# 82magnolia/piccolo

Measured on AMD Instinct MI355X. Metric: candidate-poses/s, higher is better.
Workload: dtype f32

## Files before the change

### include/piccolo_hip.h

```cpp
#ifndef PICCOLO_HIP_H
#define PICCOLO_HIP_H

#include <stddef.h>
#include <stdint.h>

#ifdef __cplusplus
extern "C" {
#endif

#define PCL_ABI_VERSION 11

#define PCL_EINVAL (-1)
#define PCL_EWORKSPACE (-2)

#define PCL_MAX_POINTS ((int64_t)1 << 27)

#define PCL_RESULT_STRIDE 8

int pcl_abi_version(void);
const char *pcl_error_string(int code);
const char *pcl_source_hash(void);
const char *pcl_library_hash(void);

#define PCL_PANO_F32 0
#define PCL_PANO_U8 1
#define PCL_PANO_F16 2
#define PCL_PANO_U8P 3
#define PCL_PANO_U8V 4
int64_t pcl_cloud_stride(int64_t n);
size_t pcl_cloud_bytes(int64_t n);
int pcl_cloud_pack(const float *xyz, const float *rgb, const int64_t *order, int64_t n, float *cloud, void *stream);
size_t pcl_cloud_sets_bytes(int64_t n, int nsets);
int pcl_cloud_pack_sets(const float *xyz, const float *const *rgb_host, int nsets, const int64_t *order, int64_t n, float *cloud, void *stream);
size_t pcl_cloud_order_workspace_bytes(int64_t n);
int pcl_cloud_order(const float *xyz, int64_t n, int64_t *order, void *workspace, size_t workspace_bytes, void *stream);
int pcl_morton_keys(const float *xyz, int64_t n, const float *lo_host, const float *hi_host, int64_t *keys, void *stream);

size_t pcl_pano_bytes(int H, int W, int pano_format);
int pcl_pano_pack(const float *img_hwc, int H, int W, float *pano, void *stream);
int pcl_pano_pack_u8(const float *img_hwc, int H, int W, uint32_t *pano, int *not_exact, void *stream);
int pcl_pano_pack_u8p(const float *img_hwc, int H, int W, uint32_t *pano, int *not_exact, void *stream);
int pcl_pano_pack_u8v(const float *img_hwc, int H, int W, uint32_t *pano, int *not_exact, void *stream);
int pcl_pano_pack_f16(const float *img_hwc, int H, int W, void *pano, int *not_exact, void *stream);

size_t pcl_loss_workspace_bytes(int64_t n, int B);
size_t pcl_loss_depth_workspace_bytes(int64_t n, int B, int H, int W, int depth_h, int depth_w, int depth_stride);
int pcl_sampling_loss_depth(const float *cloud, int64_t n, const void *pano, int pano_format, int H, int W, const float *trans,
                            const float *rot, int B, int with_grad, int depth_h, int depth_w, float tau, int depth_stride, float *result,
                            void *workspace, size_t workspace_bytes, void *stream);
int pcl_sampling_loss(const float *cloud, int64_t n, const void *pano, int pano_format, int H, int W, const float *trans,
                      const float *rot, int B, int with_grad, const uint8_t *visible, float *result, void *workspace,
                      size_t workspace_bytes, void *stream);

#define PCL_GD_SEQUENTIAL 0
#define PCL_GD_BATCH 1
#define PCL_GD_RESULT_STRIDE 16

typedef struct pcl_gd_hyper {
    double lr;
    double factor;
    int32_t patience;
    int32_t mode;
    int32_t depth_mask;
    float depth_tau;
    int32_t depth_h;
    int32_t depth_w;
    int32_t depth_stride;
    int32_t fuse;
    int32_t images;
    int32_t color_sets;
} pcl_gd_hyper;

size_t pcl_gd_state_bytes(int B);
size_t pcl_gd_workspace_bytes(int64_t n, int B, int H, int W, const pcl_gd_hyper *hyper_host);
int pcl_gd_init(void *state, const float *trans, const float *rot, int B, const pcl_gd_hyper *hyper_host, void *stream);
int pcl_gd_run(const float *cloud, int64_t n, const void *pano, int pano_format, int H, int W, void *state, int B, const float *box,
               const pcl_gd_hyper *hyper_host, int num_iter, float *loss_history, void *workspace,
               size_t workspace_bytes, void *timer, void *stream);
int pcl_gd_result(const void *state, int B, float *result, void *stream);
int pcl_gd_step_from_grads(void *state, int B, const float *loss, const float *grad, const float *box, const pcl_gd_hyper *hyper_host,
                           float *scratch, void *stream);
int pcl_gd_plan(int64_t n, int B, int *nchunks_host, int *poses_per_block_host, int *fused_host);
int pcl_gd_plan_hyper(int64_t n, int B, const pcl_gd_hyper *hyper_host, int *nchunks_host, int *poses_per_block_host, int *fused_host);
int pcl_gd_set_panos(void *state, const uint64_t *panos, int B, void *stream);
int pcl_gd_set_pano_groups(void *state, const uint64_t *panos_host, int nimages, int per_image, void *stream);
int pcl_gd_winner(const void *state, int nimages, int per_image, float *winners, float *leaf_trans, float *leaf_rot, void *stream);

#define PCL_GD_MAX_ROOMS 32
typedef struct pcl_gd_room {
    const float *cloud;
    int64_t n;
    const float *box;
} pcl_gd_room;
size_t pcl_gd_rooms_workspace_bytes(const pcl_gd_room *rooms_host, int nrooms, int per_room, const pcl_gd_hyper *hyper_host);
int pcl_gd_plan_rooms(const pcl_gd_room *rooms_host, int nrooms, int per_room, const pcl_gd_hyper *hyper_host, int *nchunks_host,
                      int *poses_per_block_host, int *fused_host);
int pcl_gd_run_rooms(const pcl_gd_room *rooms_host, int nrooms, const void *pano, int pano_format, int H, int W, void *state, int per_room,
                     const pcl_gd_hyper *hyper_host, int num_iter, float *loss_history, void *workspace, size_t workspace_bytes, void *timer,
                     void *stream);

void *pcl_timer_create(int capacity);
void pcl_timer_destroy(void *timer);
void pcl_timer_reset(void *timer);
void pcl_timer_set_stride(void *timer, int stride);
int pcl_timer_read(void *timer, double *total_ms_host, int *launches_host);
int pcl_timer_calibrate(void *timer, int reps, double *pair_ms_host, void *stream);

int pcl_cloud2idx(const float *xyz, int64_t n, float *coord, void *stream);
int pcl_sample_from_img(const void *pano, int pano_format, int H, int W, const float *coord, int64_t n, float *rgb_out,
                        void *stream);
int pcl_cloud2idx_backward(const float *xyz, const float *grad_coord, int64_t n, float *grad_xyz, void *stream);
int pcl_sample_from_img_backward(const void *pano, int pano_format, int H, int W, const float *coord, const float *grad_rgb,
                                 int64_t n, float *grad_coord, float *grad_img, void *stream);
int pcl_rot_from_ypr(const float *rot, int B, float *R, void *stream);
size_t pcl_quantile_workspace_bytes(void);
int pcl_quantile_box(const float *xyz, int64_t n, double q, float *box, void *workspace, void *stream);

int pcl_scatter_min_depth(const float *xyz_cam, int64_t n, int H, int W, uint64_t *zbuf, void *stream);
int pcl_scatter_min_unpack(const uint64_t *zbuf, int64_t n, int H, int W, float *zmin, int64_t *argmin, void *stream);
int pcl_make_pano(const float *xyz_cam, const float *rgb, int64_t n, int H, int W, float *image, uint64_t *workspace,
                  void *stream);
size_t pcl_hist_trim_workspace_bytes(int ncand, int H, int W, int nsh, int nsw);
size_t pcl_hist_trim_workspace_bytes_n(int64_t n, int ncand, int H, int W, int nsh, int nsw);
int pcl_hist_trim_scores(const float *cloud, int64_t n, const float *img_hwc, int H, int W, const float *trans,
                         const float *rot, int ncand, int nsh, int nsw, float *inter, int32_t *nproj, int32_t *nimg,
                         void *workspace, size_t workspace_bytes, void *stream);
int pcl_hist_trim_reduce(const float *inter, const int32_t *nproj, const int32_t *nimg, int ncand, int nsh, int nsw, float *score,
                         void *stream);
size_t pcl_hist_trim_images_workspace_bytes(int64_t n, int nimages, int cand_per_image, int H, int W, int nsh, int nsw);
int pcl_hist_trim_scores_images(const float *cloud, int64_t n, const float *const *imgs_host, int nimages, int cand_per_image, int H, int W,
                                const float *trans, const float *rot, int nsh, int nsw, float *inter, int32_t *nproj, int32_t *nimg,
                                void *workspace, size_t workspace_bytes, void *stream);
size_t pcl_hist_trim_images_sets_workspace_bytes(int64_t n, int color_sets, int nimages, int cand_per_image, int H, int W, int nsh, int nsw);
int pcl_hist_trim_scores_images_sets(const float *cloud, int64_t n, int color_sets, const float *const *imgs_host, int nimages, int cand_per_image,
                                     int H, int W, const float *trans, const float *rot, int nsh, int nsw, float *inter, int32_t *nproj,
                                     int32_t *nimg, void *workspace, size_t workspace_bytes, void *stream);
int pcl_hist_trim_reduce_images(const float *inter, const int32_t *nproj, const int32_t *nimg, int nimages, int cand_per_image, int nsh,
                                int nsw, float *score, void *stream);
size_t pcl_trim_groups_bytes(int R);
int pcl_select_poses(const float *values, int nprob, int M, int n_keep, int largest, const float *trans, const float *rot,
                     int rot_per_trans, int64_t pose_stride, float *out_trans, float *out_rot, int *out_idx, void *stream);
int pcl_trim_groups(const float *rot, int R, void *groups, void *stream);
size_t pcl_trim_loss_workspace_bytes(int64_t n, int K, int ngroups);
int pcl_trim_loss(const float *cloud, int64_t n, const void *pano, int pano_format, int H, int W, const float *trans, int K,
                  const float *rot, int R, const void *groups, int ngroups, const void *order, float *loss_table, float *count_table,
                  void *workspace, size_t workspace_bytes, void *stream);
size_t pcl_trim_order_bytes(int64_t n, int K, int ngroups);
size_t pcl_trim_order_workspace_bytes(int64_t n, int K, int ngroups);
int pcl_trim_order(const float *cloud, int64_t n, int pano_format, int H, int W, const float *trans, int K, const float *rot, int R,
                   const void *groups, int ngroups, void *order, void *workspace, size_t workspace_bytes, void *stream);
size_t pcl_trim_loss_images_workspace_bytes(int64_t n, int K, int ngroups, int nimages);
int pcl_trim_loss_images(const float *cloud, int64_t n, const void *const *panos_host, int nimages, int pano_format, int H, int W,
                         const float *trans, int K, const float *rot, int R, const void *groups, int ngroups, const void *order,
                         float *loss_tables, float *count_tables, void *workspace, size_t workspace_bytes, void *stream);
int pcl_trim_loss_images_sets(const float *cloud, int64_t n, int color_sets, const void *const *panos_host, int nimages, int pano_format, int H,
                              int W, const float *trans, int K, const float *rot, int R, const void *groups, int ngroups, const void *order,
                              float *loss_tables, float *count_tables, void *workspace, size_t workspace_bytes, void *stream);
int pcl_depth_default(int64_t n, int H, int W, int stride_in, int *depth_h_host, int *depth_w_host, float *tau_host, int *stride_host);
size_t pcl_depth_workspace_bytes(int B, int H, int W);
int pcl_depth_mask(const float *cloud, int64_t n, const float *trans, const float *rot, int B, int H, int W, float tau, int stride,
                   uint8_t *visible, void *workspace, size_t workspace_bytes, void *stream);
size_t pcl_color_template_bytes(int64_t n);
size_t pcl_color_template_workspace_bytes(int64_t n);
int pcl_color_template_build(const float *rgb, int64_t n, float *tmpl, void *workspace, size_t workspace_bytes, void *stream);
size_t pcl_color_workspace_bytes(void);
int pcl_color_match(const float *img_hwc, int H, int W, const float *tmpl, int64_t n, float *out, int32_t *not_exact,
                    void *workspace, size_t workspace_bytes, void *stream);
int pcl_color_mod(const float *img_hwc, int H, int W, const float *rgb, int64_t n, int num_bins, float *out_img,
                  float *out_rgb, void *workspace, size_t workspace_bytes, void *stream);
size_t pcl_histogram_workspace_bytes(int c0, int c1, int c2);
int pcl_histogram(const float *img, const uint8_t *mask, int64_t npix, int c0, int c1, int c2, int normalize, float eps,
                  float *hist, void *workspace, size_t workspace_bytes, void *stream);
int pcl_histogram_intersection(const float *a, const float *b, int batch, int nbins, float *out, void *stream);
int pcl_transform_cloud(const float *xyz, int64_t n, const float *trans, const float *rot, float *out, void *stream);

int64_t pcl_cloud_txt_rows(const char *path);
int64_t pcl_cloud_txt_read(const char *path, int64_t rows, int cols, double *out, int nthreads);

#ifdef __cplusplus
}
#endif
#endif
```

### piccolo_amd/_lib.py

```python
import ctypes
import os

from . import build as _build

_c = ctypes
_vp, _i64, _int, _sz, _dbl = _c.c_void_p, _c.c_int64, _c.c_int, _c.c_size_t, _c.c_double

ABI_VERSION = 11
RESULT_STRIDE = 8
GD_RESULT_STRIDE = 16
GD_SEQUENTIAL, GD_BATCH = 0, 1
PANO_F32, PANO_U8, PANO_F16, PANO_U8P, PANO_U8V = 0, 1, 2, 3, 4


class GdHyper(_c.Structure):
    _fields_ = [("lr", _dbl), ("factor", _dbl), ("patience", _c.c_int32), ("mode", _c.c_int32),
                ("depth_mask", _c.c_int32), ("depth_tau", _c.c_float), ("depth_h", _c.c_int32), ("depth_w", _c.c_int32),
                ("depth_stride", _c.c_int32), ("fuse", _c.c_int32), ("images", _c.c_int32), ("color_sets", _c.c_int32)]


GD_MAX_ROOMS = 32


class GdRoom(_c.Structure):
    _fields_ = [("cloud", _vp), ("n", _i64), ("box", _vp)]


SIGNATURES = {
    "pcl_abi_version": (_int, []),
    "pcl_error_string": (_c.c_char_p, [_int]),
    "pcl_source_hash": (_c.c_char_p, []),
    "pcl_library_hash": (_c.c_char_p, []),
    "pcl_cloud_stride": (_i64, [_i64]),
    "pcl_cloud_bytes": (_sz, [_i64]),
    "pcl_cloud_pack": (_int, [_vp, _vp, _vp, _i64, _vp, _vp]),
    "pcl_cloud_sets_bytes": (_sz, [_i64, _int]),
    "pcl_cloud_pack_sets": (_int, [_vp, _c.POINTER(_vp), _int, _vp, _i64, _vp, _vp]),
    "pcl_morton_keys": (_int, [_vp, _i64, _c.POINTER(_c.c_float), _c.POINTER(_c.c_float), _vp, _vp]),
    "pcl_pano_bytes": (_sz, [_int, _int, _int]),
    "pcl_pano_pack": (_int, [_vp, _int, _int, _vp, _vp]),
    "pcl_cloud_order_workspace_bytes": (_sz, [_i64]),
    "pcl_cloud_order": (_int, [_vp, _i64, _vp, _vp, _sz, _vp]),
    "pcl_pano_pack_u8": (_int, [_vp, _int, _int, _vp, _vp, _vp]),
    "pcl_pano_pack_u8p": (_int, [_vp, _int, _int, _vp, _vp, _vp]),
    "pcl_pano_pack_u8v": (_int, [_vp, _int, _int, _vp, _vp, _vp]),
    "pcl_pano_pack_f16": (_int, [_vp, _int, _int, _vp, _vp, _vp]),
    "pcl_loss_workspace_bytes": (_sz, [_i64, _int]),
    "pcl_sampling_loss": (_int, [_vp, _i64, _vp, _int, _int, _int, _vp, _vp, _int, _int, _vp, _vp, _vp, _sz, _vp]),
    "pcl_loss_depth_workspace_bytes": (_sz, [_i64, _int, _int, _int, _int, _int, _int]),
    "pcl_sampling_loss_depth": (_int, [_vp, _i64, _vp, _int, _int, _int, _vp, _vp, _int, _int, _int, _int, _c.c_float, _int, _vp, _vp, _sz, _vp]),
    "pcl_depth_default": (_int, [_i64, _int, _int, _int, _c.POINTER(_int), _c.POINTER(_int), _c.POINTER(_c.c_float), _c.POINTER(_int)]),
    "pcl_gd_state_bytes": (_sz, [_int]),
    "pcl_gd_workspace_bytes": (_sz, [_i64, _int, _int, _int, _c.POINTER(GdHyper)]),
    "pcl_hist_trim_workspace_bytes": (_sz, [_int, _int, _int, _int, _int]),
    "pcl_hist_trim_workspace_bytes_n": (_sz, [_i64, _int, _int, _int, _int, _int]),
    "pcl_hist_trim_scores": (_int, [_vp, _i64, _vp, _int, _int, _vp, _vp, _int, _int, _int, _vp, _vp, _vp, _vp, _sz, _vp]),
    "pcl_color_template_bytes": (_sz, [_i64]),
    "pcl_color_template_workspace_bytes": (_sz, [_i64]),
    "pcl_color_template_build": (_int, [_vp, _i64, _vp, _vp, _sz, _vp]),
    "pcl_color_workspace_bytes": (_sz, []),
    "pcl_color_match": (_int, [_vp, _int, _int, _vp, _i64, _vp, _vp, _vp, _sz, _vp]),
    "pcl_color_mod": (_int, [_vp, _int, _int, _vp, _i64, _int, _vp, _vp, _vp, _sz, _vp]),
    "pcl_histogram_workspace_bytes": (_sz, [_int, _int, _int]),
    "pcl_histogram": (_int, [_vp, _vp, _i64, _int, _int, _int, _int, _c.c_float, _vp, _vp, _sz, _vp]),
    "pcl_histogram_intersection": (_int, [_vp, _vp, _int, _int, _vp, _vp]),
    "pcl_cloud_txt_rows": (_i64, [_c.c_char_p]),
    "pcl_cloud_txt_read": (_i64, [_c.c_char_p, _i64, _int, _vp, _int]),
    "pcl_hist_trim_reduce": (_int, [_vp, _vp, _vp, _int, _int, _int, _vp, _vp]),
    "pcl_hist_trim_images_workspace_bytes": (_sz, [_i64, _int, _int, _int, _int, _int, _int]),
    "pcl_hist_trim_scores_images": (_int, [_vp, _i64, _c.POINTER(_vp), _int, _int, _int, _int, _vp, _vp, _int, _int, _vp, _vp, _vp, _vp, _sz, _vp]),
    "pcl_hist_trim_reduce_images": (_int, [_vp, _vp, _vp, _int, _int, _int, _int, _vp, _vp]),
    "pcl_hist_trim_images_sets_workspace_bytes": (_sz, [_i64, _int, _int, _int, _int, _int, _int, _int]),
    "pcl_hist_trim_scores_images_sets": (_int, [_vp, _i64, _int, _c.POINTER(_vp), _int, _int, _int, _int, _vp, _vp, _int, _int, _vp, _vp, _vp, _vp, _sz, _vp]),
    "pcl_trim_groups_bytes": (_sz, [_int]),
    "pcl_trim_groups": (_int, [_vp, _int, _vp, _vp]),
    "pcl_trim_loss_workspace_bytes": (_sz, [_i64, _int, _int]),
    "pcl_trim_loss": (_int, [_vp, _i64, _vp, _int, _int, _int, _vp, _int, _vp, _int, _vp, _int, _vp, _vp, _vp, _vp, _sz, _vp]),
    "pcl_trim_order_bytes": (_sz, [_i64, _int, _int]),
    "pcl_trim_order_workspace_bytes": (_sz, [_i64, _int, _int]),
    "pcl_trim_order": (_int, [_vp, _i64, _int, _int, _int, _vp, _int, _vp, _int, _vp, _int, _vp, _vp, _sz, _vp]),
    "pcl_trim_loss_images_workspace_bytes": (_sz, [_i64, _int, _int, _int]),
    "pcl_trim_loss_images": (_int, [_vp, _i64, _c.POINTER(_vp), _int, _int, _int, _int, _vp, _int, _vp, _int, _vp, _int, _vp, _vp, _vp, _vp, _sz, _vp]),
    "pcl_trim_loss_images_sets": (_int, [_vp, _i64, _int, _c.POINTER(_vp), _int, _int, _int, _int, _vp, _int, _vp, _int, _vp, _int, _vp, _vp, _vp, _vp, _sz, _vp]),
    "pcl_depth_workspace_bytes": (_sz, [_int, _int, _int]),
    "pcl_depth_mask": (_int, [_vp, _i64, _vp, _vp, _int, _int, _int, _c.c_float, _int, _vp, _vp, _sz, _vp]),
    "pcl_gd_init": (_int, [_vp, _vp, _vp, _int, _c.POINTER(GdHyper), _vp]),
    "pcl_gd_run": (_int, [_vp, _i64, _vp, _int, _int, _int, _vp, _int, _vp, _c.POINTER(GdHyper), _int, _vp, _vp, _sz, _vp, _vp]),
    "pcl_timer_create": (_vp, [_int]),
    "pcl_timer_destroy": (None, [_vp]),
    "pcl_timer_reset": (None, [_vp]),
    "pcl_timer_set_stride": (None, [_vp, _int]),
    "pcl_timer_read": (_int, [_vp, _c.POINTER(_dbl), _c.POINTER(_int)]),
    "pcl_timer_calibrate": (_int, [_vp, _int, _c.POINTER(_dbl), _vp]),
    "pcl_gd_result": (_int, [_vp, _int, _vp, _vp]),
    "pcl_gd_step_from_grads": (_int, [_vp, _int, _vp, _vp, _vp, _vp, _vp, _vp]),
    "pcl_gd_plan": (_int, [_i64, _int, _c.POINTER(_int), _c.POINTER(_int), _c.POINTER(_int)]),
    "pcl_gd_plan_hyper": (_int, [_i64, _int, _c.POINTER(GdHyper), _c.POINTER(_int), _c.POINTER(_int), _c.POINTER(_int)]),
    "pcl_gd_set_panos": (_int, [_vp, _vp, _int, _vp]),
    "pcl_gd_set_pano_groups": (_int, [_vp, _c.POINTER(_c.c_uint64), _int, _int, _vp]),
    "pcl_gd_winner": (_int, [_vp, _int, _int, _vp, _vp, _vp, _vp]),
    "pcl_gd_rooms_workspace_bytes": (_sz, [_c.POINTER(GdRoom), _int, _int, _c.POINTER(GdHyper)]),
    "pcl_gd_plan_rooms": (_int, [_c.POINTER(GdRoom), _int, _int, _c.POINTER(GdHyper), _c.POINTER(_int), _c.POINTER(_int), _c.POINTER(_int)]),
    "pcl_gd_run_rooms": (_int, [_c.POINTER(GdRoom), _int, _vp, _int, _int, _int, _vp, _int, _c.POINTER(GdHyper), _int, _vp, _vp, _sz, _vp, _vp]),
    "pcl_select_poses": (_int, [_vp, _int, _int, _int, _int, _vp, _vp, _int, _i64, _vp, _vp, _vp, _vp]),
    "pcl_cloud2idx": (_int, [_vp, _i64, _vp, _vp]),
    "pcl_sample_from_img": (_int, [_vp, _int, _int, _int, _vp, _i64, _vp, _vp]),
    "pcl_cloud2idx_backward": (_int, [_vp, _vp, _i64, _vp, _vp]),
    "pcl_sample_from_img_backward": (_int, [_vp, _int, _int, _int, _vp, _vp, _i64, _vp, _vp, _vp]),
    "pcl_rot_from_ypr": (_int, [_vp, _int, _vp, _vp]),
    "pcl_quantile_workspace_bytes": (_sz, []),
    "pcl_quantile_box": (_int, [_vp, _i64, _dbl, _vp, _vp, _vp]),
    "pcl_scatter_min_depth": (_int, [_vp, _i64, _int, _int, _vp, _vp]),
    "pcl_scatter_min_unpack": (_int, [_vp, _i64, _int, _int, _vp, _vp, _vp]),
    "pcl_make_pano": (_int, [_vp, _vp, _i64, _int, _int, _vp, _vp, _vp]),
    "pcl_transform_cloud": (_int, [_vp, _i64, _vp, _vp, _vp, _vp]),
}

_lib = None


class PiccoloHipError(RuntimeError):
    pass


def so_path():
    return os.environ.get("PCL_SO", _build.SO)


def load():
    global _lib
    if _lib is not None:
        return _lib
    import torch
    path = so_path()
    if not os.path.exists(path):
        raise PiccoloHipError(
            "piccolo_amd: %s not found. The MI355X HIP library is the only back end (no CPU fallback); "
            "build it with `python -m piccolo_amd.build`." % path)
    lib = ctypes.CDLL(path)
    for name, (res, args) in SIGNATURES.items():
        fn = getattr(lib, name)
        fn.restype, fn.argtypes = res, args
    if lib.pcl_abi_version() != ABI_VERSION:
        raise PiccoloHipError("piccolo_amd: ABI mismatch: library %d, binding %d" % (lib.pcl_abi_version(), ABI_VERSION))
    _lib = lib
    return lib


def check(rc, what):
    if rc != 0:
        raise PiccoloHipError("%s failed: %s (code %d)" % (what, load().pcl_error_string(rc).decode(), rc))
```

### piccolo_amd/csrc/pcl_device.h

```cpp
#pragma once
#include <hip/hip_runtime.h>
#include <stddef.h>
#include <stdint.h>

#include "../../include/piccolo_hip.h"

#ifdef PCL_EXPERIMENTS
#include <stdlib.h>
static inline int pcl_knob_read(const char* name, int dflt)
{
    const char* v = getenv(name);
    return v && *v ? atoi(v) : dflt;
}
#define PCL_KNOB(NAME, dflt) pcl_knob_read("PCL_" #NAME, (dflt))
#else
#define PCL_KNOB(NAME, dflt) (dflt)
#endif

#define PCL_WAVE 64
#define PCL_BLOCK 256
#define PCL_NACC 8

typedef float pcl_f4 __attribute__((ext_vector_type(4)));
typedef int pcl_i4 __attribute__((ext_vector_type(4)));
typedef int pcl_i2 __attribute__((ext_vector_type(2)));

struct PclPoseRec {
    float R[9];
    float t[3];
    uint32_t pano_lo, pano_hi;
    uint32_t cset;
    float pad;
};
static_assert(sizeof(PclPoseRec) == 64, "pose record is one 64-byte scalar-load line");
static_assert(offsetof(PclPoseRec, R) == 0 && offsetof(PclPoseRec, t) == 36, "pose record: t directly after R[9]");

struct PclGdPose {
    double lr;
    double best;
    float leaf[6];
    float fwd[6];
    float m[6];
    float v[6];
    float last_loss;
    int32_t num_bad;
    int32_t step;
    int32_t pad;
    double beta1_pow, beta2_pow;
    float sc[4];
};
static_assert(sizeof(PclGdPose) == 160, "GD state record");

struct PclDims {
    int H, W;
    int Wp;
    float half_w, half_h;
    float off_x, off_y;
    float k_phi, k_theta;
    float c_scale;
    float k_ix, k_iy;
};

__host__ __device__ inline PclDims pcl_make_dims(int H, int W, int pano_format = PCL_PANO_F32)
{
    PclDims d;
    d.H = H; d.W = W; d.Wp = W + 2;
    d.half_w = 0.5f * (float)W; d.half_h = 0.5f * (float)H;
    d.off_x = 0.5f * (float)(W - 1) + 1.0f; d.off_y = 0.5f * (float)(H - 1) + 1.0f;
    d.k_phi = (float)(-(double)W / (2.0 * 3.14159265358979323846));
    d.k_theta = (float)((double)H / 3.14159265358979323846);
    d.c_scale = 1.0f;
    d.k_ix = (float)(-(double)W / (2.0 * 3.14159265358979323846));
    d.k_iy = (float)(-(double)H / 3.14159265358979323846);
    if (pano_format == PCL_PANO_U8 || pano_format == PCL_PANO_F16) {
        d.k_phi = (float)(-(double)W / (2.0 * 3.14159265358979323846) / 255.0);
        d.k_theta = (float)((double)H / 3.14159265358979323846 / 255.0);
        d.c_scale = (float)(1.0 / 255.0);
    }
    return d;
}

struct PclDepthGrid {
    int Hd, Wd, last;
    float wm1, hm1;
    float tol2;
};
__host__ __device__ inline PclDepthGrid pcl_make_depth_grid(int Hd, int Wd, float tau)
{
    PclDepthGrid g;
    g.Hd = Hd; g.Wd = Wd; g.last = Hd * Wd - 1;
    g.wm1 = (float)(Wd - 1); g.hm1 = (float)(Hd - 1);
    g.tol2 = (1.0f + tau) * (1.0f + tau);
    return g;
}
struct PclDepthLook {
    const uint32_t* zbuf;
    PclDepthGrid grid;
    uint32_t* zclear;
    int64_t zclear_vec4;
};
__device__ inline void pcl_rot_from_ypr(float yaw, float pitch, float roll, float R[9])
{
    double sy, cy, sp, cp, sr, cr;
    sincos((double)yaw, &sy, &cy);
    sincos((double)pitch, &sp, &cp);
    sincos((double)roll, &sr, &cr);
    sy = (double)(float)sy; cy = (double)(float)cy; sp = (double)(float)sp;
    cp = (double)(float)cp; sr = (double)(float)sr; cr = (double)(float)cr;
    R[0] = (float)(cy * cp); R[1] = (float)(cy * sp * sr - sy * cr); R[2] = (float)(cy * sp * cr + sy * sr);
    R[3] = (float)(sy * cp); R[4] = (float)(sy * sp * sr + cy * cr); R[5] = (float)(sy * sp * cr - cy * sr);
    R[6] = (float)(-sp);     R[7] = (float)(cp * sr);                R[8] = (float)(cp * cr);
}

__device__ inline void pcl_write_pose_rec(PclPoseRec* rec, const float p[6])
{
    float R[9];
    pcl_rot_from_ypr(p[3], p[4], p[5], R);
    for (int k = 0; k < 9; k++) rec->R[k] = R[k];
    rec->t[0] = p[0]; rec->t[1] = p[1]; rec->t[2] = p[2];
    rec->pano_lo = 0u; rec->pano_hi = 0u;
    rec->cset = 0u; rec->pad = 0.f;
}

__device__ inline void pcl_write_pose_rec_fast(PclPoseRec* rec, const float p[6], float sc[4])
{
    float sy, cy, sp, cp, sr, cr;
    sincosf(p[3], &sy, &cy);
    sincosf(p[4], &sp, &cp);
    sincosf(p[5], &sr, &cr);
    double dsy = sy, dcy = cy, dsp = sp, dcp = cp, dsr = sr, dcr = cr;
    rec->R[0] = (float)(dcy * dcp); rec->R[1] = (float)(dcy * dsp * dsr - dsy * dcr); rec->R[2] = (float)(dcy * dsp * dcr + dsy * dsr);
    rec->R[3] = (float)(dsy * dcp); rec->R[4] = (float)(dsy * dsp * dsr + dcy * dcr); rec->R[5] = (float)(dsy * dsp * dcr - dcy * dsr);
    rec->R[6] = (float)(-dsp);      rec->R[7] = (float)(dcp * dsr);                   rec->R[8] = (float)(dcp * dcr);
    rec->t[0] = p[0]; rec->t[1] = p[1]; rec->t[2] = p[2];
    sc[0] = sy; sc[1] = cy; sc[2] = sp; sc[3] = cp;
}

__device__ inline void pcl_cloud2idx_point(float px, float py, float pz, float& gx, float& gy)
{
#pragma clang fp contract(off)
    const float pi = 3.14159265358979323846f, two_pi = 6.28318530717958647692f;
    float rho = sqrtf(px * px + py * py);
    float theta = atan2f(rho, pz + 1e-6f);
    float phi = atan2f(py, px + 1e-6f) + pi;
    float cx = 1.0f - phi / two_pi;
    float cy = theta / pi;
    gx = 2.0f * cx - 1.0f;
    gy = 2.0f * cy - 1.0f;
}

__device__ __forceinline__ float pcl_atan_poly(float t)
{
    float s = t * t;
    float p = 2.4566929979e-03f;
    p = fmaf(p, s, -1.4401224869e-02f);
    p = fmaf(p, s, 3.9780993102e-02f);
    p = fmaf(p, s, -7.2348362183e-02f);
    p = fmaf(p, s, 1.0498935044e-01f);
    p = fmaf(p, s, -1.4161225936e-01f);
    p = fmaf(p, s, 1.9985906258e-01f);
    p = fmaf(p, s, -3.3332596993e-01f);
    p = fmaf(p, s, 9.9999988638e-01f);
    return p * t;
}

__device__ __forceinline__ float pcl_atan2(float y, float x)
{
    const float pi = 3.14159265358979323846f, half_pi = 1.57079632679489661923f;
    float ax = fabsf(x), ay = fabsf(y);
    float mx = fmaxf(fmaxf(ax, ay), 1e-37f), mn = fminf(ax, ay);
    float r = pcl_atan_poly(mn * __builtin_amdgcn_rcpf(mx));
    r = ay > ax ? half_pi - r : r;
    r = x < 0.f ? pi - r : r;
    return copysignf(r, y);
}

__device__ __forceinline__ float pcl_atan2_ypos(float y, float x)
{
    const float pi = 3.14159265358979323846f, half_pi = 1.57079632679489661923f;
    float ax = fabsf(x);
    float mx = fmaxf(fmaxf(ax, y), 1e-37f), mn = fminf(ax, y);
    float r = pcl_atan_poly(mn * __builtin_amdgcn_rcpf(mx));
    r = y > ax ? half_pi - r : r;
    return x < 0.f ? pi - r : r;
}

__device__ inline __amdgpu_buffer_rsrc_t pcl_tex_rsrc(const void* pano, int H, int W, int texel_bytes = 16)
{
    return __builtin_amdgcn_make_buffer_rsrc((void*)pano, 0, (int)((size_t)(H + 2) * (size_t)(W + 2) * (size_t)texel_bytes),
                                             0x00020000);
}

__host__ __device__ constexpr int pcl_texel_bytes(int fmt) { return fmt == PCL_PANO_U8 ? 4 : fmt == PCL_PANO_F16 ? 8 : 16; }

__device__ inline pcl_i2 pcl_texel_pair_u8(__amdgpu_buffer_rsrc_t rsrc, int voff, int soff)
{
    return __builtin_amdgcn_raw_buffer_load_b64(rsrc, voff, soff, 0);
}
__device__ __forceinline__ float pcl_ub0(int v) { float f; asm("v_cvt_f32_ubyte0 %0, %1" : "=v"(f) : "v"(v)); return f; }
__device__ __forceinline__ float pcl_ub1(int v) { float f; asm("v_cvt_f32_ubyte1 %0, %1" : "=v"(f) : "v"(v)); return f; }
__device__ __forceinline__ float pcl_ub2(int v) { float f; asm("v_cvt_f32_ubyte2 %0, %1" : "=v"(f) : "v"(v)); return f; }

__device__ inline pcl_f4 pcl_texel(__amdgpu_buffer_rsrc_t rsrc, int voff, int soff)
{
    pcl_i4 v = __builtin_amdgcn_raw_buffer_load_b128(rsrc, voff, soff, 0);
    return __builtin_bit_cast(pcl_f4, v);
}

template <int CTRL>
__device__ __forceinline__ float pcl_dpp(float v)
{
    return __builtin_bit_cast(float, __builtin_amdgcn_update_dpp(0, __builtin_bit_cast(int, v), CTRL, 0xf, 0xf, true));
}
__device__ __forceinline__ float pcl_wave_sum(float v)
{
    v += pcl_dpp<0xB1>(v);
    v += pcl_dpp<0x4E>(v);
    v += pcl_dpp<0x141>(v);
    v += pcl_dpp<0x140>(v);
    float r0 = __builtin_bit_cast(float, __builtin_amdgcn_readlane(__builtin_bit_cast(int, v), 0));
    float r1 = __builtin_bit_cast(float, __builtin_amdgcn_readlane(__builtin_bit_cast(int, v), 16));
    float r2 = __builtin_bit_cast(float, __builtin_amdgcn_readlane(__builtin_bit_cast(int, v), 32));
    float r3 = __builtin_bit_cast(float, __builtin_amdgcn_readlane(__builtin_bit_cast(int, v), 48));
    return (r0 + r1) + (r2 + r3);
}

template <int CTRL>
__device__ __forceinline__ double pcl_dpp_d(double v)
{
    pcl_i2 w = __builtin_bit_cast(pcl_i2, v);
    w.x = __builtin_amdgcn_update_dpp(0, w.x, CTRL, 0xf, 0xf, true);
    w.y = __builtin_amdgcn_update_dpp(0, w.y, CTRL, 0xf, 0xf, true);
    return __builtin_bit_cast(double, w);
}
__device__ __forceinline__ double pcl_readlane_d(double v, int lane)
{
    pcl_i2 w = __builtin_bit_cast(pcl_i2, v);
    w.x = __builtin_amdgcn_readlane(w.x, lane);
    w.y = __builtin_amdgcn_readlane(w.y, lane);
    return __builtin_bit_cast(double, w);
}
__device__ __forceinline__ double pcl_wave_sum_d(double v)
{
    v += pcl_dpp_d<0xB1>(v);
    v += pcl_dpp_d<0x4E>(v);
    v += pcl_dpp_d<0x141>(v);
    v += pcl_dpp_d<0x140>(v);
    return (pcl_readlane_d(v, 0) + pcl_readlane_d(v, 16)) + (pcl_readlane_d(v, 32) + pcl_readlane_d(v, 48));
}

#define PCL_LAUNCH_CHECK()                         \
    do {                                           \
        hipError_t e_ = hipGetLastError();         \
        if (e_ != hipSuccess) return (int)e_;      \
    } while (0)
```

### piccolo_amd/csrc/pcl_loss.hip

```cpp
#include <stdlib.h>

#include "pcl_gd_device.h"
#include "pcl_sample_device.h"

struct PclLossArgs {
    const float* cloud;
    int64_t n, stride;
    const void* pano;
    PclDims dims;
    const PclPoseRec* poses;
    int B;
    const uint8_t* visible;
    const uint32_t* zbuf;
    PclDepthGrid dgrid;
    pcl_i4* zclear;
    int zclear_per_block;
    int64_t zclear_total;
    float* partials;
    int nchunks;
    int ngroups;
    int flip;
    int seg_len;
    int xcd_groups;
    int steps_base, steps_rem;
    int color_sets;
};

#define PCL_STEP (2 * PCL_BLOCK)

#ifdef PCL_BLOCK_TRACE
__device__ unsigned long long* pcl_trace_buf = nullptr;
extern "C" int pcl_debug_set_block_trace(unsigned long long* buf)
{
    return (int)hipMemcpyToSymbol(HIP_SYMBOL(pcl_trace_buf), &buf, sizeof(buf));
}
#define PCL_TRACE_NOW() __builtin_amdgcn_s_memrealtime()
__global__ void pcl_debug_stamp_kernel(unsigned long long* slot) { *slot = PCL_TRACE_NOW(); }
extern "C" int pcl_debug_stamp(unsigned long long* slot, void* stream)
{
    hipLaunchKernelGGL(pcl_debug_stamp_kernel, dim3(1), dim3(1), 0, (hipStream_t)stream, slot);
    return (int)hipGetLastError();
}
#endif

template <int G, bool FUSED>
__device__ __forceinline__ unsigned pcl_room_select(const PclLossArgs& a_in, const PclFuseArgs& f_in, const PclRoomTable* __restrict__ tb, PclLossArgs& a,
                                                    PclFuseArgs& f)
{
    int r = -1;
#pragma unroll
    for (int q = 0; q < PCL_GD_MAX_ROOMS; q++) r += (int)blockIdx.x >= pcl_rfl(tb->block0[q]) ? 1 : 0;
    const PclRoomRec* __restrict__ rm = tb->rec + r;
    const int group0 = pcl_rfl(rm->group0), pose0 = group0 * G;
    const long long poff = (long long)pcl_rfl64((unsigned long long)rm->partials);
    a = a_in;
    a.cloud = (const float*)pcl_rfl64(rm->cloud);
    a.n = pcl_rfl(rm->n); a.stride = pcl_rfl(rm->stride);
    a.nchunks = pcl_rfl(rm->nchunks); a.seg_len = pcl_rfl(rm->seg_len);
    a.steps_base = pcl_rfl(rm->steps_base); a.steps_rem = pcl_rfl(rm->steps_rem);
    a.poses = a_in.poses + pose0;
    a.partials = a_in.partials + poff;
    a.xcd_groups = 0;
    f = f_in;
    if constexpr (FUSED) {
        f.partials_in = f_in.partials_in + poff;
        f.st_in = f_in.st_in + pose0; f.recs_in = f_in.recs_in + pose0;
        f.st_out = f_in.st_out + pose0; f.recs_out = f_in.recs_out + pose0;
        f.box = (const float*)pcl_rfl64(rm->box);
        f.loss_out = f_in.loss_out ? f_in.loss_out + pose0 : nullptr;
    }
    return blockIdx.x - (unsigned)pcl_rfl(rm->block0);
}

template <int G, bool GRAD, int VIS, int FMT, bool FUSED, bool CS = false, bool RM = false>
__device__ __forceinline__ void pcl_loss_body(const PclLossArgs& a_in, const PclFuseArgs& f_in, const PclRoomTable* rooms = nullptr)
{
    PclLossArgs a_rm;
    PclFuseArgs f_rm;
    unsigned bid = blockIdx.x;
    if constexpr (RM) bid = pcl_room_select<G, FUSED>(a_in, f_in, rooms, a_rm, f_rm);
    const PclLossArgs& a = RM ? a_rm : a_in;
    const PclFuseArgs& f = RM ? f_rm : f_in;
    int group, chunk;
    if (a.xcd_groups) {
        const int gpx = a.ngroups >> 3, j = (int)(bid >> 3), cj = j / gpx;
        group = (int)(bid & 7) * gpx + (j - cj * gpx);
        chunk = a.flip ? a.nchunks - 1 - cj : cj;
    } else {
        const int lq = (int)(bid >> 3) / a.ngroups;
        group = (int)(bid >> 3) - lq * a.ngroups;
        const int lc = a.flip ? (a.nchunks >> 3) - 1 - lq : lq;
        const int run = lc / a.seg_len;
        chunk = (run * 8 + (int)(bid & 7)) * a.seg_len + (lc - run * a.seg_len);
    }
    const int pose0 = group * G;

    PclPose6 P6[G];
    unsigned PANO[G][2];
    __amdgpu_buffer_rsrc_t tex = pcl_tex_rsrc(a.pano, a.dims.H, a.dims.W, pcl_texel_bytes(FMT));
    __amdgpu_buffer_rsrc_t cld = __builtin_amdgcn_make_buffer_rsrc((void*)a.cloud, 0, CS ? (int)(a.stride * (3 + 3 * a.color_sets) * 4) : (int)(a.stride * 6 * 4),
                                                                   0x00020000);
    const int plane = (int)a.stride * 4;
    int cplane = 3 * plane;
    if constexpr (CS) cplane = (int)(3u + 3u * (unsigned)__builtin_amdgcn_readfirstlane((int)(a.poses + pose0)->cset)) * plane;
    __amdgpu_buffer_rsrc_t zb = __amdgpu_buffer_rsrc_t();
    if constexpr (VIS == 2) zb = __builtin_amdgcn_make_buffer_rsrc((void*)a.zbuf, 0, (int)((unsigned)a.B * (unsigned)(a.dgrid.last + 1) * 4u), 0x00020000);

    f2 acc[G][PCL_NACC];
    int count[G];
#pragma unroll
    for (int g = 0; g < G; g++) {
        count[g] = 0;
#pragma unroll
        for (int k = 0; k < PCL_NACC; k++) acc[g][k] = F2(0.f);
    }

    int first = chunk * a.steps_base + min(chunk, a.steps_rem);
    int nsteps = a.steps_base + (chunk < a.steps_rem ? 1 : 0);
    const int begin = first * PCL_STEP;
    int end = begin + nsteps * PCL_STEP;
    if (end > (int)a.n) end = (int)a.n;
    const int last = (int)a.n - 1;

    auto load_step = [&](int base, float (&dst)[2][6]) {
        int j0 = min(base + (int)threadIdx.x, last), j1 = min(base + PCL_BLOCK + (int)threadIdx.x, last);
#pragma unroll
        for (int k = 0; k < 6; k++) {
            const int soff = (CS && k >= 3) ? cplane + (k - 3) * plane : k * plane;
            dst[0][k] = __builtin_bit_cast(float, __builtin_amdgcn_raw_buffer_load_b32(cld, j0 * 4, soff, 0));
            dst[1][k] = __builtin_bit_cast(float, __builtin_amdgcn_raw_buffer_load_b32(cld, j1 * 4, soff, 0));
        }
    };
    auto eval_step = [&](int base, const float (&src)[2][6]) {
        const int i0 = base + threadIdx.x, i1 = i0 + PCL_BLOCK;
        const bool valid0 = i0 < end, valid1 = i1 < end;
        const unsigned long long vmask0 = __builtin_amdgcn_ballot_w64(valid0), vmask1 = __builtin_amdgcn_ballot_w64(valid1);
        f2 x = {src[0][0], src[1][0]}, y = {src[0][1], src[1][1]}, z = {src[0][2], src[1][2]};
        f2 ncr = {src[0][3], src[1][3]}, ncg = {src[0][4], src[1][4]}, ncb = {src[0][5], src[1][5]};
#ifndef PCL_NO_ROTATE_PAIR
        f2 rot_p[G][3];
#ifdef PCL_TIMING_ONLY_NO_ROTATION
        if constexpr (G == 2) {
            const f2 oa = F2((a.poses + pose0)->t[0]), ob = F2((a.poses + pose0 + 1)->t[0]);
            rot_p[0][0] = x - oa; rot_p[0][1] = y; rot_p[0][2] = z;
            rot_p[1][0] = x - ob; rot_p[1][1] = y; rot_p[1][2] = z;
        } else
#endif
        if constexpr (G == 2) {
            if constexpr (FUSED) pcl_rotate2x2(x, y, z, P6[0], P6[1], rot_p[0][0], rot_p[0][1], rot_p[0][2], rot_p[1][0], rot_p[1][1], rot_p[1][2]);
            else pcl_rotate2x2(x, y, z, pcl_pose6(a.poses + pose0), pcl_pose6(a.poses + pose0 + 1), rot_p[0][0], rot_p[0][1], rot_p[0][2],
                               rot_p[1][0], rot_p[1][1], rot_p[1][2]);
        }
#endif
#pragma unroll
        for (int g = 0; g < G; g++) {
            const PclPoseRec* __restrict__ pr = a.poses + (pose0 + g);
            bool ok0 = valid0, ok1 = valid1;
            unsigned long long m0 = vmask0, m1 = vmask1;
            if constexpr (VIS == 1) {
                const uint8_t* vis = a.visible + (int64_t)(pose0 + g) * a.n;
                ok0 = ok0 && vis[min(i0, last)] != 0;
                ok1 = ok1 && vis[min(i1, last)] != 0;
                m0 = __builtin_amdgcn_ballot_w64(ok0); m1 = __builtin_amdgcn_ballot_w64(ok1);
            }
            __amdgpu_buffer_rsrc_t tg = tex;
            unsigned pano_lo = pr->pano_lo, pano_hi = pr->pano_hi;
            if constexpr (FUSED) {
                pano_lo = PANO[g][0]; pano_hi = PANO[g][1];
            }
            if (pano_lo | pano_hi) {
                const void* pp = (const void*)(((unsigned long long)pano_hi << 32) | (unsigned long long)pano_lo);
                tg = pcl_tex_rsrc(pp, a.dims.H, a.dims.W, pcl_texel_bytes(FMT));
            }
            PclProj<FMT> pj;
            const int zoff = VIS == 2 ? (int)((unsigned)(pose0 + g) * (unsigned)(a.dgrid.last + 1) * 4u) : 0;
#ifndef PCL_NO_ROTATE_PAIR
            if constexpr (G == 2) {
                pj.px = rot_p[g][0]; pj.py = rot_p[g][1]; pj.pz = rot_p[g][2];
                pcl_project2_rotated<FMT, VIS == 2>(tg, a.dims, pj, zb, zoff, &a.dgrid);
            } else
#endif
            if constexpr (FUSED) pcl_project2<FMT, VIS == 2>(x, y, z, P6[g], tg, a.dims, pj, zb, zoff, &a.dgrid);
            else pcl_project2<FMT, VIS == 2>(x, y, z, pcl_pose6(pr), tg, a.dims, pj, zb, zoff, &a.dgrid);
            if constexpr (VIS == 2) {
                f2 d2 = pcl_fma2(pj.pz, pj.pz, pj.rho2);
                const bool v0 = d2.x <= __uint_as_float(pj.zq0), v1 = d2.y <= __uint_as_float(pj.zq1);
                ok0 = ok0 & v0; ok1 = ok1 & v1;
                m0 = __builtin_amdgcn_ballot_w64(ok0); m1 = __builtin_amdgcn_ballot_w64(ok1);
            }
            pcl_sample2<GRAD, FMT>(pj, ncr, ncg, ncb, ok0, ok1, m0, m1, tg, a.dims, acc[g], count[g]);
        }
    };
    float bufA[2][6], bufB[2][6];
    load_step(begin, bufA);
    if constexpr (FUSED) {
        static_assert(PCL_BLOCK == PCL_GD_THREADS, "the fused prologue reduces with the epilogue kernel's thread layout");
        __shared__ double gd_rows[(PCL_GD_THREADS / 16) * 2 * G][4];
        __shared__ double gd_sums[G][PCL_NACC];
        __shared__ float pose_sh[G][12];
        pcl_gd_finish_group<G, true>(f.partials_in, a.nchunks, group, (int)threadIdx.x, f.st_in, f.recs_in, f.st_out, f.recs_out, chunk == 0,
                                     f.box, f.factor, f.patience, f.mode, f.loss_out, gd_rows, gd_sums, pose_sh);
        __syncthreads();
#pragma unroll
        for (int g = 0; g < G; g++) {
            float v[12];
#pragma unroll
            for (int k = 0; k < 12; k++) v[k] = __builtin_bit_cast(float, __builtin_amdgcn_readfirstlane(__builtin_bit_cast(int, pose_sh[g][k])));
            P6[g] = PclPose6{(f2){v[0], v[1]}, (f2){v[2], v[3]}, (f2){v[4], v[5]}, (f2){v[6], v[7]}, (f2){v[8], v[9]}, (f2){v[10], v[11]}};
            const PclPoseRec* pr = a.poses + (pose0 + g);
            PANO[g][0] = (unsigned)__builtin_amdgcn_readfirstlane((int)pr->pano_lo);
            PANO[g][1] = (unsigned)__builtin_amdgcn_readfirstlane((int)pr->pano_hi);
        }
    }

    for (int base = begin; base < end; base += 2 * PCL_STEP) {
        load_step(base + PCL_STEP, bufB);
        eval_step(base, bufA);
        if (base + PCL_STEP < end) {
            load_step(base + 2 * PCL_STEP, bufA);
            eval_step(base + PCL_STEP, bufB);
        }
    }

    __shared__ float red[PCL_BLOCK / PCL_WAVE][G * PCL_NACC];
    const int lane = threadIdx.x & 63, wave = threadIdx.x >> 6;
#pragma unroll
    for (int g = 0; g < G; g++)
#pragma unroll
        for (int k = 0; k < PCL_NACC; k++) {
            if (k == 1) {
                if (lane == 0) red[wave][g * PCL_NACC + 1] = (float)count[g];
                continue;
            }
            if (!GRAD && k >= 2) continue;
            float s = pcl_wave_sum(acc[g][k].x + acc[g][k].y);
            if (lane == 0) red[wave][g * PCL_NACC + k] = s;
        }
    __syncthreads();
    if (threadIdx.x < G * PCL_NACC) {
        int g = threadIdx.x / PCL_NACC, k = threadIdx.x - g * PCL_NACC;
        float s = 0.f;
        if (GRAD || k < 2) s = red[0][threadIdx.x] + red[1][threadIdx.x] + red[2][threadIdx.x] + red[3][threadIdx.x];
        a.partials[pcl_partials_row(a.nchunks, G, group, chunk, g) + k] = s;
    }
    if constexpr (VIS == 2) {
        if (a.zclear) {
            const pcl_i4 inf4 = {0x7f800000, 0x7f800000, 0x7f800000, 0x7f800000};
            const int64_t z0 = (int64_t)blockIdx.x * a.zclear_per_block;
            for (int i = threadIdx.x; i < a.zclear_per_block; i += PCL_BLOCK)
                if (z0 + i < a.zclear_total) a.zclear[z0 + i] = inf4;
        }
    }
#ifdef PCL_BLOCK_TRACE
    if (pcl_trace_buf && threadIdx.x == 0) {
        unsigned hw, xcc;
        asm volatile("s_getreg_b32 %0, hwreg(HW_REG_HW_ID)" : "=s"(hw));
        asm volatile("s_getreg_b32 %0, hwreg(HW_REG_XCC_ID)" : "=s"(xcc));
        unsigned long long* t = pcl_trace_buf + (size_t)blockIdx.x * 4;
        t[0] = 0; t[1] = 0; t[2] = PCL_TRACE_NOW(); t[3] = ((unsigned long long)xcc << 32) | hw;
    }
#endif
}

template <int G, bool GRAD, int VIS, int FMT>
__global__ void __launch_bounds__(PCL_BLOCK) pcl_loss_kernel(PclLossArgs a)
{
    pcl_loss_body<G, GRAD, VIS, FMT, false>(a, PclFuseArgs{});
}

template <int G, int FMT>
__global__ void __launch_bounds__(PCL_BLOCK) pcl_loss_fused_kernel(PclLossArgs a, PclFuseArgs f)
{
    pcl_loss_body<G, true, 0, FMT, true>(a, f);
}

template <int G, int FMT>
__global__ void __launch_bounds__(PCL_BLOCK) pcl_loss_sets_kernel(PclLossArgs a)
{
    pcl_loss_body<G, true, 0, FMT, false, true>(a, PclFuseArgs{});
}

template <int G, int FMT>
__global__ void __launch_bounds__(PCL_BLOCK) pcl_loss_fused_sets_kernel(PclLossArgs a, PclFuseArgs f)
{
    pcl_loss_body<G, true, 0, FMT, true, true>(a, f);
}

template <int G, int FMT>
__global__ void __launch_bounds__(PCL_BLOCK) pcl_loss_rooms_kernel(PclLossArgs a, const PclRoomTable* rooms)
{
    pcl_loss_body<G, true, 0, FMT, false, false, true>(a, PclFuseArgs{}, rooms);
}

template <int G, int FMT>
__global__ void __launch_bounds__(PCL_BLOCK) pcl_loss_fused_rooms_kernel(PclLossArgs a, PclFuseArgs f, const PclRoomTable* rooms)
{
    pcl_loss_body<G, true, 0, FMT, true, false, true>(a, f, rooms);
}



struct PclPlan {
    int G, ngroups, nchunks;
    int seg_len;
    int steps_base, steps_rem;
};

static int pcl_xcd_seg_len(int nchunks, int64_t nblocks)
{
    static const int runs_env = PCL_KNOB(XCD_RUNS, 0);
    int cpx = nchunks / 8, runs = runs_env < 1 || runs_env > cpx ? cpx : runs_env;
    if (runs_env < 1 && nblocks <= 1024) runs = 1;
    while (cpx % runs) runs--;
    return cpx / runs;
}

static PclPlan pcl_plan(int64_t n, int B)
{
    static const int g_env = PCL_KNOB(G, 0), blocks_env = PCL_KNOB(BLOCKS, 4096);
    PclPlan p;
    p.G = (B % 2 == 0) ? 2 : 1;
    if (g_env > 0 && B % g_env == 0) p.G = g_env;
    p.ngroups = B / p.G;
    int64_t want = blocks_env / p.ngroups;
    if (want < 64) want = 64;
    if (n > 2000000 && want < n / 8192) want = n / 8192;
    int64_t steps = (n + PCL_STEP - 1) / PCL_STEP;
    if (steps < 3 * want) {
        int64_t alt = steps / 3;
        if (alt < 1024 / p.ngroups) alt = 1024 / p.ngroups;
        if (alt < 32) alt = 32;
        if (alt < want) want = alt;
    }
    if (want > steps) want = steps;
    want = ((want + 7) / 8) * 8;
    p.nchunks = (int)want;
    p.steps_base = (int)(steps / want);
    p.steps_rem = (int)(steps % want);
    p.seg_len = pcl_xcd_seg_len(p.nchunks, (int64_t)p.nchunks * p.ngroups);
    return p;
}

static PclPlan pcl_plan_sets(int64_t n, int B, int sets)
{
    if (sets <= 1) return pcl_plan(n, B);
    PclPlan p = pcl_plan(n, B / sets);
    p.ngroups = B / p.G;
    p.seg_len = pcl_xcd_seg_len(p.nchunks, (int64_t)p.nchunks * p.ngroups);
    return p;
}

void pcl_plan_room(int64_t n, int per_room, int* G, int* ngroups, int* nchunks, int* seg_len, int* steps_base, int* steps_rem)
{
    const PclPlan p = pcl_plan(n, per_room);
    *G = p.G; *ngroups = p.ngroups; *nchunks = p.nchunks; *seg_len = p.seg_len; *steps_base = p.steps_base; *steps_rem = p.steps_rem;
}

size_t pcl_partials_bytes(int64_t n, int B, int sets)
{
    PclPlan p = pcl_plan_sets(n, B, sets);
    return (size_t)p.nchunks * (size_t)B * PCL_NACC * sizeof(float);
}

int pcl_plan_nchunks(int64_t n, int B, int sets) { return pcl_plan_sets(n, B, sets).nchunks; }
int pcl_plan_nblocks(int64_t n, int B, int sets) { PclPlan p = pcl_plan_sets(n, B, sets); return p.nchunks * p.ngroups; }
int pcl_plan_G(int64_t n, int B, int sets) { return pcl_plan_sets(n, B, sets).G; }

void pcl_plan_for_groups(int64_t n, int ngroups, int* nchunks, int* seg_len, int* steps_base, int* steps_rem)
{
    PclPlan p = pcl_plan(n, 2 * ngroups);
    static const int chunks_env = PCL_KNOB(TRIM_CHUNKS, 0);
    int auto_chunks = 0;
    const int64_t per_chunk = n <= 2000000 ? 8192 : 16384;
    if (chunks_env < 8 && n > 64 * per_chunk) auto_chunks = (int)((n + per_chunk - 1) / per_chunk);
    if (chunks_env >= 8 || auto_chunks) {
        int64_t steps = (n + PCL_STEP - 1) / PCL_STEP, want = (((chunks_env >= 8 ? chunks_env : auto_chunks) + 7) / 8) * 8;
        if (want > steps) want = ((steps + 7) / 8) * 8;
        p.nchunks = (int)want; p.steps_base = (int)(steps / want); p.steps_rem = (int)(steps % want);
        static const int runs_env = PCL_KNOB(TRIM_RUNS, 0);
        int cpx = p.nchunks / 8, runs = runs_env < 1 || runs_env > cpx ? cpx : runs_env;
        while (cpx % runs) runs--;
        p.seg_len = cpx / runs;
    }
    *nchunks = p.nchunks; *seg_len = p.seg_len; *steps_base = p.steps_base; *steps_rem = p.steps_rem;
}

template <int G, int FMT>
static void pcl_launch_g(const PclLossArgs& a, int nblk, bool grad, int vis, hipStream_t s)
{
    if (grad) {
        if (vis == 2) hipLaunchKernelGGL((pcl_loss_kernel<G, true, 2, FMT>), dim3(nblk), dim3(PCL_BLOCK), 0, s, a);
        else if (vis) hipLaunchKernelGGL((pcl_loss_kernel<G, true, 1, FMT>), dim3(nblk), dim3(PCL_BLOCK), 0, s, a);
        else hipLaunchKernelGGL((pcl_loss_kernel<G, true, 0, FMT>), dim3(nblk), dim3(PCL_BLOCK), 0, s, a);
    } else {
        if (vis == 2) hipLaunchKernelGGL((pcl_loss_kernel<G, false, 2, FMT>), dim3(nblk), dim3(PCL_BLOCK), 0, s, a);
        else if (vis) hipLaunchKernelGGL((pcl_loss_kernel<G, false, 1, FMT>), dim3(nblk), dim3(PCL_BLOCK), 0, s, a);
        else hipLaunchKernelGGL((pcl_loss_kernel<G, false, 0, FMT>), dim3(nblk), dim3(PCL_BLOCK), 0, s, a);
    }
}

template <int FMT>
static void pcl_launch_f(const PclLossArgs& a, int G, int nblk, bool grad, int vis, hipStream_t s)
{
    if (G == 4) pcl_launch_g<4, FMT>(a, nblk, grad, vis, s);
    else if (G == 2) pcl_launch_g<2, FMT>(a, nblk, grad, vis, s);
    else pcl_launch_g<1, FMT>(a, nblk, grad, vis, s);
}

template <int FMT>
static void pcl_launch_fused(const PclLossArgs& a, const PclFuseArgs& f, int G, int nblk, hipStream_t s)
{
    if (G == 4) hipLaunchKernelGGL((pcl_loss_fused_kernel<4, FMT>), dim3(nblk), dim3(PCL_BLOCK), 0, s, a, f);
    else if (G == 2) hipLaunchKernelGGL((pcl_loss_fused_kernel<2, FMT>), dim3(nblk), dim3(PCL_BLOCK), 0, s, a, f);
    else hipLaunchKernelGGL((pcl_loss_fused_kernel<1, FMT>), dim3(nblk), dim3(PCL_BLOCK), 0, s, a, f);
}

template <int FMT>
static void pcl_launch_sets(const PclLossArgs& a, const PclFuseArgs* f, int G, int nblk, hipStream_t s)
{
    if (f) {
        if (G == 4) hipLaunchKernelGGL((pcl_loss_fused_sets_kernel<4, FMT>), dim3(nblk), dim3(PCL_BLOCK), 0, s, a, *f);
        else if (G == 2) hipLaunchKernelGGL((pcl_loss_fused_sets_kernel<2, FMT>), dim3(nblk), dim3(PCL_BLOCK), 0, s, a, *f);
        else hipLaunchKernelGGL((pcl_loss_fused_sets_kernel<1, FMT>), dim3(nblk), dim3(PCL_BLOCK), 0, s, a, *f);
    } else {
        if (G == 4) hipLaunchKernelGGL((pcl_loss_sets_kernel<4, FMT>), dim3(nblk), dim3(PCL_BLOCK), 0, s, a);
        else if (G == 2) hipLaunchKernelGGL((pcl_loss_sets_kernel<2, FMT>), dim3(nblk), dim3(PCL_BLOCK), 0, s, a);
        else hipLaunchKernelGGL((pcl_loss_sets_kernel<1, FMT>), dim3(nblk), dim3(PCL_BLOCK), 0, s, a);
    }
}

int pcl_launch_loss_rooms(const PclRoomTable* rooms, const void* pano, int pano_format, int H, int W, const PclPoseRec* poses, int B, int G,
                          int ngroups, int nblk, float* partials, hipStream_t s, int flip, const PclFuseArgs* fuse)
{
    if (pano_format != PCL_PANO_F32 && pano_format != PCL_PANO_U8 && pano_format != PCL_PANO_F16) return PCL_EINVAL;
    if ((int64_t)(H + 2) * (W + 2) * pcl_texel_bytes(pano_format) >= ((int64_t)1 << 31)) return PCL_EINVAL;
    PclLossArgs a = PclLossArgs{};
    a.pano = pano; a.dims = pcl_make_dims(H, W, pano_format);
    a.poses = poses; a.B = B; a.partials = partials;
    a.ngroups = ngroups; a.flip = flip & 1; a.xcd_groups = 0; a.color_sets = 1;
    const dim3 grid(nblk), blk(PCL_BLOCK);
    if (fuse) {
        if (pano_format == PCL_PANO_U8) {
            if (G == 2) hipLaunchKernelGGL((pcl_loss_fused_rooms_kernel<2, PCL_PANO_U8>), grid, blk, 0, s, a, *fuse, rooms);
            else hipLaunchKernelGGL((pcl_loss_fused_rooms_kernel<1, PCL_PANO_U8>), grid, blk, 0, s, a, *fuse, rooms);
        } else if (pano_format == PCL_PANO_F16) {
            if (G == 2) hipLaunchKernelGGL((pcl_loss_fused_rooms_kernel<2, PCL_PANO_F16>), grid, blk, 0, s, a, *fuse, rooms);
            else hipLaunchKernelGGL((pcl_loss_fused_rooms_kernel<1, PCL_PANO_F16>), grid, blk, 0, s, a, *fuse, rooms);
        } else {
            if (G == 2) hipLaunchKernelGGL((pcl_loss_fused_rooms_kernel<2, PCL_PANO_F32>), grid, blk, 0, s, a, *fuse, rooms);
            else hipLaunchKernelGGL((pcl_loss_fused_rooms_kernel<1, PCL_PANO_F32>), grid, blk, 0, s, a, *fuse, rooms);
        }
    } else {
        if (pano_format == PCL_PANO_U8) {
            if (G == 2) hipLaunchKernelGGL((pcl_loss_rooms_kernel<2, PCL_PANO_U8>), grid, blk, 0, s, a, rooms);
            else hipLaunchKernelGGL((pcl_loss_rooms_kernel<1, PCL_PANO_U8>), grid, blk, 0, s, a, rooms);
        } else if (pano_format == PCL_PANO_F16) {
            if (G == 2) hipLaunchKernelGGL((pcl_loss_rooms_kernel<2, PCL_PANO_F16>), grid, blk, 0, s, a, rooms);
            else hipLaunchKernelGGL((pcl_loss_rooms_kernel<1, PCL_PANO_F16>), grid, blk, 0, s, a, rooms);
        } else {
            if (G == 2) hipLaunchKernelGGL((pcl_loss_rooms_kernel<2, PCL_PANO_F32>), grid, blk, 0, s, a, rooms);
            else hipLaunchKernelGGL((pcl_loss_rooms_kernel<1, PCL_PANO_F32>), grid, blk, 0, s, a, rooms);
        }
    }
    PCL_LAUNCH_CHECK();
    return 0;
}

int pcl_launch_loss(const float* cloud, int64_t n, const void* pano, int pano_format, int H, int W, const PclPoseRec* poses,
                    int B, bool grad, const uint8_t* visible, float* partials, hipStream_t s, int flip, const PclFuseArgs* fuse,
                    const PclDepthLook* depth, int color_sets)
{
    if (pano_format != PCL_PANO_F32 && pano_format != PCL_PANO_U8 && pano_format != PCL_PANO_F16) return PCL_EINVAL;
    if (n > PCL_MAX_POINTS || (int64_t)(H + 2) * (W + 2) * pcl_texel_bytes(pano_format) >= ((int64_t)1 << 31)) return PCL_EINVAL;
    const bool sets = color_sets > 1;
    if (sets && (B % color_sets || !grad || visible || depth || pcl_cloud_sets_bytes(n, color_sets) == 0)) return PCL_EINVAL;
    PclPlan p = pcl_plan_sets(n, B, color_sets);
    PclLossArgs a;
    a.cloud = cloud; a.n = n; a.stride = pcl_cloud_stride(n);
    a.pano = pano; a.dims = pcl_make_dims(H, W, pano_format);
    a.poses = poses; a.B = B; a.visible = visible; a.partials = partials;
    a.zbuf = nullptr; a.dgrid = PclDepthGrid{};
    a.zclear = nullptr; a.zclear_per_block = 0; a.zclear_total = 0;
    if (depth) {
        if (visible || !depth->zbuf || depth->grid.Hd <= 0 || depth->grid.Wd <= 0) return PCL_EINVAL;
        if ((int64_t)B * depth->grid.Hd * depth->grid.Wd * 4 >= ((int64_t)1 << 32)) return PCL_EINVAL;
        a.zbuf = depth->zbuf; a.dgrid = depth->grid;
        if (depth->zclear) {
            const int64_t nblk64 = (int64_t)p.nchunks * p.ngroups;
            a.zclear = (pcl_i4*)depth->zclear;
            a.zclear_total = depth->zclear_vec4;
            a.zclear_per_block = (int)((depth->zclear_vec4 + nblk64 - 1) / nblk64);
        }
    }
    a.nchunks = p.nchunks; a.ngroups = p.ngroups; a.seg_len = p.seg_len; a.flip = flip & 1; a.steps_base = p.steps_base; a.steps_rem = p.steps_rem;
    a.color_sets = sets ? color_sets : 1;
    static const int xg_env = PCL_KNOB(XCD_GROUPS, -1);
    a.xcd_groups = ((flip & 2) != 0 || xg_env == 1) && xg_env != 0 && p.ngroups % 8 == 0 ? 1 : 0;
    int nblk = p.nchunks * p.ngroups;
    const int vis = depth ? 2 : visible != nullptr ? 1 : 0;
    if (sets) {
        if (pano_format == PCL_PANO_U8) pcl_launch_sets<PCL_PANO_U8>(a, fuse, p.G, nblk, s);
        else if (pano_format == PCL_PANO_F16) pcl_launch_sets<PCL_PANO_F16>(a, fuse, p.G, nblk, s);
        else pcl_launch_sets<PCL_PANO_F32>(a, fuse, p.G, nblk, s);
        PCL_LAUNCH_CHECK();
        return 0;
    }
    if (fuse) {
        if (!grad || vis) return PCL_EINVAL;
        if (pano_format == PCL_PANO_U8) pcl_launch_fused<PCL_PANO_U8>(a, *fuse, p.G, nblk, s);
        else if (pano_format == PCL_PANO_F16) pcl_launch_fused<PCL_PANO_F16>(a, *fuse, p.G, nblk, s);
        else pcl_launch_fused<PCL_PANO_F32>(a, *fuse, p.G, nblk, s);
        PCL_LAUNCH_CHECK();
        return 0;
    }
    if (pano_format == PCL_PANO_U8) pcl_launch_f<PCL_PANO_U8>(a, p.G, nblk, grad, vis, s);
    else if (pano_format == PCL_PANO_F16) pcl_launch_f<PCL_PANO_F16>(a, p.G, nblk, grad, vis, s);
    else pcl_launch_f<PCL_PANO_F32>(a, p.G, nblk, grad, vis, s);
    PCL_LAUNCH_CHECK();
    return 0;
}
```

### piccolo_amd/csrc/pcl_pack.hip

```cpp
#include "pcl_device.h"

#include <rocprim/device/device_radix_sort.hpp>

extern "C" int pcl_abi_version(void) { return PCL_ABI_VERSION; }

#ifndef PCL_SOURCE_HASH
#define PCL_SOURCE_HASH "unstamped"
#endif
extern "C" const char* pcl_source_hash(void) { return PCL_SOURCE_HASH; }
#ifndef PCL_LIBRARY_HASH
#define PCL_LIBRARY_HASH "unstamped"
#endif
extern "C" const char* pcl_library_hash(void) { return PCL_LIBRARY_HASH; }

extern "C" const char* pcl_error_string(int code)
{
    if (code == 0) return "success";
    if (code == PCL_EINVAL) return "piccolo_hip: invalid argument";
    if (code == PCL_EWORKSPACE) return "piccolo_hip: workspace too small";
    if (code > 0) return hipGetErrorString((hipError_t)code);
    return "piccolo_hip: unknown error";
}

extern "C" int64_t pcl_cloud_stride(int64_t n) { return n <= 0 ? 0 : ((n + 255) / 256) * 256; }
extern "C" size_t pcl_cloud_bytes(int64_t n) { return (size_t)pcl_cloud_stride(n) * 6 * sizeof(float); }
extern "C" size_t pcl_pano_bytes(int H, int W, int pano_format)
{
    if (H <= 0 || W <= 0) return 0;
    if (pano_format == PCL_PANO_U8P) return (size_t)((H + 3) >> 1) * (size_t)(W + 2) * 8;
    if (pano_format == PCL_PANO_U8V) return (size_t)(H + 2) * (size_t)(W + 2) * 8;
    if (pano_format != PCL_PANO_F32 && pano_format != PCL_PANO_U8 && pano_format != PCL_PANO_F16) return 0;
    return (size_t)(H + 2) * (size_t)(W + 2) * (size_t)pcl_texel_bytes(pano_format);
}

__global__ void __launch_bounds__(PCL_BLOCK) pcl_cloud_pack_kernel(const float* __restrict__ xyz, const float* __restrict__ rgb,
                                                                   const int64_t* __restrict__ order, int64_t n,
                                                                   int64_t stride, float* __restrict__ cloud)
{
    int64_t i = (int64_t)blockIdx.x * PCL_BLOCK + threadIdx.x;
    if (i >= stride) return;
    float v[6] = {0.f, 0.f, 0.f, 0.f, 0.f, 0.f};
    if (i < n) {
        int64_t j = order ? order[i] : i;
        v[0] = xyz[3 * j]; v[1] = xyz[3 * j + 1]; v[2] = xyz[3 * j + 2];
        v[3] = -rgb[3 * j]; v[4] = -rgb[3 * j + 1]; v[5] = -rgb[3 * j + 2];
    }
#pragma unroll
    for (int k = 0; k < 6; k++) cloud[k * stride + i] = v[k];
}

extern "C" int pcl_cloud_pack(const float* xyz, const float* rgb, const int64_t* order, int64_t n, float* cloud, void* stream)
{
    if (!xyz || !rgb || !cloud || n <= 0) return PCL_EINVAL;
    int64_t stride = pcl_cloud_stride(n);
    hipLaunchKernelGGL(pcl_cloud_pack_kernel, dim3((unsigned)(stride / PCL_BLOCK)), dim3(PCL_BLOCK), 0, (hipStream_t)stream,
                       xyz, rgb, order, n, stride, cloud);
    PCL_LAUNCH_CHECK();
    return 0;
}

extern "C" size_t pcl_cloud_sets_bytes(int64_t n, int nsets)
{
    if (n <= 0 || n > PCL_MAX_POINTS || nsets <= 0) return 0;
    if (nsets == 1) return pcl_cloud_bytes(n);
    const int64_t bytes = (int64_t)pcl_cloud_stride(n) * 4 * (3 + 3 * (int64_t)nsets);
    return bytes < ((int64_t)1 << 31) ? (size_t)bytes : 0;
}

#define PCL_PACK_SETS 16
struct PclRgbList { const float* p[PCL_PACK_SETS]; };

__global__ void __launch_bounds__(PCL_BLOCK) pcl_cloud_pack_sets_kernel(const float* __restrict__ xyz, PclRgbList rgb, int k0, int m,
                                                                        const int64_t* __restrict__ order, int64_t n, int64_t stride,
                                                                        float* __restrict__ cloud)
{
    int64_t i = (int64_t)blockIdx.x * PCL_BLOCK + threadIdx.x;
    if (i >= stride) return;
    const int64_t j = i < n ? (order ? order[i] : i) : 0;
    if (k0 == 0)
        for (int c = 0; c < 3; c++) cloud[c * stride + i] = i < n ? xyz[3 * j + c] : 0.f;
    for (int k = 0; k < m; k++)
        for (int c = 0; c < 3; c++) cloud[(3 + 3 * (int64_t)(k0 + k) + c) * stride + i] = i < n ? -rgb.p[k][3 * j + c] : 0.f;
}

extern "C" int pcl_cloud_pack_sets(const float* xyz, const float* const* rgb_host, int nsets, const int64_t* order, int64_t n, float* cloud,
                                   void* stream)
{
    if (!xyz || !rgb_host || !cloud || n <= 0 || nsets <= 0) return PCL_EINVAL;
    if (pcl_cloud_sets_bytes(n, nsets) == 0) return PCL_EINVAL;
    for (int k = 0; k < nsets; k++)
        if (!rgb_host[k]) return PCL_EINVAL;
    if (nsets == 1) return pcl_cloud_pack(xyz, rgb_host[0], order, n, cloud, stream);
    const int64_t stride = pcl_cloud_stride(n);
    for (int k0 = 0; k0 < nsets; k0 += PCL_PACK_SETS) {
        const int m = nsets - k0 < PCL_PACK_SETS ? nsets - k0 : PCL_PACK_SETS;
        PclRgbList l;
        for (int k = 0; k < PCL_PACK_SETS; k++) l.p[k] = k < m ? rgb_host[k0 + k] : nullptr;
        hipLaunchKernelGGL(pcl_cloud_pack_sets_kernel, dim3((unsigned)(stride / PCL_BLOCK)), dim3(PCL_BLOCK), 0, (hipStream_t)stream, xyz, l, k0, m,
                           order, n, stride, cloud);
        PCL_LAUNCH_CHECK();
    }
    return 0;
}

__device__ inline uint64_t pcl_spread21(uint32_t v)
{
    uint64_t x = v & 0x1fffffu;
    x = (x | x << 32) & 0x1f00000000ffffull;
    x = (x | x << 16) & 0x1f0000ff0000ffull;
    x = (x | x << 8) & 0x100f00f00f00f00full;
    x = (x | x << 4) & 0x10c30c30c30c30c3ull;
    x = (x | x << 2) & 0x1249249249249249ull;
    return x;
}

__global__ void __launch_bounds__(PCL_BLOCK) pcl_morton_kernel(const float* __restrict__ xyz, int64_t n, float lx, float ly,
                                                               float lz, float sx, float sy, float sz,
                                                               int64_t* __restrict__ keys)
{
    int64_t i = (int64_t)blockIdx.x * PCL_BLOCK + threadIdx.x;
    if (i >= n) return;
    const float top = 2097151.f;
    float fx = __builtin_amdgcn_fmed3f((xyz[3 * i] - lx) * sx, 0.f, top);
    float fy = __builtin_amdgcn_fmed3f((xyz[3 * i + 1] - ly) * sy, 0.f, top);
    float fz = __builtin_amdgcn_fmed3f((xyz[3 * i + 2] - lz) * sz, 0.f, top);
    uint64_t k = pcl_spread21((uint32_t)fx) | (pcl_spread21((uint32_t)fy) << 1) | (pcl_spread21((uint32_t)fz) << 2);
    keys[i] = (int64_t)k;
}

extern "C" int pcl_morton_keys(const float* xyz, int64_t n, const float* lo, const float* hi, int64_t* keys, void* stream)
{
    if (!xyz || !lo || !hi || !keys || n <= 0) return PCL_EINVAL;
    float s[3];
    for (int k = 0; k < 3; k++) s[k] = hi[k] > lo[k] ? 2097151.f / (hi[k] - lo[k]) : 0.f;
    hipLaunchKernelGGL(pcl_morton_kernel, dim3((unsigned)((n + PCL_BLOCK - 1) / PCL_BLOCK)), dim3(PCL_BLOCK), 0,
                       (hipStream_t)stream, xyz, n, lo[0], lo[1], lo[2], s[0], s[1], s[2], keys);
    PCL_LAUNCH_CHECK();
    return 0;
}

__device__ __forceinline__ unsigned int pcl_ordered_key(float v)
{
    unsigned int b = __float_as_uint(v);
    return (b & 0x80000000u) ? ~b : (b | 0x80000000u);
}
__device__ __forceinline__ float pcl_ordered_value(unsigned int k)
{
    return __uint_as_float((k & 0x80000000u) ? (k & 0x7fffffffu) : ~k);
}

__global__ void __launch_bounds__(PCL_BLOCK) pcl_bbox_kernel(const float* __restrict__ xyz, int64_t n, unsigned int* __restrict__ box)
{
    unsigned int lo[3] = {~0u, ~0u, ~0u}, hi[3] = {0u, 0u, 0u};
    for (int64_t i = (int64_t)blockIdx.x * PCL_BLOCK + threadIdx.x; i < n; i += (int64_t)gridDim.x * PCL_BLOCK) {
#pragma unroll
        for (int c = 0; c < 3; c++) {
            unsigned int k = pcl_ordered_key(xyz[3 * i + c]);
            lo[c] = min(lo[c], k); hi[c] = max(hi[c], k);
        }
    }
#pragma unroll
    for (int c = 0; c < 3; c++) {
#pragma unroll
        for (int o = 32; o > 0; o >>= 1) {
            lo[c] = min(lo[c], (unsigned int)__shfl_xor((int)lo[c], o, 64));
            hi[c] = max(hi[c], (unsigned int)__shfl_xor((int)hi[c], o, 64));
        }
        if ((threadIdx.x & 63) == 0) { atomicMin(&box[c], lo[c]); atomicMax(&box[3 + c], hi[c]); }
    }
}

__global__ void __launch_bounds__(PCL_BLOCK) pcl_morton_box_kernel(const float* __restrict__ xyz, int64_t n, const unsigned int* __restrict__ box,
                                                                   unsigned long long* __restrict__ keys, int64_t* __restrict__ iota)
{
    int64_t i = (int64_t)blockIdx.x * PCL_BLOCK + threadIdx.x;
    if (i >= n) return;
    const float top = 2097151.f;
    unsigned long long k = 0ull;
#pragma unroll
    for (int c = 0; c < 3; c++) {
        float lo = pcl_ordered_value(box[c]), hi = pcl_ordered_value(box[3 + c]);
        float sc = hi > lo ? top / (hi - lo) : 0.f;
        float f = __builtin_amdgcn_fmed3f((xyz[3 * i + c] - lo) * sc, 0.f, top);
        k |= pcl_spread21((uint32_t)f) << c;
    }
    keys[i] = k;
    iota[i] = i;
}

static size_t order_align(size_t v) { return (v + 255) & ~(size_t)255; }
static size_t order_sort_temp_bytes(int64_t n)
{
    size_t bytes = 0;
    (void)rocprim::radix_sort_pairs<rocprim::default_config, const unsigned long long*, unsigned long long*, const int64_t*, int64_t*>(
        nullptr, bytes, nullptr, nullptr, nullptr, nullptr, (size_t)n, 0, 63, nullptr, false);
    return bytes;
}

extern "C" size_t pcl_cloud_order_workspace_bytes(int64_t n)
{
    if (n <= 0) return 0;
    return order_align(64) + 3 * order_align((size_t)n * 8) + order_align(order_sort_temp_bytes(n));
}

extern "C" int pcl_cloud_order(const float* xyz, int64_t n, int64_t* order, void* workspace, size_t workspace_bytes, void* stream)
{
    if (!xyz || !order || !workspace || n <= 0 || n > PCL_MAX_POINTS) return PCL_EINVAL;
    if (workspace_bytes < pcl_cloud_order_workspace_bytes(n)) return PCL_EWORKSPACE;
    hipStream_t s = (hipStream_t)stream;
    char* ws = (char*)workspace;
    unsigned int* box = (unsigned int*)ws; ws += order_align(64);
    unsigned long long* keys = (unsigned long long*)ws; ws += order_align((size_t)n * 8);
    unsigned long long* keys_sorted = (unsigned long long*)ws; ws += order_align((size_t)n * 8);
    int64_t* iota = (int64_t*)ws; ws += order_align((size_t)n * 8);
    hipError_t e = hipMemsetAsync(box, 0xff, 12, s);
    if (e == hipSuccess) e = hipMemsetAsync(box + 3, 0, 12, s);
    if (e != hipSuccess) return (int)e;
    int64_t blocks = (n + PCL_BLOCK - 1) / PCL_BLOCK;
    hipLaunchKernelGGL(pcl_bbox_kernel, dim3((unsigned)(blocks < 1024 ? blocks : 1024)), dim3(PCL_BLOCK), 0, s, xyz, n, box);
    hipLaunchKernelGGL(pcl_morton_box_kernel, dim3((unsigned)blocks), dim3(PCL_BLOCK), 0, s, xyz, n, box, keys, iota);
    PCL_LAUNCH_CHECK();
    size_t temp_bytes = order_sort_temp_bytes(n);
    e = rocprim::radix_sort_pairs(ws, temp_bytes, (const unsigned long long*)keys, keys_sorted, (const int64_t*)iota, order, (size_t)n, 0, 63,
                                  s, false);
    return e == hipSuccess ? 0 : (int)e;
}

__global__ void __launch_bounds__(PCL_BLOCK) pcl_pano_pack_kernel(const float* __restrict__ img, int H, int W,
                                                                  pcl_f4* __restrict__ pano)
{
    int Wp = W + 2, Hp = H + 2;
    int64_t i = (int64_t)blockIdx.x * PCL_BLOCK + threadIdx.x;
    if (i >= (int64_t)Wp * Hp) return;
    int yp = (int)(i / Wp), xp = (int)(i - (int64_t)yp * Wp);
    pcl_f4 v = {0.f, 0.f, 0.f, 0.f};
    if (yp >= 1 && yp <= H && xp >= 1 && xp <= W) {
        const float* s = img + ((int64_t)(yp - 1) * W + (xp - 1)) * 3;
        v.x = s[0]; v.y = s[1]; v.z = s[2];
    }
    pano[i] = v;
}

extern "C" int pcl_pano_pack(const float* img_hwc, int H, int W, float* pano, void* stream)
{
    if (!img_hwc || !pano || H <= 0 || W <= 0) return PCL_EINVAL;
    int64_t total = (int64_t)(H + 2) * (W + 2);
    hipLaunchKernelGGL(pcl_pano_pack_kernel, dim3((unsigned)((total + PCL_BLOCK - 1) / PCL_BLOCK)), dim3(PCL_BLOCK), 0,
                       (hipStream_t)stream, img_hwc, H, W, (pcl_f4*)pano);
    PCL_LAUNCH_CHECK();
    return 0;
}

__global__ void __launch_bounds__(PCL_BLOCK) pcl_pano_pack_u8_kernel(const float* __restrict__ img, int H, int W,
                                                                     uint32_t* __restrict__ pano, int* __restrict__ not_exact)
{
    int Wp = W + 2, Hp = H + 2;
    int64_t i = (int64_t)blockIdx.x * PCL_BLOCK + threadIdx.x;
    if (i >= (int64_t)Wp * Hp) return;
    int yp = (int)(i / Wp), xp = (int)(i - (int64_t)yp * Wp);
    uint32_t v = 0u;
    if (yp >= 1 && yp <= H && xp >= 1 && xp <= W) {
        const float* s = img + ((int64_t)(yp - 1) * W + (xp - 1)) * 3;
        bool bad = false;
#pragma unroll
        for (int c = 0; c < 3; c++) {
            float f = s[c], k = rintf(f * 255.f);
            bad = bad || !(k >= 0.f && k <= 255.f) || __fdiv_rn(k, 255.f) != f;
            v |= ((uint32_t)k & 255u) << (8 * c);
        }
        if (bad) *not_exact = 1;
    }
    pano[i] = v;
}

__global__ void __launch_bounds__(PCL_BLOCK) pcl_pano_pack_u8p_kernel(const float* __restrict__ img, int H, int W,
                                                                      uint32_t* __restrict__ pano, int* __restrict__ not_exact)
{
    const int Wp = W + 2, pairs = (H + 3) >> 1;
    int64_t i = (int64_t)blockIdx.x * PCL_BLOCK + threadIdx.x;
    if (i >= (int64_t)Wp * pairs * 2) return;
    const int yp = (int)(i / Wp), xp = (int)(i - (int64_t)yp * Wp);
    uint32_t v = 0u;
    if (yp >= 1 && yp <= H && xp >= 1 && xp <= W) {
        const float* s = img + ((int64_t)(yp - 1) * W + (xp - 1)) * 3;
        bool bad = false;
#pragma unroll
        for (int c = 0; c < 3; c++) {
            float f = s[c], k = rintf(f * 255.f);
            bad = bad || !(k >= 0.f && k <= 255.f) || __fdiv_rn(k, 255.f) != f;
            v |= ((uint32_t)k & 255u) << (8 * c);
        }
        if (bad) *not_exact = 1;
    }
    pano[((int64_t)(yp >> 1) * Wp + xp) * 2 + (yp & 1)] = v;
}

__global__ void __launch_bounds__(PCL_BLOCK) pcl_pano_pack_u8v_kernel(const float* __restrict__ img, int H, int W,
                                                                      pcl_i2* __restrict__ pano, int* __restrict__ not_exact)
{
    const int Wp = W + 2, Hp = H + 2;
    int64_t i = (int64_t)blockIdx.x * PCL_BLOCK + threadIdx.x;
    if (i >= (int64_t)Wp * Hp) return;
    const int yp = (int)(i / Wp), xp = (int)(i - (int64_t)yp * Wp);
    uint32_t v[2] = {0u, 0u};
    bool bad = false;
#pragma unroll
    for (int d = 0; d < 2; d++) {
        const int y = yp + d;
        if (y >= 1 && y <= H && xp >= 1 && xp <= W) {
            const float* s = img + ((int64_t)(y - 1) * W + (xp - 1)) * 3;
#pragma unroll
            for (int c = 0; c < 3; c++) {
                float f = s[c], k = rintf(f * 255.f);
                bad = bad || !(k >= 0.f && k <= 255.f) || __fdiv_rn(k, 255.f) != f;
                v[d] |= ((uint32_t)k & 255u) << (8 * c);
            }
        }
    }
    if (bad) *not_exact = 1;
    pano[i] = (pcl_i2){(int)v[0], (int)v[1]};
}

extern "C" int pcl_pano_pack_u8v(const float* img_hwc, int H, int W, uint32_t* pano, int* not_exact, void* stream)
{
    if (!img_hwc || !pano || !not_exact || H <= 0 || W <= 0) return PCL_EINVAL;
    int64_t total = (int64_t)(H + 2) * (W + 2);
    hipLaunchKernelGGL(pcl_pano_pack_u8v_kernel, dim3((unsigned)((total + PCL_BLOCK - 1) / PCL_BLOCK)), dim3(PCL_BLOCK), 0,
                       (hipStream_t)stream, img_hwc, H, W, (pcl_i2*)pano, not_exact);
    PCL_LAUNCH_CHECK();
    return 0;
}

__global__ void __launch_bounds__(PCL_BLOCK) pcl_pano_pack_f16_kernel(const float* __restrict__ img, int H, int W,
                                                                      pcl_i2* __restrict__ pano, int* __restrict__ not_exact)
{
    typedef _Float16 h2 __attribute__((ext_vector_type(2)));
    int Wp = W + 2, Hp = H + 2;
    int64_t i = (int64_t)blockIdx.x * PCL_BLOCK + threadIdx.x;
    if (i >= (int64_t)Wp * Hp) return;
    int yp = (int)(i / Wp), xp = (int)(i - (int64_t)yp * Wp);
    float lv[3] = {0.f, 0.f, 0.f};
    if (yp >= 1 && yp <= H && xp >= 1 && xp <= W) {
        const float* s = img + ((int64_t)(yp - 1) * W + (xp - 1)) * 3;
        bool bad = false;
#pragma unroll
        for (int c = 0; c < 3; c++) {
            float f = s[c], k = rintf(f * 255.f);
            bad = bad || !(k >= 0.f && k <= 255.f) || __fdiv_rn(k, 255.f) != f;
            lv[c] = k;
        }
        if (bad) *not_exact = 1;
    }
    h2 rg = {(_Float16)lv[0], (_Float16)lv[1]}, b0 = {(_Float16)lv[2], (_Float16)0.f};
    pano[i] = (pcl_i2){__builtin_bit_cast(int, rg), __builtin_bit_cast(int, b0)};
}

extern "C" int pcl_pano_pack_f16(const float* img_hwc, int H, int W, void* pano, int* not_exact, void* stream)
{
    if (!img_hwc || !pano || !not_exact || H <= 0 || W <= 0) return PCL_EINVAL;
    int64_t total = (int64_t)(H + 2) * (W + 2);
    hipLaunchKernelGGL(pcl_pano_pack_f16_kernel, dim3((unsigned)((total + PCL_BLOCK - 1) / PCL_BLOCK)), dim3(PCL_BLOCK), 0,
                       (hipStream_t)stream, img_hwc, H, W, (pcl_i2*)pano, not_exact);
    PCL_LAUNCH_CHECK();
    return 0;
}

extern "C" int pcl_pano_pack_u8p(const float* img_hwc, int H, int W, uint32_t* pano, int* not_exact, void* stream)
{
    if (!img_hwc || !pano || !not_exact || H <= 0 || W <= 0) return PCL_EINVAL;
    int64_t total = (int64_t)((H + 3) >> 1) * 2 * (W + 2);
    hipLaunchKernelGGL(pcl_pano_pack_u8p_kernel, dim3((unsigned)((total + PCL_BLOCK - 1) / PCL_BLOCK)), dim3(PCL_BLOCK), 0,
                       (hipStream_t)stream, img_hwc, H, W, pano, not_exact);
    PCL_LAUNCH_CHECK();
    return 0;
}

extern "C" int pcl_pano_pack_u8(const float* img_hwc, int H, int W, uint32_t* pano, int* not_exact, void* stream)
{
    if (!img_hwc || !pano || !not_exact || H <= 0 || W <= 0) return PCL_EINVAL;
    int64_t total = (int64_t)(H + 2) * (W + 2);
    hipLaunchKernelGGL(pcl_pano_pack_u8_kernel, dim3((unsigned)((total + PCL_BLOCK - 1) / PCL_BLOCK)), dim3(PCL_BLOCK), 0,
                       (hipStream_t)stream, img_hwc, H, W, pano, not_exact);
    PCL_LAUNCH_CHECK();
    return 0;
}
```

### piccolo_amd/csrc/pcl_sample_device.h

```cpp
#pragma once
#include "pcl_device.h"

typedef float f2 __attribute__((ext_vector_type(2)));
#define F2(s) ((f2){(s), (s)})

__device__ __forceinline__ f2 pcl_fma2(f2 a, f2 b, f2 c) { return __builtin_elementwise_fma(a, b, c); }

__device__ __forceinline__ f2 pcl_atan_poly2(f2 t)
{
    f2 s = t * t;
    f2 p = F2(2.4566929979e-03f);
    p = pcl_fma2(p, s, F2(-1.4401224869e-02f));
    p = pcl_fma2(p, s, F2(3.9780993102e-02f));
    p = pcl_fma2(p, s, F2(-7.2348362183e-02f));
    p = pcl_fma2(p, s, F2(1.0498935044e-01f));
    p = pcl_fma2(p, s, F2(-1.4161225936e-01f));
    p = pcl_fma2(p, s, F2(1.9985906258e-01f));
    p = pcl_fma2(p, s, F2(-3.3332596993e-01f));
    p = pcl_fma2(p, s, F2(9.9999988638e-01f));
    return p * t;
}

__device__ __forceinline__ float pcl_min_abs(float a, float b)
{
    float r;
    asm("v_min_f32_e64 %0, |%1|, |%2|" : "=v"(r) : "v"(a), "v"(b));
    return r;
}
__device__ __forceinline__ f2 pcl_atan_ratio2(float u0, float v0, float u1, float v1)
{
    f2 mn = {pcl_min_abs(u0, v0), pcl_min_abs(u1, v1)};
    f2 rc = {__builtin_amdgcn_rcpf(fmaxf(fmaxf(fabsf(u0), fabsf(v0)), 1e-37f)), __builtin_amdgcn_rcpf(fmaxf(fmaxf(fabsf(u1), fabsf(v1)), 1e-37f))};
    return pcl_atan_poly2(mn * rc);
}

__device__ __forceinline__ f2 pcl_atan2_2(f2 y, f2 x)
{
    const float half_pi = 1.57079632679489661923f;
    float ax0 = fabsf(x.x), ax1 = fabsf(x.y), ay0 = fabsf(y.x), ay1 = fabsf(y.y);
    f2 r = pcl_atan_ratio2(x.x, y.x, x.y, y.y);
    f2 alt = F2(half_pi) - r;
    r = (f2){ay0 > ax0 ? alt.x : r.x, ay1 > ax1 ? alt.y : r.y};
    f2 w = F2(half_pi) - r;
    w = (f2){copysignf(w.x, x.x), copysignf(w.y, x.y)};
    r = F2(half_pi) - w;
    return (f2){copysignf(r.x, y.x), copysignf(r.y, y.y)};
}

__device__ __forceinline__ f2 pcl_elevation2(f2 z, f2 rho)
{
    const float half_pi = 1.57079632679489661923f;
    float az0 = fabsf(z.x), az1 = fabsf(z.y);
    f2 r = pcl_atan_ratio2(rho.x, z.x, rho.y, z.y);
    f2 alt = F2(half_pi) - r;
    r = (f2){az0 > rho.x ? alt.x : r.x, az1 > rho.y ? alt.y : r.y};
    return (f2){copysignf(r.x, z.x), copysignf(r.y, z.y)};
}

template <int FMT> struct PclTaps;
template <> struct PclTaps<PCL_PANO_U8> { pcl_i2 top, bot; };
template <> struct PclTaps<PCL_PANO_F32> { int voff, row; };
template <> struct PclTaps<PCL_PANO_F16> { pcl_i4 top, bot; };

__device__ __forceinline__ void pcl_issue_taps(__amdgpu_buffer_rsrc_t tex, int x0, int y0, int Wp, PclTaps<PCL_PANO_U8>& o)
{
    int voff = (int)(__umul24((unsigned)y0, (unsigned)Wp) + (unsigned)x0) * 4;
    o.top = pcl_texel_pair_u8(tex, voff, 0);
    o.bot = pcl_texel_pair_u8(tex, voff, Wp * 4);
}
__device__ __forceinline__ void pcl_issue_taps(__amdgpu_buffer_rsrc_t tex, int x0, int y0, int Wp, PclTaps<PCL_PANO_F16>& o)
{
    int voff = (int)(__umul24((unsigned)y0, (unsigned)Wp) + (unsigned)x0) * 8;
    o.top = __builtin_amdgcn_raw_buffer_load_b128(tex, voff, 0, 0);
    o.bot = __builtin_amdgcn_raw_buffer_load_b128(tex, voff, Wp * 8, 0);
}
__device__ __forceinline__ void pcl_issue_taps(__amdgpu_buffer_rsrc_t tex, int x0, int y0, int Wp, PclTaps<PCL_PANO_F32>& o)
{
    o.voff = (int)(__umul24((unsigned)y0, (unsigned)Wp) + (unsigned)x0) * 16;
    o.row = Wp * 16;
}
__device__ __forceinline__ void pcl_unpack_taps(__amdgpu_buffer_rsrc_t, const PclTaps<PCL_PANO_U8>& r, float t[12])
{
    t[0] = pcl_ub0(r.top.x); t[1] = pcl_ub1(r.top.x); t[2] = pcl_ub2(r.top.x);
    t[3] = pcl_ub0(r.top.y); t[4] = pcl_ub1(r.top.y); t[5] = pcl_ub2(r.top.y);
    t[6] = pcl_ub0(r.bot.x); t[7] = pcl_ub1(r.bot.x); t[8] = pcl_ub2(r.bot.x);
    t[9] = pcl_ub0(r.bot.y); t[10] = pcl_ub1(r.bot.y); t[11] = pcl_ub2(r.bot.y);
}
__device__ __forceinline__ void pcl_unpack_taps(__amdgpu_buffer_rsrc_t tex, const PclTaps<PCL_PANO_F32>& r, float t[12])
{
    pcl_f4 t00 = pcl_texel(tex, r.voff, 0), t01 = pcl_texel(tex, r.voff + 16, 0);
    pcl_f4 t10 = pcl_texel(tex, r.voff, r.row), t11 = pcl_texel(tex, r.voff + 16, r.row);
    t[0] = t00.x; t[1] = t00.y; t[2] = t00.z; t[3] = t01.x; t[4] = t01.y; t[5] = t01.z;
    t[6] = t10.x; t[7] = t10.y; t[8] = t10.z; t[9] = t11.x; t[10] = t11.y; t[11] = t11.z;
}

typedef _Float16 pcl_h2 __attribute__((ext_vector_type(2)));
__device__ __forceinline__ float pcl_mix_lo(float a, pcl_h2 b, pcl_h2 c)
{
    float r;
    asm("v_fma_mix_f32 %0, %1, %2, %3 op_sel:[0,0,0] op_sel_hi:[0,1,1]" : "=v"(r) : "v"(a), "v"(b), "v"(c));
    return r;
}
__device__ __forceinline__ float pcl_mix_hi(float a, pcl_h2 b, pcl_h2 c)
{
    float r;
    asm("v_fma_mix_f32 %0, %1, %2, %3 op_sel:[0,1,1] op_sel_hi:[0,1,1]" : "=v"(r) : "v"(a), "v"(b), "v"(c));
    return r;
}
struct PclBilerp1 { float top[3], bot[3], dh[3]; };
template <bool GRAD>
__device__ __forceinline__ void pcl_bilerp_f16(const PclTaps<PCL_PANO_F16>& r, float fx, float fy, PclBilerp1& o)
{
    typedef _Float16 pcl_h8 __attribute__((ext_vector_type(8)));
    pcl_h8 tv = __builtin_bit_cast(pcl_h8, r.top), bv = __builtin_bit_cast(pcl_h8, r.bot);
    pcl_h2 t00a = __builtin_shufflevector(tv, tv, 0, 1), t00b = __builtin_shufflevector(tv, tv, 2, 3);
    pcl_h2 t01a = __builtin_shufflevector(tv, tv, 4, 5), t01b = __builtin_shufflevector(tv, tv, 6, 7);
    pcl_h2 t10a = __builtin_shufflevector(bv, bv, 0, 1), t10b = __builtin_shufflevector(bv, bv, 2, 3);
    pcl_h2 t11a = __builtin_shufflevector(bv, bv, 4, 5), t11b = __builtin_shufflevector(bv, bv, 6, 7);
    pcl_h2 dta = t01a - t00a, dtb = t01b - t00b, dba = t11a - t10a, dbb = t11b - t10b;
    o.top[0] = pcl_mix_lo(fx, dta, t00a); o.bot[0] = pcl_mix_lo(fx, dba, t10a);
    o.top[1] = pcl_mix_hi(fx, dta, t00a); o.bot[1] = pcl_mix_hi(fx, dba, t10a);
    o.top[2] = pcl_mix_lo(fx, dtb, t00b); o.bot[2] = pcl_mix_lo(fx, dbb, t10b);
    if (GRAD) {
        pcl_h2 dda = dba - dta, ddb = dbb - dtb;
        o.dh[0] = pcl_mix_lo(fy, dda, dta);
        o.dh[1] = pcl_mix_hi(fy, dda, dta);
        o.dh[2] = pcl_mix_lo(fy, ddb, dtb);
    }
}

template <int FMT>
struct PclProj {
    f2 px, py, pz;
    f2 rho2, rinv;
    f2 rs2;
    f2 fx, fy;
    bool in_phi0, in_phi1, in_th0, in_th1;
    PclTaps<FMT> ta, tb;
    unsigned zq0, zq1;
};

__device__ __forceinline__ void pcl_depth_cells2(f2 phi, f2 hel, const PclDepthGrid& g, int& row0, int& col0, int& row1, int& col1)
{
    const float inv_2pi = 0.15915494309189532f;
    f2 colf = pcl_fma2(-phi, F2(inv_2pi), F2(0.5f)) * F2(g.wm1);
    f2 rowf = pcl_fma2(-(hel * F2(4.0f)), F2(inv_2pi), F2(0.5f)) * F2(g.hm1);
    row0 = (int)rowf.x; col0 = (int)colf.x; row1 = (int)rowf.y; col1 = (int)colf.y;
}

struct PclPose6 { f2 p0, p1, p2, p3, p4, p5; };
__device__ __forceinline__ PclPose6 pcl_pose6(const PclPoseRec* __restrict__ pose)
{
    const f2* __restrict__ P = reinterpret_cast<const f2*>(pose->R);
    return PclPose6{P[0], P[1], P[2], P[3], P[4], P[5]};
}
__device__ __forceinline__ void pcl_rotate2(f2 x, f2 y, f2 z, const PclPose6& P, f2& opx, f2& opy, f2& opz)
{
    const f2 p0 = P.p0, p1 = P.p1, p2 = P.p2, p3 = P.p3, p4 = P.p4, p5 = P.p5;
    f2 qx, qy, qz, px, py, pz;
    asm("v_pk_add_f32 %3, %6, %13 op_sel:[0,1] op_sel_hi:[1,1] neg_lo:[0,1] neg_hi:[0,1]\n\t"
        "v_pk_add_f32 %4, %7, %14 op_sel_hi:[1,0] neg_lo:[0,1] neg_hi:[0,1]\n\t"
        "v_pk_add_f32 %5, %8, %14 op_sel:[0,1] op_sel_hi:[1,1] neg_lo:[0,1] neg_hi:[0,1]\n\t"
        "v_pk_mul_f32 %0, %3, %9 op_sel_hi:[1,0]\n\t"
        "v_pk_mul_f32 %1, %3, %10 op_sel:[0,1] op_sel_hi:[1,1]\n\t"
        "v_pk_mul_f32 %2, %3, %12 op_sel_hi:[1,0]\n\t"
        "v_pk_fma_f32 %0, %9, %4, %0 op_sel:[1,0,0] op_sel_hi:[1,1,1]\n\t"
        "v_pk_fma_f32 %1, %11, %4, %1 op_sel_hi:[0,1,1]\n\t"
        "v_pk_fma_f32 %2, %12, %4, %2 op_sel:[1,0,0] op_sel_hi:[1,1,1]\n\t"
        "v_pk_fma_f32 %0, %10, %5, %0 op_sel_hi:[0,1,1]\n\t"
        "v_pk_fma_f32 %1, %11, %5, %1 op_sel:[1,0,0] op_sel_hi:[1,1,1]\n\t"
        "v_pk_fma_f32 %2, %13, %5, %2 op_sel_hi:[0,1,1]\n\t"
        "s_nop 0"
        : "=&v"(px), "=&v"(py), "=&v"(pz), "=&v"(qx), "=&v"(qy), "=&v"(qz)
        : "v"(x), "v"(y), "v"(z), "s"(p0), "s"(p1), "s"(p2), "s"(p3), "s"(p4), "s"(p5));
    opx = px; opy = py; opz = pz;
}
#ifndef PCL_NO_ROTATE_PAIR
__device__ __forceinline__ void pcl_rotate2x2(f2 x, f2 y, f2 z, const PclPose6& A, const PclPose6& B, f2& apx, f2& apy, f2& apz, f2& bpx,
                                              f2& bpy, f2& bpz)
{
    f2 aqx, aqy, aqz, bqx, bqy, bqz, ax, ay, az, bx, by, bz;
    asm("v_pk_add_f32 %6, %12, %19 op_sel:[0,1] op_sel_hi:[1,1] neg_lo:[0,1] neg_hi:[0,1]\n\t"
        "v_pk_add_f32 %9, %12, %25 op_sel:[0,1] op_sel_hi:[1,1] neg_lo:[0,1] neg_hi:[0,1]\n\t"
        "v_pk_add_f32 %7, %13, %20 op_sel_hi:[1,0] neg_lo:[0,1] neg_hi:[0,1]\n\t"
        "v_pk_add_f32 %10, %13, %26 op_sel_hi:[1,0] neg_lo:[0,1] neg_hi:[0,1]\n\t"
        "v_pk_add_f32 %8, %14, %20 op_sel:[0,1] op_sel_hi:[1,1] neg_lo:[0,1] neg_hi:[0,1]\n\t"
        "v_pk_add_f32 %11, %14, %26 op_sel:[0,1] op_sel_hi:[1,1] neg_lo:[0,1] neg_hi:[0,1]\n\t"
        "v_pk_mul_f32 %0, %6, %15 op_sel_hi:[1,0]\n\t"
        "v_pk_mul_f32 %3, %9, %21 op_sel_hi:[1,0]\n\t"
        "v_pk_mul_f32 %1, %6, %16 op_sel:[0,1] op_sel_hi:[1,1]\n\t"
        "v_pk_mul_f32 %4, %9, %22 op_sel:[0,1] op_sel_hi:[1,1]\n\t"
        "v_pk_mul_f32 %2, %6, %18 op_sel_hi:[1,0]\n\t"
        "v_pk_mul_f32 %5, %9, %24 op_sel_hi:[1,0]\n\t"
        "v_pk_fma_f32 %0, %15, %7, %0 op_sel:[1,0,0] op_sel_hi:[1,1,1]\n\t"
        "v_pk_fma_f32 %3, %21, %10, %3 op_sel:[1,0,0] op_sel_hi:[1,1,1]\n\t"
        "v_pk_fma_f32 %1, %17, %7, %1 op_sel_hi:[0,1,1]\n\t"
        "v_pk_fma_f32 %4, %23, %10, %4 op_sel_hi:[0,1,1]\n\t"
        "v_pk_fma_f32 %2, %18, %7, %2 op_sel:[1,0,0] op_sel_hi:[1,1,1]\n\t"
        "v_pk_fma_f32 %5, %24, %10, %5 op_sel:[1,0,0] op_sel_hi:[1,1,1]\n\t"
        "v_pk_fma_f32 %0, %16, %8, %0 op_sel_hi:[0,1,1]\n\t"
        "v_pk_fma_f32 %3, %22, %11, %3 op_sel_hi:[0,1,1]\n\t"
        "v_pk_fma_f32 %1, %17, %8, %1 op_sel:[1,0,0] op_sel_hi:[1,1,1]\n\t"
        "v_pk_fma_f32 %4, %23, %11, %4 op_sel:[1,0,0] op_sel_hi:[1,1,1]\n\t"
        "v_pk_fma_f32 %2, %19, %8, %2 op_sel_hi:[0,1,1]\n\t"
        "v_pk_fma_f32 %5, %25, %11, %5 op_sel_hi:[0,1,1]\n\t"
        "s_nop 0"
        : "=&v"(ax), "=&v"(ay), "=&v"(az), "=&v"(bx), "=&v"(by), "=&v"(bz), "=&v"(aqx), "=&v"(aqy), "=&v"(aqz), "=&v"(bqx), "=&v"(bqy), "=&v"(bqz)
        : "v"(x), "v"(y), "v"(z), "s"(A.p0), "s"(A.p1), "s"(A.p2), "s"(A.p3), "s"(A.p4), "s"(A.p5), "s"(B.p0), "s"(B.p1), "s"(B.p2), "s"(B.p3),
          "s"(B.p4), "s"(B.p5));
    apx = ax; apy = ay; apz = az; bpx = bx; bpy = by; bpz = bz;
}
#endif

__device__ __forceinline__ void pcl_rotate2(f2 x, f2 y, f2 z, const PclPoseRec* __restrict__ pose, f2& opx, f2& opy, f2& opz)
{
    pcl_rotate2(x, y, z, pcl_pose6(pose), opx, opy, opz);
}

template <int FMT, bool DEPTH = false>
__device__ __forceinline__ void pcl_project2_rotated(__amdgpu_buffer_rsrc_t tex, const PclDims& dm, PclProj<FMT>& o,
                                                     __amdgpu_buffer_rsrc_t zb = __amdgpu_buffer_rsrc_t(), int zoff = 0,
                                                     const PclDepthGrid* dg = nullptr);

template <int FMT, bool DEPTH = false>
__device__ __forceinline__ void pcl_project2(f2 x, f2 y, f2 z, const PclPose6& pose,
                                             __amdgpu_buffer_rsrc_t tex, const PclDims& dm, PclProj<FMT>& o,
                                             __amdgpu_buffer_rsrc_t zb = __amdgpu_buffer_rsrc_t(), int zoff = 0, const PclDepthGrid* dg = nullptr)
{
    pcl_rotate2(x, y, z, pose, o.px, o.py, o.pz);
    pcl_project2_rotated<FMT, DEPTH>(tex, dm, o, zb, zoff, dg);
}

__device__ __forceinline__ void pcl_angles2(f2 px, f2 py, f2 pz, f2& rho2, f2& rinv, f2& rs2, f2& phi, f2& half_el)
{
    f2 a = px + F2(1e-6f), b = pz + F2(1e-6f);
    rho2 = pcl_fma2(px, px, py * py);
    f2 rg = rho2 + F2(1e-37f);
    rinv = (f2){__builtin_amdgcn_rsqf(rg.x), __builtin_amdgcn_rsqf(rg.y)};
    f2 rho = rho2 * rinv;
    phi = pcl_atan2_2(py, a);
    f2 s2 = pcl_fma2(b, b, rho2) + F2(1e-37f);
    rs2 = (f2){__builtin_amdgcn_rsqf(s2.x), __builtin_amdgcn_rsqf(s2.y)};
    f2 den = pcl_fma2(s2, rs2, rho);
    half_el = pcl_atan_poly2(b * (f2){__builtin_amdgcn_rcpf(den.x), __builtin_amdgcn_rcpf(den.y)});
}

template <int FMT, bool DEPTH>
__device__ __forceinline__ void pcl_project2_rotated(__amdgpu_buffer_rsrc_t tex, const PclDims& dm, PclProj<FMT>& o, __amdgpu_buffer_rsrc_t zb,
                                                     int zoff, const PclDepthGrid* dg)
{
    f2 phi, half_el;
    pcl_angles2(o.px, o.py, o.pz, o.rho2, o.rinv, o.rs2, phi, half_el);
    if constexpr (DEPTH) {
        int r0, c0, r1, c1;
        pcl_depth_cells2(phi, half_el, *dg, r0, c0, r1, c1);
        o.zq0 = (unsigned)__builtin_amdgcn_raw_buffer_load_b32(zb, (int)(__umul24((unsigned)r0, (unsigned)dg->Wd) + (unsigned)c0) * 4, zoff, 0);
        o.zq1 = (unsigned)__builtin_amdgcn_raw_buffer_load_b32(zb, (int)(__umul24((unsigned)r1, (unsigned)dg->Wd) + (unsigned)c1) * 4, zoff, 0);
    }
    const float lim_phi = 0.99f * 3.14159265358979323846f, lim_hel = 0.2475f * 3.14159265358979323846f;
    f2 phic = {__builtin_amdgcn_fmed3f(phi.x, -lim_phi, lim_phi), __builtin_amdgcn_fmed3f(phi.y, -lim_phi, lim_phi)};
    f2 helc = {__builtin_amdgcn_fmed3f(half_el.x, -lim_hel, lim_hel), __builtin_amdgcn_fmed3f(half_el.y, -lim_hel, lim_hel)};
    f2 ix = pcl_fma2(phic, F2(dm.k_ix), F2(dm.off_x));
    f2 iy = pcl_fma2(helc, F2(2.f * dm.k_iy), F2(dm.off_y));
    pcl_issue_taps(tex, (int)ix.x, (int)iy.x, dm.Wp, o.ta);
    pcl_issue_taps(tex, (int)ix.y, (int)iy.y, dm.Wp, o.tb);
    o.fx = (f2){__builtin_amdgcn_fractf(ix.x), __builtin_amdgcn_fractf(ix.y)};
    o.fy = (f2){__builtin_amdgcn_fractf(iy.x), __builtin_amdgcn_fractf(iy.y)};
    o.in_phi0 = phi.x == phic.x; o.in_phi1 = phi.y == phic.y;
    o.in_th0 = half_el.x == helc.x; o.in_th1 = half_el.y == helc.y;
}

template <bool GRAD, int FMT>
__device__ __forceinline__ void pcl_sample2(const PclProj<FMT>& o, f2 ncr, f2 ncg, f2 ncb, bool valid0, bool valid1,
                                            unsigned long long vmask0, unsigned long long vmask1,
                                            __amdgpu_buffer_rsrc_t tex, const PclDims& dm, f2* acc, int& count)
{
    const f2 px = o.px, py = o.py, pz = o.pz, fx = o.fx, fy = o.fy;
    f2 c[3], dv[3], dtop[3], dbot[3], dhp[3];
    if constexpr (FMT == PCL_PANO_F16) {
        PclBilerp1 ba, bb;
        pcl_bilerp_f16<GRAD>(o.ta, fx.x, fy.x, ba);
        pcl_bilerp_f16<GRAD>(o.tb, fx.y, fy.y, bb);
#pragma unroll
        for (int k = 0; k < 3; k++) {
            f2 top = {ba.top[k], bb.top[k]};
            dv[k] = (f2){ba.bot[k], bb.bot[k]} - top;
            c[k] = pcl_fma2(fy, dv[k], top);
            if (GRAD) dhp[k] = (f2){ba.dh[k], bb.dh[k]};
        }
    } else {
        float ta[12], tb[12];
        pcl_unpack_taps(tex, o.ta, ta);
        pcl_unpack_taps(tex, o.tb, tb);
#pragma unroll
        for (int k = 0; k < 3; k++) {
            f2 t00 = {ta[k], tb[k]}, t01 = {ta[3 + k], tb[3 + k]}, t10 = {ta[6 + k], tb[6 + k]}, t11 = {ta[9 + k], tb[9 + k]};
            dtop[k] = t01 - t00;
            dbot[k] = t11 - t10;
            f2 top = pcl_fma2(fx, dtop[k], t00), bot = pcl_fma2(fx, dbot[k], t10);
            dv[k] = bot - top;
            c[k] = pcl_fma2(fy, dv[k], top);
        }
    }
    float m0 = fmaxf(fmaxf(fabsf(c[0].x), fabsf(c[1].x)), fabsf(c[2].x));
    float m1 = fmaxf(fmaxf(fabsf(c[0].y), fabsf(c[1].y)), fabsf(c[2].y));
    bool keep0 = valid0 && m0 > 0.f, keep1 = valid1 && m1 > 0.f;
    count += __builtin_popcountll(__builtin_amdgcn_fcmpf(m0, 0.f, 2) & vmask0) +
             __builtin_popcountll(__builtin_amdgcn_fcmpf(m1, 0.f, 2) & vmask1);
    f2 d0, d1, d2;
    if (FMT != PCL_PANO_F32) {
        d0 = pcl_fma2(c[0], F2(dm.c_scale), ncr); d1 = pcl_fma2(c[1], F2(dm.c_scale), ncg); d2 = pcl_fma2(c[2], F2(dm.c_scale), ncb);
    } else {
        d0 = c[0] + ncr; d1 = c[1] + ncg; d2 = c[2] + ncb;
    }
    f2 n2 = pcl_fma2(d0, d0, pcl_fma2(d1, d1, d2 * d2));
    f2 ng = n2 + F2(1e-37f);
    f2 rn = {keep0 ? __builtin_amdgcn_rsqf(ng.x) : 0.f, keep1 ? __builtin_amdgcn_rsqf(ng.y) : 0.f};
    acc[0] = pcl_fma2(n2, rn, acc[0]);
    if (GRAD) {
        f2 dh0, dh1, dh2;
        if constexpr (FMT == PCL_PANO_F16) { dh0 = dhp[0]; dh1 = dhp[1]; dh2 = dhp[2]; }
        else {
            dh0 = pcl_fma2(fy, dbot[0] - dtop[0], dtop[0]);
            dh1 = pcl_fma2(fy, dbot[1] - dtop[1], dtop[1]);
            dh2 = pcl_fma2(fy, dbot[2] - dtop[2], dtop[2]);
        }
        f2 sx = pcl_fma2(d0, dh0, pcl_fma2(d1, dh1, d2 * dh2));
        f2 sy = pcl_fma2(d0, dv[0], pcl_fma2(d1, dv[1], d2 * dv[2]));
        f2 rphi = {o.in_phi0 ? rn.x : 0.f, o.in_phi1 ? rn.y : 0.f}, rth = {o.in_th0 ? rn.x : 0.f, o.in_th1 ? rn.y : 0.f};
        f2 dphi = (sx * F2(dm.k_phi)) * rphi, dth = (sy * F2(dm.k_theta)) * rth;
        f2 a = px + F2(1e-6f), b = pz + F2(1e-6f), rho = o.rho2 * o.rinv;
        f2 s1 = pcl_fma2(a, a, py * py);
        f2 ai = dphi * (f2){__builtin_amdgcn_rcpf(s1.x), __builtin_amdgcn_rcpf(s1.y)};
        f2 bi = dth * (o.rs2 * o.rs2);
        f2 k = b * bi * o.rinv;
        f2 g0 = pcl_fma2(k, px, -(py * ai));
        f2 g1 = pcl_fma2(k, py, a * ai);
        f2 g2 = -(rho * bi);
        acc[2] += g0; acc[3] += g1; acc[4] += g2;
        acc[5] = pcl_fma2(py, g2, pcl_fma2(-pz, g1, acc[5]));
        acc[6] = pcl_fma2(pz, g0, pcl_fma2(-px, g2, acc[6]));
        acc[7] = pcl_fma2(px, g1, pcl_fma2(-py, g0, acc[7]));
    }
}
```

### piccolo_amd/omniloc.py

```python
import weakref
from collections import OrderedDict

import torch
import torch.nn as nn

from . import ops

strict_reference_asserts = True

_CAPACITY = {"cloud": 2, "order": 2, "box": 8, "grid": 4, "pano": 16, "pano_u8": 16, "pano_u8p": 16, "pano_u8v": 16, "gd": 6, "gd_rooms": 4, "trimgroups": 4}


class _PackCache:
    def __init__(self):
        self.kinds = {}

    def _lru(self, kind):
        lru = self.kinds.get(kind)
        if lru is None:
            lru = self.kinds[kind] = OrderedDict()
        return lru

    def get(self, kind, key, tensors):
        lru = self._lru(kind)
        hit = lru.get(key)
        if hit is not None and all(r() is t for r, t in zip(hit[0], tensors)):
            lru.move_to_end(key)
            return hit[1]
        return None

    def put(self, kind, key, tensors, obj):
        lru = self._lru(kind)
        for k in [k for k, (refs, _) in lru.items() if any(r() is None for r in refs)]:
            del lru[k]
        lru[key] = ([weakref.ref(t) for t in tensors], obj)
        lru.move_to_end(key)
        while len(lru) > _CAPACITY.get(kind, 4):
            lru.popitem(last=False)

    def clear(self):
        self.kinds.clear()

    def __len__(self):
        return sum(len(v) for v in self.kinds.values())


_cache = _PackCache()


def _key(*tensors):
    return tuple((t.data_ptr(), tuple(t.shape), t._version, str(t.device), t.dtype) for t in tensors)


def _cached(kind, tensors, make, sub=None):
    k = (sub,) + _key(*tensors)
    obj = _cache.get(kind, k, tensors)
    if obj is None:
        obj = make()
        _cache.put(kind, k, tensors, obj)
    return obj


def quantile_box_of(xyz, out_quantile):
    return _cached("box", (xyz,), lambda: ops.quantile_box(xyz, out_quantile), sub=float(out_quantile))


def packed_cloud(xyz, rgb):
    def make():
        order = _cache.get("order", (None,) + _key(xyz), (xyz,))
        if order is not None:
            return ops.Cloud(xyz, rgb, order=order)
        c = ops.Cloud(xyz, rgb)
        if c.order is not None:
            _cache.put("order", (None,) + _key(xyz), (xyz,), c.order)
        return c
    return _cached("cloud", (xyz, rgb), make)


def packed_cloud_sets(xyz, rgbs):
    def make():
        order = _cache.get("order", (None,) + _key(xyz), (xyz,))
        if order is not None:
            return ops.Cloud.with_color_sets(xyz, rgbs, order=order)
        c = ops.Cloud.with_color_sets(xyz, rgbs)
        if c.order is not None:
            _cache.put("order", (None,) + _key(xyz), (xyz,), c.order)
        return c
    return _cached("cloud", (xyz,) + tuple(rgbs), make)


def color_set_groups(n, I, cap=None):
    cap = max(1, min(ops.max_color_sets(n), ops.TRIM_MAX_IMAGES, ops.HIST_MAX_IMAGES, cap if cap is not None else I))
    return [min(cap, I - i0) for i0 in range(0, I, cap)]


def shared_rgb(rgb):
    if isinstance(rgb, (list, tuple)):
        if len(rgb) == 0:
            raise ValueError("rgb: an empty list of colour sets")
        if all(r is rgb[0] for r in rgb):
            return rgb[0]
        return list(rgb)
    return rgb


def packed_pano(img, many_poses=False, n_points=None):
    rgba8 = many_poses or (n_points is not None and ops.refine_texels(n_points, img.shape[0], img.shape[1]) == "u8")
    if ops.EXPERIMENT.pano_fmt in ("f16", "f32") and not many_poses:
        rgba8 = False
    if not rgba8:
        return _cached("pano", (img,), lambda: ops.Pano(img))
    fmt = ops.trim_texels(n_points, img.shape[0], img.shape[1]) if many_poses and n_points is not None else "u8"
    if ops.EXPERIMENT.trim_fmt in ("u8", "u8p", "u8v") and many_poses:
        fmt = ops.EXPERIMENT.trim_fmt

    def make():
        try:
            return ops.Pano(img, fmt=fmt)
        except ValueError:
            return ops.Pano(img, fmt="f32")
    return _cached("pano_" + fmt, (img,), make)


def _cfg(cfg, key, default):
    return getattr(cfg, key, default)


def _rot_matrix(ypr):
    return ops.rot_from_ypr(ypr.reshape(1, 3))[0]


GRAPH_POINT_POSES = 16_000_000


def _refine(xyz, rgb, panos, trans, rot, box, cfg, batch_mode, vis_hook=None):
    cloud = packed_cloud_sets(xyz, rgb) if isinstance(rgb, list) else packed_cloud(xyz, rgb)
    trans, rot = ops._dev(trans).reshape(-1, 3), ops._dev(rot).reshape(-1, 3)
    B = int(trans.shape[0])
    p0 = panos[0]
    num_iter = _cfg(cfg, "num_iter", 100)
    depth = bool(_cfg(cfg, "depth_mask", False))
    d_tau, d_res, d_st = _cfg(cfg, "depth_tau", None), _cfg(cfg, "depth_res", None), _cfg(cfg, "depth_stride", None)
    hyper = (float(_cfg(cfg, "lr", 0.1)), int(_cfg(cfg, "patience", 5)), float(_cfg(cfg, "factor", 0.9)), bool(batch_mode), depth,
             None if d_tau is None else float(d_tau), None if d_res is None else (int(d_res[0]), int(d_res[1])), None if d_st is None else int(d_st))
    use_graph = _cfg(cfg, "gd_graph", None)
    if use_graph is None and ops.EXPERIMENT.gd_graph is not None:
        use_graph = bool(ops.EXPERIMENT.gd_graph)
    fuse = None if _cfg(cfg, "gd_fuse", True) else False
    if use_graph is None:
        use_graph = cloud.n * B <= GRAPH_POINT_POSES
    use_graph = bool(use_graph) and vis_hook is None and not depth

    def make(c=cloud, bx=box):
        return ops.GradientDescent(c, p0, trans, rot, bx, lr=hyper[0], patience=hyper[1], factor=hyper[2], batch_mode=hyper[3],
                                   depth_mask=hyper[4], depth_tau=hyper[5], depth_res=hyper[6], depth_stride=hyper[7], fuse=fuse)
    if not use_graph:
        gd = make()
    else:
        def make_private():
            g = make(ops.Cloud.private_copy(cloud), ops._dev(box).reshape(6).clone())
            g._cloud_src = weakref.ref(cloud)
            g._box_src, g._fresh = box, True
            return g
        gd = _cached("gd", (xyz,), make_private, sub=(B, len(panos), p0.H, p0.W, p0.fmt, fuse, cloud.color_sets) + hyper)
        fresh, gd._fresh = gd._fresh, False
        if gd._cloud_src() is not cloud:
            gd.cloud.data.copy_(cloud.data)
            gd._cloud_src = weakref.ref(cloud)
        if gd._box_src is not box:
            gd.box.copy_(ops._dev(box).reshape(6))
            gd._box_src = box
        if not fresh:
            gd.reset(trans, rot)
    if len(panos) > 1 or use_graph:
        gd.set_pano_groups(list(panos))
    if vis_hook is not None:
        vis_hook(gd, num_iter)
    elif use_graph:
        gd.run_graph(num_iter)
    else:
        gd.run(num_iter)
    return gd


def _leaf_buffers(input_trans, input_rot, B):
    def usable(t):
        return torch.is_tensor(t) and t.is_cuda and t.dtype == torch.float32 and t.is_contiguous() and t.numel() == 3 * B and not t.requires_grad
    bt = input_trans if usable(input_trans) else torch.empty(B, 3, dtype=torch.float32, device=ops.device())
    br = input_rot if usable(input_rot) else torch.empty(B, 3, dtype=torch.float32, device=ops.device())

    def after():
        with torch.no_grad():
            if bt is not input_trans:
                input_trans.copy_(bt.reshape(input_trans.shape).to(input_trans.device))
            if br is not input_rot:
                input_rot.copy_(br.reshape(input_rot.shape).to(input_rot.device))
    return bt, br, after


def omniloc(img, xyz, rgb, input_trans, input_rot, starting_point, cfg, scalar_summaries):
    vis = _cfg(cfg, "visualize", False)
    out_quantile = _cfg(cfg, "out_of_room_quantile", 0.05)

    pano = packed_pano(img, n_points=xyz.shape[0])
    box = quantile_box_of(xyz, out_quantile)
    frames = []
    hook = (lambda gd, n: frames.extend(_run_with_frames(gd, img, xyz, rgb, n))) if vis else None
    res = _refine(xyz, rgb, [pano], input_trans[starting_point], input_rot[starting_point], box, cfg, False, vis_hook=hook).result()[0]
    R = _rot_matrix(res[3:6])
    out = torch.cat([res[0:3], R.reshape(-1), res[12:13]]).cpu()
    with torch.no_grad():
        input_trans[starting_point] = res[6:9].to(input_trans.device)
        input_rot[starting_point] = res[9:12].to(input_rot.device)
    ret = [out[0:3].reshape(3, 1).clone(), out[3:12].reshape(3, 3).clone(), out[12].clone()]
    if vis:
        ret.append(frames)
    return ret


def _run_with_frames(gd, img, xyz, rgb, num_iter):
    import numpy as np
    from PIL import Image
    h, w = int(img.shape[0]) // 2, int(img.shape[1]) // 2
    gt_img = Image.fromarray(np.uint8(ops._dev(img).cpu().numpy() * 255), "RGB").resize((w, h))
    frames, new_frame = [], None
    for it in range(num_iter):
        pose = gd.result()[0]
        gd.run(1)
        cur = ops.make_pano(ops.transform_cloud(xyz, pose[0:3], pose[3:6]), rgb, (h, w)).cpu().numpy().astype(np.uint8)
        new_frame = Image.new("RGB", (w, 2 * h))
        new_frame.paste(gt_img, (0, 0))
        new_frame.paste(Image.fromarray(cur), (0, h))
        frames.extend([new_frame] * (5 if it == 0 else 1))
    if new_frame is not None:
        last_frame = Image.new("RGB", (w, 2 * h))
        last_frame.paste(gt_img, (0, 0))
        frames.extend([new_frame] * 10 + [last_frame] * 5)
    return frames


def omniloc_all(img, xyz, rgb, input_trans, input_rot, cfg, scalar_summaries=None):
    box = quantile_box_of(xyz, _cfg(cfg, "out_of_room_quantile", 0.05))
    res = _refine(xyz, rgb, [packed_pano(img, n_points=xyz.shape[0])], input_trans, input_rot, box, cfg, False).result()
    K = res.shape[0]
    R = ops.rot_from_ypr(res[:, 3:6])
    host = torch.cat([res[:, 0:3], R.reshape(K, 9), res[:, 12:13]], dim=1).cpu()
    with torch.no_grad():
        input_trans.copy_(res[:, 6:9].to(input_trans.device))
        input_rot.copy_(res[:, 9:12].to(input_rot.device))
    return [[host[i, 0:3].reshape(3, 1).clone(), host[i, 3:12].reshape(3, 3).clone(), host[i, 12].clone()] for i in range(K)]


def omniloc_batch(img, xyz, rgb, input_trans, input_rot, cfg, scalar_summaries):
    if strict_reference_asserts:
        assert cfg.num_input > 1
    box = quantile_box_of(xyz, _cfg(cfg, "out_of_room_quantile", 0.05))
    gd = _refine(xyz, rgb, [packed_pano(img, n_points=xyz.shape[0])], input_trans, input_rot, box, cfg, True)
    bt, br, after = _leaf_buffers(input_trans, input_rot, gd.B)
    out = gd.winner(1, bt, br)[0].cpu()
    after()
    return [out[0:3].reshape(3, 1).clone(), out[3:12].reshape(3, 3).clone(), out[12].clone()]


def omniloc_batch_images(imgs, xyz, rgb, input_trans_list, input_rot_list, cfg, scalar_summaries=None, batch_mode=True):
    if strict_reference_asserts and batch_mode:
        assert cfg.num_input > 1
    I = len(imgs)
    rgb = shared_rgb(rgb)
    if isinstance(rgb, list):
        if len(rgb) != I:
            raise ValueError("omniloc_batch_images: %d colour sets for %d images" % (len(rgb), I))
        sizes = [1] * I if bool(_cfg(cfg, "depth_mask", False)) else color_set_groups(int(xyz.shape[0]), I)
        if len(sizes) > 1:
            out, i0 = [], 0
            for m in sizes:
                out += omniloc_batch_images(imgs[i0:i0 + m], xyz, rgb[i0:i0 + m] if m > 1 else rgb[i0], input_trans_list[i0:i0 + m],
                                            input_rot_list[i0:i0 + m], cfg, scalar_summaries, batch_mode)
                i0 += m
            return out
    B = int(input_trans_list[0].shape[0])
    fmt = ops.refine_texels(xyz.shape[0], imgs[0].shape[0], imgs[0].shape[1])
    panos = [packed_pano(im, n_points=xyz.shape[0]) if I <= 8 else ops.Pano(im, fmt=fmt if ops._known_levels(im) else "auto") for im in imgs]
    if len({p.fmt for p in panos}) > 1:
        panos = [ops.Pano(im, fmt="f32") for im in imgs]
    box = quantile_box_of(xyz, _cfg(cfg, "out_of_room_quantile", 0.05))
    tr = torch.cat([ops._dev(t).reshape(B, 3) for t in input_trans_list])
    ro = torch.cat([ops._dev(r).reshape(B, 3) for r in input_rot_list])
    gd = _refine(xyz, rgb, panos, tr, ro, box, cfg, batch_mode)
    leaf_t, leaf_r = torch.empty(I * B, 3, dtype=torch.float32, device=tr.device), torch.empty(I * B, 3, dtype=torch.float32, device=tr.device)
    host = gd.winner(I, leaf_t, leaf_r).cpu()
    with torch.no_grad():
        for i in range(I):
            input_trans_list[i].copy_(leaf_t[i * B:(i + 1) * B].to(input_trans_list[i].device))
            input_rot_list[i].copy_(leaf_r[i * B:(i + 1) * B].to(input_rot_list[i].device))
    return [[host[i, 0:3].reshape(3, 1).clone(), host[i, 3:12].reshape(3, 3).clone(), host[i, 12].clone()] for i in range(I)]


def _rooms_chain(img, rooms, tr, ro, cfg, batch_mode):
    clouds = [packed_cloud(xyz, rgb) for xyz, rgb in rooms]
    boxes = [quantile_box_of(xyz, _cfg(cfg, "out_of_room_quantile", 0.05)) for xyz, _ in rooms]
    B = int(tr.shape[0])
    per_room = B // len(rooms)
    pano = packed_pano(img, n_points=max(int(xyz.shape[0]) for xyz, _ in rooms))
    num_iter = _cfg(cfg, "num_iter", 100)
    hyper = (float(_cfg(cfg, "lr", 0.1)), int(_cfg(cfg, "patience", 5)), float(_cfg(cfg, "factor", 0.9)), bool(batch_mode))
    fuse = None if _cfg(cfg, "gd_fuse", True) else False
    use_graph = _cfg(cfg, "gd_graph", None)
    if use_graph is None and ops.EXPERIMENT.gd_graph is not None:
        use_graph = bool(ops.EXPERIMENT.gd_graph)
    if use_graph is None:
        use_graph = sum(c.n for c in clouds) * per_room <= GRAPH_POINT_POSES

    def make(cs, bs):
        return ops.GradientDescentRooms(list(zip(cs, bs)), pano, tr, ro, lr=hyper[0], patience=hyper[1], factor=hyper[2], batch_mode=hyper[3],
                                        fuse=fuse)
    if not use_graph:
        gd = make(clouds, boxes)
        gd.run(num_iter)
        return gd

    def make_private():
        g = make([ops.Cloud.private_copy(c) for c in clouds], [ops._dev(b).reshape(6).clone() for b in boxes])
        g._cloud_src = [weakref.ref(c) for c in clouds]
        g._box_src, g._fresh = list(boxes), True
        return g
    xyzs = tuple(xyz for xyz, _ in rooms)
    gd = _cached("gd_rooms", xyzs, make_private, sub=(per_room, pano.H, pano.W, pano.fmt, fuse) + hyper)
    fresh, gd._fresh = gd._fresh, False
    for r, c in enumerate(clouds):
        if gd._cloud_src[r]() is not c:
            gd.clouds[r].data.copy_(c.data)
            gd._cloud_src[r] = weakref.ref(c)
        if gd._box_src[r] is not boxes[r]:
            gd.boxes[r].copy_(ops._dev(boxes[r]).reshape(6))
            gd._box_src[r] = boxes[r]
    if not fresh:
        gd.reset(tr, ro)
    ops.GradientDescent.set_pano_groups(gd, [pano])
    gd.run_graph(num_iter)
    return gd


def omniloc_batch_rooms(img, rooms, input_trans_list, input_rot_list, cfg, scalar_summaries=None, batch_mode=True):
    if strict_reference_asserts and batch_mode:
        assert cfg.num_input > 1
    R = len(rooms)
    if R == 0 or len(input_trans_list) != R or len(input_rot_list) != R:
        raise ValueError("omniloc_batch_rooms: %d rooms, %d / %d starting-pose sets" % (R, len(input_trans_list), len(input_rot_list)))
    B = int(input_trans_list[0].shape[0])
    if any(int(t.shape[0]) != B for t in input_trans_list) or any(int(r.shape[0]) != B for r in input_rot_list):
        raise ValueError("omniloc_batch_rooms: every room needs the same number of starting poses")
    if bool(_cfg(cfg, "depth_mask", False)):
        return [omniloc_batch_images([img], xyz, rgb, [input_trans_list[r]], [input_rot_list[r]], cfg, scalar_summaries, batch_mode)[0]
                for r, (xyz, rgb) in enumerate(rooms)]
    if R == 1:
        xyz, rgb = rooms[0]
        if batch_mode:
            return [omniloc_batch(img, xyz, rgb, input_trans_list[0], input_rot_list[0], cfg, scalar_summaries)]
        return omniloc_batch_images([img], xyz, rgb, [input_trans_list[0]], [input_rot_list[0]], cfg, scalar_summaries, batch_mode=False)
    cap = ops._lib.GD_MAX_ROOMS
    if R > cap:
        out = []
        for r0 in range(0, R, cap):
            out += omniloc_batch_rooms(img, rooms[r0:r0 + cap], input_trans_list[r0:r0 + cap], input_rot_list[r0:r0 + cap], cfg, scalar_summaries,
                                       batch_mode)
        return out
    tr = torch.cat([ops._dev(t).reshape(B, 3) for t in input_trans_list])
    ro = torch.cat([ops._dev(r).reshape(B, 3) for r in input_rot_list])
    gd = _rooms_chain(img, rooms, tr, ro, cfg, batch_mode)
    leaf_t, leaf_r = torch.empty(R * B, 3, dtype=torch.float32, device=tr.device), torch.empty(R * B, 3, dtype=torch.float32, device=tr.device)
    host = gd.winner(leaf_t, leaf_r).cpu()
    with torch.no_grad():
        for r in range(R):
            input_trans_list[r].copy_(leaf_t[r * B:(r + 1) * B].reshape(input_trans_list[r].shape).to(input_trans_list[r].device))
            input_rot_list[r].copy_(leaf_r[r * B:(r + 1) * B].reshape(input_rot_list[r].shape).to(input_rot_list[r].device))
    return [[host[r, 0:3].reshape(3, 1).clone(), host[r, 3:12].reshape(3, 3).clone(), host[r, 12].clone()] for r in range(R)]


def sampling_loss(img, xyz, rgb, input_trans, input_rot, starting_point, cfg, return_list=True):
    cloud, pano = packed_cloud(xyz, rgb), packed_pano(img)
    t, r = input_trans[starting_point], input_rot[starting_point]
    res = ops.sampling_loss(cloud, pano, t, r, with_grad=False, depth=_depth_cfg(cfg))[0]
    loss = res[0].cpu()
    if return_list:
        return [t.detach().reshape(3, 1).cpu().clone(), _rot_matrix(ops._dev(r)).cpu(), loss]
    return loss


def _depth_cfg(cfg):
    if not bool(_cfg(cfg, "depth_mask", False)):
        return None
    return {"depth_res": _cfg(cfg, "depth_res", None), "depth_tau": _cfg(cfg, "depth_tau", None), "depth_stride": _cfg(cfg, "depth_stride", None),
            "on": True}


class _LossFn(torch.autograd.Function):

    @staticmethod
    def forward(ctx, cloud, pano, trans, rot, depth=None):
        res = ops.sampling_loss(cloud, pano, trans, rot, with_grad=True, depth=depth)
        ctx.save_for_backward(res[:, 2:5], res[:, 5:8])
        ctx.devs = (trans.device, rot.device)
        return res[:, 0].to(trans.device)

    @staticmethod
    def backward(ctx, grad_loss):
        gt, gr = ctx.saved_tensors
        g = grad_loss.to(gt.device).reshape(-1, 1)
        return None, None, (g * gt).to(ctx.devs[0]), (g * gr).to(ctx.devs[1]), None


class SamplingLoss(nn.Module):

    def __init__(self, xyz, rgb, img, device, cfg):
        super().__init__()
        self.xyz, self.rgb, self.img, self.cfg = xyz, rgb, img, cfg
        self._cloud, self._pano = ops.Cloud(xyz, rgb), ops.Pano(img)

    def forward(self, translation, yaw, pitch, roll):
        trans = translation.reshape(1, 3)
        rot = torch.cat([yaw.reshape(1), pitch.reshape(1), roll.reshape(1)]).reshape(1, 3)
        return _LossFn.apply(self._cloud, self._pano, trans, rot, _depth_cfg(self.cfg))[0]


class BatchSamplingLoss(nn.Module):

    def __init__(self, xyz, rgb, img, device, cfg):
        super().__init__()
        self.xyz, self.rgb, self.img, self.cfg = xyz, rgb, img, cfg
        self.num_input = cfg.num_input
        self._cloud, self._pano = ops.Cloud(xyz, rgb), ops.Pano(img)

    def forward(self, translation, yaw, pitch, roll):
        B = translation.shape[0]
        if B != self.num_input:
            raise RuntimeError("BatchSamplingLoss: batch size %d != cfg.num_input %d" % (B, self.num_input))
        trans = translation.reshape(B, 3)
        rot = torch.cat([yaw.reshape(B, 1), pitch.reshape(B, 1), roll.reshape(B, 1)], dim=1)
        loss_list = _LossFn.apply(self._cloud, self._pano, trans, rot, _depth_cfg(self.cfg))
        return loss_list.sum(), loss_list
```

### piccolo_amd/ops.py

```python
import ctypes

import torch

from . import _lib


class _Experiment:
    pano_fmt = None
    trim_fmt = None
    gd_graph = None
    verify_levels = False


EXPERIMENT = _Experiment()

F32 = torch.float32


_GPU_SEEN = False


def device():
    global _GPU_SEEN
    if not _GPU_SEEN:
        if not torch.cuda.is_available():
            raise _lib.PiccoloHipError("piccolo_amd needs an MI355X (torch.cuda.is_available() is False); there is no CPU path")
        _GPU_SEEN = True
    return torch.device("cuda", torch.cuda.current_device())


def _dev(t, dtype=F32):
    if torch.is_tensor(t) and t.is_cuda and t.dtype == dtype and not t.requires_grad and t.is_contiguous() and t.device.index == torch.cuda.current_device():
        return t
    if not torch.is_tensor(t):
        t = torch.as_tensor(t)
    return t.detach().to(device=device(), dtype=dtype).contiguous()


def _ptr(t):
    return ctypes.c_void_p(t.data_ptr()) if t is not None else None


def _stream():
    return ctypes.c_void_p(torch.cuda.current_stream().cuda_stream)


def _bytes(nbytes):
    return torch.empty(max(int(nbytes), 16), dtype=torch.uint8, device=device())


class Cloud:

    color_sets = 1

    def __init__(self, xyz, rgb, sort=True, order=None):
        lib = _lib.load()
        xyz, rgb = _dev(xyz), _dev(rgb)
        if xyz.dim() != 2 or xyz.shape[1] != 3 or rgb.shape != xyz.shape:
            raise ValueError("xyz and rgb must both be (N, 3)")
        self.n = int(xyz.shape[0])
        if self.n <= 0:
            raise ValueError("empty point cloud")
        self.order = None
        if order is not None:
            if order.dtype != torch.int64 or order.numel() != self.n or not order.is_cuda:
                raise ValueError("order must be a CUDA int64 tensor with one entry per point")
            self.order = order
        elif sort and self.n > 1:
            self.order = torch.empty(self.n, dtype=torch.int64, device=xyz.device)
            nws = lib.pcl_cloud_order_workspace_bytes(self.n)
            ws = _bytes(nws)
            _lib.check(lib.pcl_cloud_order(_ptr(xyz), self.n, _ptr(self.order), _ptr(ws), nws, _stream()), "pcl_cloud_order")
        self.data = _bytes(lib.pcl_cloud_bytes(self.n))
        _lib.check(lib.pcl_cloud_pack(_ptr(xyz), _ptr(rgb), _ptr(self.order), self.n, _ptr(self.data), _stream()),
                   "pcl_cloud_pack")
        self.xyz = xyz

    @classmethod
    def private_copy(cls, other):
        c = cls.__new__(cls)
        c.n, c.order, c.xyz = other.n, other.order, other.xyz
        c.color_sets = other.color_sets
        c.data = other.data.clone()
        return c

    @classmethod
    def with_color_sets(cls, xyz, rgbs, order=None, sort=True):
        lib = _lib.load()
        xyz = _dev(xyz)
        rgbs = [_dev(r) for r in rgbs]
        if xyz.dim() != 2 or xyz.shape[1] != 3 or not rgbs or any(r.shape != xyz.shape for r in rgbs):
            raise ValueError("xyz and every rgb must be (N, 3)")
        c = cls.__new__(cls)
        c.n = int(xyz.shape[0])
        if c.n <= 0:
            raise ValueError("empty point cloud")
        nbytes = lib.pcl_cloud_sets_bytes(c.n, len(rgbs))
        if nbytes == 0:
            raise ValueError("%d colour sets of %d points exceed the cloud's 32-bit addressing (at most %d)" % (len(rgbs), c.n, max_color_sets(c.n)))
        c.order = None
        if order is not None:
            if order.dtype != torch.int64 or order.numel() != c.n or not order.is_cuda:
                raise ValueError("order must be a CUDA int64 tensor with one entry per point")
            c.order = order
        elif sort and c.n > 1:
            c.order = torch.empty(c.n, dtype=torch.int64, device=xyz.device)
            nws = lib.pcl_cloud_order_workspace_bytes(c.n)
            ws = _bytes(nws)
            _lib.check(lib.pcl_cloud_order(_ptr(xyz), c.n, _ptr(c.order), _ptr(ws), nws, _stream()), "pcl_cloud_order")
        c.color_sets = len(rgbs)
        c.data = _bytes(nbytes)
        arr = (ctypes.c_void_p * len(rgbs))(*[r.data_ptr() for r in rgbs])
        _lib.check(lib.pcl_cloud_pack_sets(_ptr(xyz), arr, len(rgbs), _ptr(c.order), c.n, _ptr(c.data), _stream()), "pcl_cloud_pack_sets")
        c.xyz = xyz
        return c


def max_color_sets(n):
    lib = _lib.load()
    if lib.pcl_cloud_sets_bytes(n, 1) == 0:
        return 0
    plane = 4 * lib.pcl_cloud_stride(n)
    k = max(1, ((1 << 31) - 1) // plane // 3 - 1)
    while k > 1 and lib.pcl_cloud_sets_bytes(n, k) == 0:
        k -= 1
    return k


class Pano:

    _PACK = {"f16": ("pcl_pano_pack_f16", _lib.PANO_F16), "u8": ("pcl_pano_pack_u8", _lib.PANO_U8),
             "u8p": ("pcl_pano_pack_u8p", _lib.PANO_U8P),
             "u8v": ("pcl_pano_pack_u8v", _lib.PANO_U8V)}

    def __init__(self, img, fmt="auto"):
        lib = _lib.load()
        src = img
        img = _dev(img)
        if img.dim() != 3 or img.shape[2] != 3:
            raise ValueError("img must be (H, W, 3)")
        self.H, self.W = int(img.shape[0]), int(img.shape[1])
        self.fmt = None
        if fmt not in ("auto", "f16", "u8", "u8p", "u8v", "f32"):
            raise ValueError("unknown texel format %r" % (fmt,))
        prefer = "f16"
        if fmt == "auto":
            prefer = EXPERIMENT.pano_fmt or "f16"
            if prefer == "f32":
                fmt = "f32"
        if fmt != "f32":
            fn, code = self._PACK[prefer if fmt == "auto" else fmt]
            data = _bytes(lib.pcl_pano_bytes(self.H, self.W, code))
            known = _known_levels(src)
            flag = _scratch_flag(img.device) if known else torch.zeros(1, dtype=torch.int32, device=img.device)
            _lib.check(getattr(lib, fn)(_ptr(img), self.H, self.W, _ptr(data), _ptr(flag), _stream()), fn)
            if known or int(flag.item()) == 0:
                self.fmt, self.data = code, data
            elif fmt != "auto":
                raise ValueError("image is not exactly k/255: cannot use %s texels" % fmt)
        if self.fmt is None:
            self.fmt = _lib.PANO_F32
            self.data = _bytes(lib.pcl_pano_bytes(self.H, self.W, _lib.PANO_F32))
            _lib.check(lib.pcl_pano_pack(_ptr(img), self.H, self.W, _ptr(self.data), _stream()), "pcl_pano_pack")


_SCRATCH_FLAGS = {}


def _scratch_flag(dev):
    f = _SCRATCH_FLAGS.get(dev)
    if f is None:
        f = _SCRATCH_FLAGS[dev] = torch.zeros(1, dtype=torch.int32, device=dev)
    return f


def refine_texels(n, H, W):
    return "u8" if 20 * int(n) < 9 * int(H) * int(W) else "f16"


def trim_texels(n, H, W):
    n, px = int(n), int(H) * int(W)
    doubled = 8 * (int(H) + 2) * (int(W) + 2)
    if doubled <= 6_000_000:
        return "u8v"
    if doubled <= 24_000_000:
        return "u8p" if 3 * n < px else "u8v" if 12 * n >= 5 * px else "u8"
    return "u8p" if 20 * n < 9 * px else "u8v" if 5 * n >= 3 * px else "u8"


def trim_order_pays(n, H, W, fmt):
    doubled = 8 * (int(H) + 2) * (int(W) + 2)
    return doubled <= 24_000_000


def _known_levels(img):
    tag = getattr(img, "_pcl_levels", None)
    return tag is not None and torch.is_tensor(img) and tag == img._version and not EXPERIMENT.verify_levels


def default_depth(n, H, W, stride=0):
    dh, dw, tau, st = ctypes.c_int(0), ctypes.c_int(0), ctypes.c_float(0), ctypes.c_int(0)
    _lib.check(_lib.load().pcl_depth_default(int(n), int(H), int(W), int(stride), ctypes.byref(dh), ctypes.byref(dw), ctypes.byref(tau),
                                             ctypes.byref(st)), "pcl_depth_default")
    return dh.value, dw.value, tau.value, st.value


def default_depth_res(n, H, W, stride=0):
    return default_depth(n, H, W, stride)[:2]


def depth_tau_rule(depth_h):
    return min(max(3.5 * 3.141592653589793 / max(int(depth_h), 1), 0.02), 0.15)


def _depth_args(n, H, W, depth_res, depth_tau, depth_stride=None):
    if depth_res is None:
        dh, dw, tau, st = default_depth(n, H, W, int(depth_stride or 0))
    else:
        dh, dw = int(depth_res[0]), int(depth_res[1])
        tau, st = depth_tau_rule(dh), int(depth_stride or 1)
    if depth_tau is not None:
        tau = float(depth_tau)
    return dh, dw, float(tau), st


def sampling_loss(cloud, pano, trans, rot, with_grad=True, visible=None, depth=None):
    lib = _lib.load()
    trans, rot = _dev(trans).reshape(-1, 3), _dev(rot).reshape(-1, 3)
    B = int(trans.shape[0])
    if rot.shape[0] != B:
        raise ValueError("trans and rot must have the same number of rows")
    out = torch.empty(B, _lib.RESULT_STRIDE, dtype=F32, device=trans.device)
    if depth:
        if visible is not None:
            raise ValueError("sampling_loss: pass either a byte mask (visible) or depth, not both")
        d = depth if isinstance(depth, dict) else {}
        dh, dw, tau, st = _depth_args(cloud.n, pano.H, pano.W, d.get("depth_res"), d.get("depth_tau"), d.get("depth_stride"))
        ws_bytes = lib.pcl_loss_depth_workspace_bytes(cloud.n, B, pano.H, pano.W, dh, dw, st)
        if ws_bytes == 0:
            raise _lib.PiccoloHipError("pcl_loss_depth_workspace_bytes: invalid depth grid %dx%d" % (dh, dw))
        ws = _bytes(ws_bytes)
        _lib.check(lib.pcl_sampling_loss_depth(_ptr(cloud.data), cloud.n, _ptr(pano.data), pano.fmt, pano.H, pano.W, _ptr(trans), _ptr(rot), B,
                                               1 if with_grad else 0, dh, dw, tau, st, _ptr(out), _ptr(ws), ws_bytes, _stream()),
                   "pcl_sampling_loss_depth")
        return out
    ws_bytes = lib.pcl_loss_workspace_bytes(cloud.n, B)
    ws = _bytes(ws_bytes)
    vis = None
    if visible is not None:
        vis = _dev(visible, torch.uint8).reshape(B, cloud.n)
    _lib.check(lib.pcl_sampling_loss(_ptr(cloud.data), cloud.n, _ptr(pano.data), pano.fmt, pano.H, pano.W, _ptr(trans), _ptr(rot), B,
                                     1 if with_grad else 0, _ptr(vis), _ptr(out), _ptr(ws), ws_bytes, _stream()),
               "pcl_sampling_loss")
    return out


TRIM_MAX_ROT = 1024


class TrimGroups:

    def __init__(self, rot):
        lib = _lib.load()
        self.rot = _dev(rot).reshape(-1, 3)
        self.R = int(self.rot.shape[0])
        if self.R <= 0:
            raise ValueError("empty rotation table")
        self.data = _bytes(lib.pcl_trim_groups_bytes(self.R))
        _lib.check(lib.pcl_trim_groups(_ptr(self.rot), self.R, _ptr(self.data), _stream()), "pcl_trim_groups")
        self.ngroups = int(self.data[:4].view(torch.int32).item())


class TrimOrder:

    def __init__(self, cloud, pano_shape, trans, groups):
        lib = _lib.load()
        trans = _dev(trans).reshape(-1, 3)
        H, W, fmt = pano_shape
        self.key = (cloud.n, int(trans.shape[0]), groups.ngroups, int(H), int(W), int(fmt))
        self.data = _bytes(lib.pcl_trim_order_bytes(cloud.n, self.key[1], groups.ngroups))
        nws = lib.pcl_trim_order_workspace_bytes(cloud.n, self.key[1], groups.ngroups)
        ws = _bytes(nws)
        _lib.check(lib.pcl_trim_order(_ptr(cloud.data), cloud.n, int(fmt), int(H), int(W), _ptr(trans), self.key[1], _ptr(groups.rot), groups.R,
                                      _ptr(groups.data), groups.ngroups, _ptr(self.data), _ptr(ws), nws, _stream()), "pcl_trim_order")


def trim_loss_table(cloud, pano, trans, groups, return_count=False, order=None):
    lib = _lib.load()
    trans = _dev(trans).reshape(-1, 3)
    K = int(trans.shape[0])
    table = torch.empty(K, groups.R, dtype=F32, device=trans.device)
    count = torch.empty(K, groups.R, dtype=F32, device=trans.device) if return_count else None
    nws = lib.pcl_trim_loss_workspace_bytes(cloud.n, K, groups.ngroups)
    ws = _bytes(nws)
    _lib.check(lib.pcl_trim_loss(_ptr(cloud.data), cloud.n, _ptr(pano.data), pano.fmt, pano.H, pano.W, _ptr(trans), K, _ptr(groups.rot),
                                 groups.R, _ptr(groups.data), groups.ngroups, _ptr(order.data) if order is not None else None, _ptr(table), _ptr(count),
                                 _ptr(ws), nws, _stream()),
               "pcl_trim_loss")
    return (table, count) if return_count else table


TRIM_MAX_IMAGES = 32


def trim_loss_tables(cloud, panos, trans, groups, return_count=False, order=None):
    lib = _lib.load()
    trans = _dev(trans).reshape(-1, 3)
    K, I = int(trans.shape[0]), len(panos)
    p0 = panos[0]
    if any((p.H, p.W, p.fmt) != (p0.H, p0.W, p0.fmt) for p in panos):
        raise ValueError("all panoramas of a launch must share size and texel format")
    if cloud.color_sets > 1:
        if cloud.color_sets != I:
            raise ValueError("a cloud of %d colour sets for %d images" % (cloud.color_sets, I))
        if I > TRIM_MAX_IMAGES:
            raise ValueError("trim_loss_tables: at most %d images per call with colour sets" % TRIM_MAX_IMAGES)
        table = torch.empty(I, K, groups.R, dtype=F32, device=trans.device)
        count = torch.empty(I, K, groups.R, dtype=F32, device=trans.device) if return_count else None
        nws = lib.pcl_trim_loss_images_workspace_bytes(cloud.n, K, groups.ngroups, I)
        ws = _bytes(nws)
        arr = (ctypes.c_void_p * I)(*[p.data.data_ptr() for p in panos])
        _lib.check(lib.pcl_trim_loss_images_sets(_ptr(cloud.data), cloud.n, I, arr, I, p0.fmt, p0.H, p0.W, _ptr(trans), K, _ptr(groups.rot),
                                                 groups.R, _ptr(groups.data), groups.ngroups, _ptr(order.data) if order is not None else None,
                                                 _ptr(table), _ptr(count), _ptr(ws), nws, _stream()), "pcl_trim_loss_images_sets")
        return (table, count) if return_count else table
    table = torch.empty(I, K, groups.R, dtype=F32, device=trans.device)
    count = torch.empty(I, K, groups.R, dtype=F32, device=trans.device) if return_count else None
    for i0 in range(0, I, TRIM_MAX_IMAGES):
        part = panos[i0:i0 + TRIM_MAX_IMAGES]
        nws = lib.pcl_trim_loss_images_workspace_bytes(cloud.n, K, groups.ngroups, len(part))
        ws = _bytes(nws)
        arr = (ctypes.c_void_p * len(part))(*[p.data.data_ptr() for p in part])
        _lib.check(lib.pcl_trim_loss_images(_ptr(cloud.data), cloud.n, arr, len(part), p0.fmt, p0.H, p0.W, _ptr(trans), K, _ptr(groups.rot),
                                            groups.R, _ptr(groups.data), groups.ngroups, _ptr(order.data) if order is not None else None, _ptr(table[i0:]),
                                            _ptr(count[i0:]) if return_count else None, _ptr(ws), nws, _stream()), "pcl_trim_loss_images")
    return (table, count) if return_count else table


def select_poses(values, n_keep, trans, rot, largest=False, rot_per_trans=0, return_idx=False):
    lib = _lib.load()
    values = _dev(values)
    single = values.dim() == 1
    v = values.reshape(1, -1) if single else values.reshape(values.shape[0], -1)
    P, M = int(v.shape[0]), int(v.shape[1])
    trans, rot = _dev(trans), _dev(rot)
    stride = 0
    if trans.dim() == 3:
        if rot.dim() != 3 or trans.shape[0] != P or rot.shape[:2] != trans.shape[:2]:
            raise ValueError("select_poses: per-problem pose tables must be (P, rows, 3) for both trans and rot")
        stride = int(trans.shape[1])
    trans, rot = trans.reshape(-1, 3), rot.reshape(-1, 3)
    rows_t = trans.shape[0] if stride == 0 else stride
    rows_r = rot.shape[0] if stride == 0 else stride
    need_t = (M + rot_per_trans - 1) // rot_per_trans if rot_per_trans > 0 else M
    need_r = rot_per_trans if rot_per_trans > 0 else M
    if rows_t < need_t or rows_r < need_r:
        raise ValueError("select_poses: %d values need %d translations and %d rotations" % (M, need_t, need_r))
    n_keep = int(n_keep)
    ot = torch.empty(P, n_keep, 3, dtype=F32, device=v.device)
    orr = torch.empty(P, n_keep, 3, dtype=F32, device=v.device)
    oi = torch.empty(P, n_keep, dtype=torch.int32, device=v.device) if return_idx else None
    _lib.check(lib.pcl_select_poses(_ptr(v), P, M, n_keep, 1 if largest else 0, _ptr(trans), _ptr(rot), int(rot_per_trans), stride,
                                    _ptr(ot), _ptr(orr), _ptr(oi), _stream()), "pcl_select_poses")
    if single:
        ot, orr, oi = ot[0], orr[0], (oi[0] if oi is not None else None)
    return (ot, orr, oi) if return_idx else (ot, orr)


SELECT_MAX_KEEP = 1024


def hist_trim_scores(img, cloud, trans, rot, num_split_h, num_split_w, batch=64, return_parts=False, splat=False):
    lib = _lib.load()
    img = _dev(img)
    trans, rot = _dev(trans).reshape(-1, 3), _dev(rot).reshape(-1, 3)
    K, (H, W) = int(trans.shape[0]), (int(img.shape[0]), int(img.shape[1]))
    if splat:
        size_of = lambda b: lib.pcl_hist_trim_workspace_bytes(b, H, W, num_split_h, num_split_w)
    else:
        size_of = lambda b: lib.pcl_hist_trim_workspace_bytes_n(cloud.n, b, H, W, num_split_h, num_split_w)
    nblk = (num_split_h - 2) * num_split_w
    inter = torch.empty(K, nblk, dtype=F32, device=img.device)
    nproj = torch.empty(K, nblk, dtype=torch.int32, device=img.device)
    nimg = torch.empty(nblk, dtype=torch.int32, device=img.device)
    per_cand = max(size_of(1), 1)
    batch = max(1, min(batch, K, int(HIST_BATCH_BYTES // per_cand)))
    if size_of(batch) == 0:
        raise ValueError("hist_trim_scores: need num_split_h >= 3 and blocks of at least one pixel")
    ws = None
    while ws is None:
        nws = size_of(batch)
        try:
            ws = _bytes(nws)
        except torch.cuda.OutOfMemoryError:
            torch.cuda.empty_cache()
            if batch > 1:
                batch = (batch + 1) // 2
                continue
            nws = lib.pcl_hist_trim_workspace_bytes(1, H, W, num_split_h, num_split_w)
            ws = _bytes(nws)
    for k0 in range(0, K, batch):
        k1 = min(k0 + batch, K)
        _lib.check(lib.pcl_hist_trim_scores(_ptr(cloud.data), cloud.n, _ptr(img), H, W, _ptr(trans[k0:k1]),
                                            _ptr(rot[k0:k1]), k1 - k0, num_split_h, num_split_w, _ptr(inter[k0:k1]),
                                            _ptr(nproj[k0:k1]), _ptr(nimg), _ptr(ws), nws, _stream()), "pcl_hist_trim_scores")
    scores = torch.empty(K, dtype=F32, device=img.device)
    _lib.check(lib.pcl_hist_trim_reduce(_ptr(inter), _ptr(nproj), _ptr(nimg), K, num_split_h, num_split_w, _ptr(scores), _stream()),
               "pcl_hist_trim_reduce")
    if return_parts:
        return scores, inter, nproj, nimg
    return scores


HIST_MAX_IMAGES = 32
HIST_BATCH_BYTES = 8e9


def hist_trim_scores_images(imgs, cloud, trans, rot, num_split_h, num_split_w, splat=False):
    if cloud.color_sets > 1:
        return _hist_trim_scores_sets(imgs, cloud, trans, rot, num_split_h, num_split_w, splat)
    lib = _lib.load()
    imgs = [_dev(im) for im in imgs]
    trans, rot = _dev(trans), _dev(rot)
    I, K = int(trans.shape[0]), int(trans.shape[1])
    H, W = int(imgs[0].shape[0]), int(imgs[0].shape[1])
    if len(imgs) != I or any(tuple(im.shape) != (H, W, 3) or not im.is_contiguous() for im in imgs):
        raise ValueError("hist_trim_scores_images: one contiguous (H, W, 3) image per row of candidates, all of one size")
    nblk = (num_split_h - 2) * num_split_w
    dev = imgs[0].device
    inter = torch.empty(I * K, nblk, dtype=F32, device=dev)
    nproj = torch.empty(I * K, nblk, dtype=torch.int32, device=dev)
    nimg = torch.empty(I, nblk, dtype=torch.int32, device=dev)
    scores = torch.empty(I, K, dtype=F32, device=dev)
    if splat:
        size_of = lambda m: lib.pcl_hist_trim_images_sets_workspace_bytes(0, 1, m, K, H, W, num_split_h, num_split_w)
    else:
        size_of = lambda m: lib.pcl_hist_trim_images_workspace_bytes(cloud.n, m, K, H, W, num_split_h, num_split_w)
    per_image = size_of(1)
    if per_image == 0:
        raise ValueError("hist_trim_scores_images: need num_split_h >= 3 and blocks of at least one pixel")
    group = max(1, min(HIST_MAX_IMAGES, I, int(HIST_BATCH_BYTES // per_image)))
    t2, r2 = trans.reshape(I * K, 3).contiguous(), rot.reshape(I * K, 3).contiguous()
    i0 = 0
    while i0 < I:
        m = min(group, I - i0)
        nws = size_of(m)
        try:
            ws = _bytes(nws)
        except torch.cuda.OutOfMemoryError:
            torch.cuda.empty_cache()
            if group > 1:
                group = (group + 1) // 2
                continue
            scores[i0] = hist_trim_scores(imgs[i0], cloud, trans[i0], rot[i0], num_split_h, num_split_w, splat=splat)
            i0 += 1
            continue
        arr = (ctypes.c_void_p * m)(*[im.data_ptr() for im in imgs[i0:i0 + m]])
        _lib.check(lib.pcl_hist_trim_scores_images(_ptr(cloud.data), cloud.n, arr, m, K, H, W, _ptr(t2[i0 * K:]), _ptr(r2[i0 * K:]), num_split_h,
                                                   num_split_w, _ptr(inter[i0 * K:]), _ptr(nproj[i0 * K:]), _ptr(nimg[i0:]), _ptr(ws), nws, _stream()),
                   "pcl_hist_trim_scores_images")
        _lib.check(lib.pcl_hist_trim_reduce_images(_ptr(inter[i0 * K:]), _ptr(nproj[i0 * K:]), _ptr(nimg[i0:]), m, K, num_split_h, num_split_w,
                                                   _ptr(scores[i0:]), _stream()), "pcl_hist_trim_reduce_images")
        i0 += m
    return scores


def _hist_trim_scores_sets(imgs, cloud, trans, rot, num_split_h, num_split_w, splat):
    lib = _lib.load()
    imgs = [_dev(im) for im in imgs]
    trans, rot = _dev(trans), _dev(rot)
    I, K = int(trans.shape[0]), int(trans.shape[1])
    H, W = int(imgs[0].shape[0]), int(imgs[0].shape[1])
    if len(imgs) != I or any(tuple(im.shape) != (H, W, 3) or not im.is_contiguous() for im in imgs):
        raise ValueError("hist_trim_scores_images: one contiguous (H, W, 3) image per row of candidates, all of one size")
    if cloud.color_sets != I or I > HIST_MAX_IMAGES:
        raise ValueError("a cloud of %d colour sets for %d images (at most %d per call)" % (cloud.color_sets, I, HIST_MAX_IMAGES))
    nblk = (num_split_h - 2) * num_split_w
    dev = imgs[0].device
    inter = torch.empty(I * K, nblk, dtype=F32, device=dev)
    nproj = torch.empty(I * K, nblk, dtype=torch.int32, device=dev)
    nimg = torch.empty(I, nblk, dtype=torch.int32, device=dev)
    scores = torch.empty(I, K, dtype=F32, device=dev)
    nws = lib.pcl_hist_trim_images_sets_workspace_bytes(0 if splat else cloud.n, I, I, K, H, W, num_split_h, num_split_w)
    if nws == 0:
        raise ValueError("hist_trim_scores_images: need num_split_h >= 3 and blocks of at least one pixel")
    try:
        ws = _bytes(nws)
    except torch.cuda.OutOfMemoryError:
        torch.cuda.empty_cache()
        nws = lib.pcl_hist_trim_images_sets_workspace_bytes(0, I, I, K, H, W, num_split_h, num_split_w)
        ws = _bytes(nws)
    t2, r2 = trans.reshape(I * K, 3).contiguous(), rot.reshape(I * K, 3).contiguous()
    arr = (ctypes.c_void_p * I)(*[im.data_ptr() for im in imgs])
    _lib.check(lib.pcl_hist_trim_scores_images_sets(_ptr(cloud.data), cloud.n, I, arr, I, K, H, W, _ptr(t2), _ptr(r2), num_split_h, num_split_w,
                                                    _ptr(inter), _ptr(nproj), _ptr(nimg), _ptr(ws), nws, _stream()), "pcl_hist_trim_scores_images_sets")
    _lib.check(lib.pcl_hist_trim_reduce_images(_ptr(inter), _ptr(nproj), _ptr(nimg), I, K, num_split_h, num_split_w, _ptr(scores), _stream()),
               "pcl_hist_trim_reduce_images")
    return scores


def depth_mask(cloud, trans, rot, resolution, tau=None, stride=1):
    lib = _lib.load()
    trans, rot = _dev(trans).reshape(-1, 3), _dev(rot).reshape(-1, 3)
    B, (H, W) = int(trans.shape[0]), (int(resolution[0]), int(resolution[1]))
    if tau is None:
        tau = depth_tau_rule(H)
    vis = torch.empty(B, cloud.n, dtype=torch.uint8, device=trans.device)
    nws = lib.pcl_depth_workspace_bytes(B, H, W)
    ws = _bytes(nws)
    _lib.check(lib.pcl_depth_mask(_ptr(cloud.data), cloud.n, _ptr(trans), _ptr(rot), B, H, W, float(tau), int(stride), _ptr(vis), _ptr(ws), nws,
                                  _stream()), "pcl_depth_mask")
    return vis


class ColorTemplate:

    def __init__(self, rgb):
        lib = _lib.load()
        rgb = _dev(rgb).reshape(-1, 3)
        self.n = int(rgb.shape[0])
        self.data = torch.empty(3, self.n, dtype=F32, device=rgb.device)
        nws = lib.pcl_color_template_workspace_bytes(self.n)
        ws = _bytes(nws)
        _lib.check(lib.pcl_color_template_build(_ptr(rgb), self.n, _ptr(self.data), _ptr(ws), nws, _stream()),
                   "pcl_color_template_build")


def color_match(img, template):
    lib = _lib.load()
    known = _known_levels(img)
    img = _dev(img)
    H, W = int(img.shape[0]), int(img.shape[1])
    out = torch.empty_like(img)
    flag = torch.zeros(1, dtype=torch.int32, device=img.device)
    nws = lib.pcl_color_workspace_bytes()
    ws = _bytes(nws)
    _lib.check(lib.pcl_color_match(_ptr(img), H, W, _ptr(template.data), template.n, _ptr(out), _ptr(flag), _ptr(ws), nws,
                                   _stream()), "pcl_color_match")
    if not known and int(flag.item()):
        raise ValueError("color_match: the panorama must hold levels k/255 (an image file's uint8 / 255); "
                         "found a non-black pixel channel in between")
    return out


def color_mod(img, rgb, num_bins=256):
    lib = _lib.load()
    img, rgb = _dev(img), _dev(rgb).reshape(-1, 3)
    H, W = int(img.shape[0]), int(img.shape[1])
    out_img, out_rgb = torch.empty_like(img), torch.empty_like(rgb)
    nws = lib.pcl_color_workspace_bytes()
    ws = _bytes(nws)
    _lib.check(lib.pcl_color_mod(_ptr(img), H, W, _ptr(rgb), int(rgb.shape[0]), int(num_bins), _ptr(out_img), _ptr(out_rgb),
                                 _ptr(ws), nws, _stream()), "pcl_color_mod")
    return out_img, out_rgb


def histogram(img, mask, channels, normalize=True, eps=0.0):
    lib = _lib.load()
    img = _dev(img).reshape(-1, 3)
    mask = _dev(mask != 0, torch.uint8).reshape(-1)
    c0, c1, c2 = (int(c) for c in channels)
    nws = lib.pcl_histogram_workspace_bytes(c0, c1, c2)
    if nws == 0:
        raise ValueError("histogram: bad bin counts %r" % (channels,))
    ws = _bytes(nws)
    hist = torch.empty(c0 * c1 * c2, dtype=F32, device=img.device)
    _lib.check(lib.pcl_histogram(_ptr(img), _ptr(mask), int(img.shape[0]), c0, c1, c2, int(bool(normalize)), float(eps),
                                 _ptr(hist), _ptr(ws), nws, _stream()), "pcl_histogram")
    return hist


def histogram_intersection(h1, h2):
    lib = _lib.load()
    h1, h2 = _dev(h1), _dev(h2)
    B, nbins = int(h1.shape[0]), int(h1.shape[1])
    out = torch.empty(B, dtype=F32, device=h1.device)
    _lib.check(lib.pcl_histogram_intersection(_ptr(h1), _ptr(h2), B, nbins, _ptr(out), _stream()), "pcl_histogram_intersection")
    return out


def quantile_box(xyz, q):
    lib = _lib.load()
    xyz = _dev(xyz)
    box = torch.empty(6, dtype=F32, device=xyz.device)
    ws = _bytes(lib.pcl_quantile_workspace_bytes())
    _lib.check(lib.pcl_quantile_box(_ptr(xyz), int(xyz.shape[0]), float(q), _ptr(box), _ptr(ws), _stream()), "pcl_quantile_box")
    return box


class GradientDescent:

    def __init__(self, cloud, pano, trans, rot, box, lr=0.1, patience=5, factor=0.9, batch_mode=True, depth_mask=False,
                 depth_tau=None, depth_res=None, depth_stride=None, fuse=None):
        lib = _lib.load()
        self.cloud, self.pano = cloud, pano
        trans, rot = _dev(trans).reshape(-1, 3), _dev(rot).reshape(-1, 3)
        self.B = int(trans.shape[0])
        self.box = _dev(box).reshape(6)
        dh, dw, tau, st = _depth_args(cloud.n, pano.H, pano.W, depth_res, depth_tau, depth_stride) if depth_mask else (0, 0, 0.0, 0)
        self.hyper = _lib.GdHyper(float(lr), float(factor), int(patience), _lib.GD_BATCH if batch_mode else _lib.GD_SEQUENTIAL,
                                  1 if depth_mask else 0, float(tau), int(dh), int(dw), int(st), -1 if fuse is False else 0, 0)
        self.hyper.color_sets = int(cloud.color_sets)
        if cloud.color_sets > 1 and (self.B % cloud.color_sets or depth_mask):
            raise ValueError("GradientDescent: %d candidates over %d colour sets%s" % (self.B, cloud.color_sets, " with the depth mask" if depth_mask else ""))
        self.state = _bytes(lib.pcl_gd_state_bytes(self.B))
        self.ws_bytes = lib.pcl_gd_workspace_bytes(cloud.n, self.B, pano.H, pano.W, ctypes.byref(self.hyper))
        if self.ws_bytes == 0:
            raise _lib.PiccoloHipError("pcl_gd_workspace_bytes: invalid arguments (depth grid %dx%d?)" % (dh, dw))
        self.ws = _bytes(self.ws_bytes)
        _lib.check(lib.pcl_gd_init(_ptr(self.state), _ptr(trans), _ptr(rot), self.B, ctypes.byref(self.hyper), _stream()),
                   "pcl_gd_init")

    def run(self, num_iter, history=False, timer=None):
        lib = _lib.load()
        hist = torch.empty(num_iter, self.B, dtype=F32, device=self.state.device) if history else None
        _lib.check(lib.pcl_gd_run(_ptr(self.cloud.data), self.cloud.n, _ptr(self.pano.data), self.pano.fmt, self.pano.H, self.pano.W,
                                  _ptr(self.state), self.B, _ptr(self.box), ctypes.byref(self.hyper), int(num_iter),
                                  _ptr(hist), _ptr(self.ws), self.ws_bytes, timer.handle if timer else None, _stream()),
                   "pcl_gd_run")
        return hist

    def run_graph(self, num_iter):
        cache = self.__dict__.setdefault("_graphs", {})
        g = cache.get(num_iter)
        if g is None:
            g = torch.cuda.CUDAGraph()
            side = torch.cuda.Stream(device=self.state.device)
            side.wait_stream(torch.cuda.current_stream())
            with torch.cuda.stream(side):
                with torch.cuda.graph(g, stream=side):
                    self.run(num_iter)
            torch.cuda.current_stream().wait_stream(side)
            cache[num_iter] = g
        g.replay()

    def reset(self, trans, rot):
        lib = _lib.load()
        trans, rot = _dev(trans).reshape(-1, 3), _dev(rot).reshape(-1, 3)
        assert trans.shape[0] == self.B
        _lib.check(lib.pcl_gd_init(_ptr(self.state), _ptr(trans), _ptr(rot), self.B, ctypes.byref(self.hyper), _stream()),
                   "pcl_gd_init")

    def set_panos(self, panos):
        lib = _lib.load()
        assert len(panos) == self.B
        for p in panos:
            if (p.H, p.W, p.fmt) != (self.pano.H, self.pano.W, self.pano.fmt):
                raise ValueError("all panoramas of a launch must share size and texel format")
        self._panos = list(panos)
        self.set_pano_table(torch.tensor([p.data.data_ptr() for p in panos], dtype=torch.int64, device=self.state.device),
                            images=len({id(p) for p in panos}))

    def set_pano_table(self, table, images=0):
        self.hyper.images = int(images)
        assert table.dtype == torch.int64 and table.numel() == self.B and table.is_cuda
        _lib.check(_lib.load().pcl_gd_set_panos(_ptr(self.state), _ptr(table), self.B, _stream()), "pcl_gd_set_panos")
        self._pano_table = table

    def set_pano_groups(self, panos):
        lib = _lib.load()
        I = len(panos)
        if I <= 0 or self.B % I:
            raise ValueError("set_pano_groups: %d candidates do not split into %d images" % (self.B, I))
        for p in panos:
            if (p.H, p.W, p.fmt) != (self.pano.H, self.pano.W, self.pano.fmt):
                raise ValueError("all panoramas of a launch must share size and texel format")
        self._panos = list(panos)
        self.hyper.images = I
        arr = (ctypes.c_uint64 * I)(*[p.data.data_ptr() for p in panos])
        _lib.check(lib.pcl_gd_set_pano_groups(_ptr(self.state), arr, I, self.B // I, _stream()), "pcl_gd_set_pano_groups")

    def winner(self, nimages=1, leaf_trans=None, leaf_rot=None):
        lib = _lib.load()
        if nimages <= 0 or self.B % nimages:
            raise ValueError("winner: %d candidates do not split into %d images" % (self.B, nimages))
        out = torch.empty(nimages, 16, dtype=F32, device=self.state.device)
        for t in (leaf_trans, leaf_rot):
            if t is not None and not (t.is_cuda and t.dtype == F32 and t.is_contiguous() and t.numel() == 3 * self.B):
                raise ValueError("winner: leaf buffers must be contiguous float32 GPU tensors of B x 3")
        _lib.check(lib.pcl_gd_winner(_ptr(self.state), nimages, self.B // nimages, _ptr(out), _ptr(leaf_trans), _ptr(leaf_rot), _stream()),
                   "pcl_gd_winner")
        return out

    def step_from_grads(self, loss, grad):
        loss, grad = _dev(loss).reshape(self.B), _dev(grad).reshape(self.B, 6)
        scratch = torch.empty(self.B * 8, dtype=F32, device=self.state.device)
        _lib.check(_lib.load().pcl_gd_step_from_grads(_ptr(self.state), self.B, _ptr(loss), _ptr(grad), _ptr(self.box), ctypes.byref(self.hyper),
                                                      _ptr(scratch), _stream()), "pcl_gd_step_from_grads")

    def result(self):
        lib = _lib.load()
        out = torch.empty(self.B, _lib.GD_RESULT_STRIDE, dtype=F32, device=self.state.device)
        _lib.check(lib.pcl_gd_result(_ptr(self.state), self.B, _ptr(out), _stream()), "pcl_gd_result")
        return out


class GradientDescentRooms:

    def __init__(self, rooms, pano, trans, rot, lr=0.1, patience=5, factor=0.9, batch_mode=True, fuse=None):
        lib = _lib.load()
        if not 1 <= len(rooms) <= _lib.GD_MAX_ROOMS:
            raise ValueError("GradientDescentRooms: %d rooms (1..%d per chain)" % (len(rooms), _lib.GD_MAX_ROOMS))
        self.pano = pano
        self.clouds = [c for c, _ in rooms]
        for c in self.clouds:
            if c.color_sets > 1:
                raise ValueError("GradientDescentRooms: a room cloud with colour sets")
        self.boxes = [_dev(b).reshape(6) for _, b in rooms]
        trans, rot = _dev(trans).reshape(-1, 3), _dev(rot).reshape(-1, 3)
        self.nrooms = len(rooms)
        self.B = int(trans.shape[0])
        if self.B % self.nrooms or self.B == 0:
            raise ValueError("GradientDescentRooms: %d candidates do not split into %d rooms" % (self.B, self.nrooms))
        self.per_room = self.B // self.nrooms
        self.hyper = _lib.GdHyper(float(lr), float(factor), int(patience), _lib.GD_BATCH if batch_mode else _lib.GD_SEQUENTIAL,
                                  0, 0.0, 0, 0, 0, -1 if fuse is False else 0, 0, 0)
        self._rooms = (_lib.GdRoom * self.nrooms)(*[_lib.GdRoom(c.data.data_ptr(), c.n, b.data_ptr()) for c, b in zip(self.clouds, self.boxes)])
        self.state = _bytes(lib.pcl_gd_state_bytes(self.B))
        self.ws_bytes = lib.pcl_gd_rooms_workspace_bytes(self._rooms, self.nrooms, self.per_room, ctypes.byref(self.hyper))
        if self.ws_bytes == 0:
            raise _lib.PiccoloHipError("pcl_gd_rooms_workspace_bytes: invalid arguments")
        self.ws = _bytes(self.ws_bytes)
        _lib.check(lib.pcl_gd_init(_ptr(self.state), _ptr(trans), _ptr(rot), self.B, ctypes.byref(self.hyper), _stream()), "pcl_gd_init")

    def plan(self):
        nch, G, fused = (ctypes.c_int * self.nrooms)(), ctypes.c_int(0), ctypes.c_int(0)
        _lib.check(_lib.load().pcl_gd_plan_rooms(self._rooms, self.nrooms, self.per_room, ctypes.byref(self.hyper), nch, ctypes.byref(G),
                                                 ctypes.byref(fused)), "pcl_gd_plan_rooms")
        return list(nch), G.value, bool(fused.value)

    def run(self, num_iter, history=False, timer=None):
        lib = _lib.load()
        hist = torch.empty(num_iter, self.B, dtype=F32, device=self.state.device) if history else None
        _lib.check(lib.pcl_gd_run_rooms(self._rooms, self.nrooms, _ptr(self.pano.data), self.pano.fmt, self.pano.H, self.pano.W, _ptr(self.state),
                                        self.per_room, ctypes.byref(self.hyper), int(num_iter), _ptr(hist), _ptr(self.ws), self.ws_bytes,
                                        timer.handle if timer else None, _stream()), "pcl_gd_run_rooms")
        return hist

    run_graph = GradientDescent.run_graph

    def reset(self, trans, rot):
        trans, rot = _dev(trans).reshape(-1, 3), _dev(rot).reshape(-1, 3)
        assert trans.shape[0] == self.B
        _lib.check(_lib.load().pcl_gd_init(_ptr(self.state), _ptr(trans), _ptr(rot), self.B, ctypes.byref(self.hyper), _stream()), "pcl_gd_init")

    def winner(self, leaf_trans=None, leaf_rot=None):
        return GradientDescent.winner(self, self.nrooms, leaf_trans, leaf_rot)

    result = GradientDescent.result


class KernelTimer:

    def __init__(self, capacity, stride=1):
        self.handle = ctypes.c_void_p(_lib.load().pcl_timer_create(int(capacity)))
        if not self.handle:
            raise _lib.PiccoloHipError("pcl_timer_create failed")
        _lib.load().pcl_timer_set_stride(self.handle, int(stride))

    def reset(self):
        _lib.load().pcl_timer_reset(self.handle)

    def read(self):
        ms, cnt = ctypes.c_double(0), ctypes.c_int(0)
        _lib.check(_lib.load().pcl_timer_read(self.handle, ctypes.byref(ms), ctypes.byref(cnt)), "pcl_timer_read")
        return ms.value, cnt.value

    def calibrate(self, reps=64):
        ms = ctypes.c_double(0)
        _lib.check(_lib.load().pcl_timer_calibrate(self.handle, int(reps), ctypes.byref(ms), _stream()), "pcl_timer_calibrate")
        return ms.value

    def __del__(self):
        try:
            if self.handle:
                _lib.load().pcl_timer_destroy(self.handle)
                self.handle = None
        except Exception:
            pass


def cloud2idx(xyz):
    lib = _lib.load()
    x = _dev(xyz)
    shp = x.shape
    flat = x.reshape(-1, 3)
    out = torch.empty(flat.shape[0], 2, dtype=F32, device=x.device)
    if flat.shape[0]:
        _lib.check(lib.pcl_cloud2idx(_ptr(flat), int(flat.shape[0]), _ptr(out), _stream()), "pcl_cloud2idx")
    return out.reshape(shp[:-1] + (2,))


def sample_from_img(pano, coord):
    lib = _lib.load()
    c = _dev(coord)
    shp = c.shape
    flat = c.reshape(-1, 2)
    out = torch.empty(flat.shape[0], 3, dtype=F32, device=c.device)
    if flat.shape[0]:
        _lib.check(lib.pcl_sample_from_img(_ptr(pano.data), pano.fmt, pano.H, pano.W, _ptr(flat), int(flat.shape[0]), _ptr(out), _stream()),
                   "pcl_sample_from_img")
    return out.reshape(shp[:-1] + (3,))


def cloud2idx_backward(xyz, grad_coord):
    lib = _lib.load()
    x, g = _dev(xyz), _dev(grad_coord)
    flat, gflat = x.reshape(-1, 3), g.reshape(-1, 2)
    if gflat.shape[0] != flat.shape[0]:
        raise ValueError("grad_coord must have one (gx, gy) per point")
    out = torch.empty_like(flat)
    if flat.shape[0]:
        _lib.check(lib.pcl_cloud2idx_backward(_ptr(flat), _ptr(gflat), int(flat.shape[0]), _ptr(out), _stream()), "pcl_cloud2idx_backward")
    return out.reshape(x.shape)


def sample_from_img_backward(pano, coord, grad_rgb, want_coord=True, want_img=False):
    lib = _lib.load()
    c, g = _dev(coord), _dev(grad_rgb)
    flat, gflat = c.reshape(-1, 2), g.reshape(-1, 3)
    if gflat.shape[0] != flat.shape[0]:
        raise ValueError("grad_rgb must have one colour per coordinate")
    gc = torch.empty_like(flat) if want_coord else None
    gi = torch.zeros(pano.H, pano.W, 3, dtype=F32, device=c.device) if want_img else None
    if flat.shape[0] and (want_coord or want_img):
        _lib.check(lib.pcl_sample_from_img_backward(_ptr(pano.data), pano.fmt, pano.H, pano.W, _ptr(flat), _ptr(gflat), int(flat.shape[0]),
                                                    _ptr(gc), _ptr(gi), _stream()), "pcl_sample_from_img_backward")
    elif gc is not None:
        gc.zero_()
    return (gc.reshape(c.shape) if gc is not None else None), gi


def rot_from_ypr(rot):
    lib = _lib.load()
    r = _dev(rot).reshape(-1, 3)
    out = torch.empty(r.shape[0], 9, dtype=F32, device=r.device)
    _lib.check(lib.pcl_rot_from_ypr(_ptr(r), int(r.shape[0]), _ptr(out), _stream()), "pcl_rot_from_ypr")
    return out.reshape(-1, 3, 3)


def transform_cloud(xyz, trans, rot):
    lib = _lib.load()
    x = _dev(xyz)
    t, r = _dev(trans).reshape(3), _dev(rot).reshape(3)
    out = torch.empty_like(x)
    _lib.check(lib.pcl_transform_cloud(_ptr(x), int(x.shape[0]), _ptr(t), _ptr(r), _ptr(out), _stream()), "pcl_transform_cloud")
    return out


def make_pano(xyz_cam, rgb, resolution):
    lib = _lib.load()
    x, c = _dev(xyz_cam), _dev(rgb)
    H, W = int(resolution[0]), int(resolution[1])
    img = torch.empty(H, W, 3, dtype=F32, device=x.device)
    ws = _bytes(H * W * 8)
    _lib.check(lib.pcl_make_pano(_ptr(x), _ptr(c), int(x.shape[0]), H, W, _ptr(img), _ptr(ws), _stream()), "pcl_make_pano")
    return img


def scatter_min_depth(xyz_cam, resolution):
    lib = _lib.load()
    x = _dev(xyz_cam)
    H, W = int(resolution[0]), int(resolution[1])
    n = int(x.shape[0])
    zbuf = _bytes(H * W * 8)
    zmin = torch.empty(H * W, dtype=F32, device=x.device)
    arg = torch.empty(H * W, dtype=torch.int64, device=x.device)
    _lib.check(lib.pcl_scatter_min_depth(_ptr(x), n, H, W, _ptr(zbuf), _stream()), "pcl_scatter_min_depth")
    _lib.check(lib.pcl_scatter_min_unpack(_ptr(zbuf), n, H, W, _ptr(zmin), _ptr(arg), _stream()), "pcl_scatter_min_unpack")
    return zmin, arg
```

Baseline: 3522.

## Add F16 record panorama layout with precomputed blue delta for narrower taps

Adds a second copy of the f16 panorama laid out as records holding RGB of the texel plus the horizontal delta of the blue channel. The loss kernels read it with 96-bit buffer loads per row instead of 128-bit loads. This cuts texel fetch bandwidth and a few subtractions in bilinear sampling. The cost is roughly double the pano memory, an extra packing kernel, and new template instantiations throughout the loss and gradient-descent paths. It is enabled by default whenever the record buffer fits under 2 GiB.

Measured after the change: 3556 (median of 6 runs). About the same (+1.0%).

```diff
diff --git a/include/piccolo_hip.h b/include/piccolo_hip.h
--- a/include/piccolo_hip.h
+++ b/include/piccolo_hip.h
@@ -8,7 +8,7 @@
 extern "C" {
 #endif
 
-#define PCL_ABI_VERSION 11
+#define PCL_ABI_VERSION 12
 
 #define PCL_EINVAL (-1)
 #define PCL_EWORKSPACE (-2)
@@ -27,6 +27,9 @@
 #define PCL_PANO_F16 2
 #define PCL_PANO_U8P 3
 #define PCL_PANO_U8V 4
+#define PCL_PANO_F16R 5
+size_t pcl_pano_records_offset(int H, int W);
+int pcl_pano_f16_records(void *pano, int H, int W, void *stream);
 int64_t pcl_cloud_stride(int64_t n);
 size_t pcl_cloud_bytes(int64_t n);
 int pcl_cloud_pack(const float *xyz, const float *rgb, const int64_t *order, int64_t n, float *cloud, void *stream);
diff --git a/piccolo_amd/_lib.py b/piccolo_amd/_lib.py
--- a/piccolo_amd/_lib.py
+++ b/piccolo_amd/_lib.py
@@ -6,11 +6,11 @@
 _c = ctypes
 _vp, _i64, _int, _sz, _dbl = _c.c_void_p, _c.c_int64, _c.c_int, _c.c_size_t, _c.c_double
 
-ABI_VERSION = 11
+ABI_VERSION = 12
 RESULT_STRIDE = 8
 GD_RESULT_STRIDE = 16
 GD_SEQUENTIAL, GD_BATCH = 0, 1
-PANO_F32, PANO_U8, PANO_F16, PANO_U8P, PANO_U8V = 0, 1, 2, 3, 4
+PANO_F32, PANO_U8, PANO_F16, PANO_U8P, PANO_U8V, PANO_F16R = 0, 1, 2, 3, 4, 5
 
 
 class GdHyper(_c.Structure):
@@ -45,6 +45,8 @@
     "pcl_pano_pack_u8p": (_int, [_vp, _int, _int, _vp, _vp, _vp]),
     "pcl_pano_pack_u8v": (_int, [_vp, _int, _int, _vp, _vp, _vp]),
     "pcl_pano_pack_f16": (_int, [_vp, _int, _int, _vp, _vp, _vp]),
+    "pcl_pano_records_offset": (_sz, [_int, _int]),
+    "pcl_pano_f16_records": (_int, [_vp, _int, _int, _vp]),
     "pcl_loss_workspace_bytes": (_sz, [_i64, _int]),
     "pcl_sampling_loss": (_int, [_vp, _i64, _vp, _int, _int, _int, _vp, _vp, _int, _int, _vp, _vp, _vp, _sz, _vp]),
     "pcl_loss_depth_workspace_bytes": (_sz, [_i64, _int, _int, _int, _int, _int, _int]),
diff --git a/piccolo_amd/csrc/pcl_device.h b/piccolo_amd/csrc/pcl_device.h
--- a/piccolo_amd/csrc/pcl_device.h
+++ b/piccolo_amd/csrc/pcl_device.h
@@ -72,7 +72,7 @@
     d.c_scale = 1.0f;
     d.k_ix = (float)(-(double)W / (2.0 * 3.14159265358979323846));
     d.k_iy = (float)(-(double)H / 3.14159265358979323846);
-    if (pano_format == PCL_PANO_U8 || pano_format == PCL_PANO_F16) {
+    if (pano_format == PCL_PANO_U8 || pano_format == PCL_PANO_F16 || pano_format == PCL_PANO_F16R) {
         d.k_phi = (float)(-(double)W / (2.0 * 3.14159265358979323846) / 255.0);
         d.k_theta = (float)((double)H / 3.14159265358979323846 / 255.0);
         d.c_scale = (float)(1.0 / 255.0);
@@ -191,7 +191,9 @@
                                              0x00020000);
 }
 
-__host__ __device__ constexpr int pcl_texel_bytes(int fmt) { return fmt == PCL_PANO_U8 ? 4 : fmt == PCL_PANO_F16 ? 8 : 16; }
+__host__ __device__ constexpr int pcl_texel_bytes(int fmt) { return fmt == PCL_PANO_U8 ? 4 : fmt == PCL_PANO_F16 || fmt == PCL_PANO_F16R ? 8 : 16; }
+
+__host__ __device__ constexpr int64_t pcl_f16r_offset(int H, int W) { return ((int64_t)(H + 2) * (int64_t)(W + 2) * 8 + (1 << 21) - 1) >> 21 << 21; }
 
 __device__ inline pcl_i2 pcl_texel_pair_u8(__amdgpu_buffer_rsrc_t rsrc, int voff, int soff)
 {
diff --git a/piccolo_amd/csrc/pcl_loss.hip b/piccolo_amd/csrc/pcl_loss.hip
--- a/piccolo_amd/csrc/pcl_loss.hip
+++ b/piccolo_amd/csrc/pcl_loss.hip
@@ -97,7 +97,7 @@
 
     PclPose6 P6[G];
     unsigned PANO[G][2];
-    __amdgpu_buffer_rsrc_t tex = pcl_tex_rsrc(a.pano, a.dims.H, a.dims.W, pcl_texel_bytes(FMT));
+    __amdgpu_buffer_rsrc_t tex = pcl_sample_rsrc<FMT>(a.pano, a.dims);
     __amdgpu_buffer_rsrc_t cld = __builtin_amdgcn_make_buffer_rsrc((void*)a.cloud, 0, CS ? (int)(a.stride * (3 + 3 * a.color_sets) * 4) : (int)(a.stride * 6 * 4),
                                                                    0x00020000);
     const int plane = (int)a.stride * 4;
@@ -170,7 +170,7 @@
             }
             if (pano_lo | pano_hi) {
                 const void* pp = (const void*)(((unsigned long long)pano_hi << 32) | (unsigned long long)pano_lo);
-                tg = pcl_tex_rsrc(pp, a.dims.H, a.dims.W, pcl_texel_bytes(FMT));
+                tg = pcl_sample_rsrc<FMT>(pp, a.dims);
             }
             PclProj<FMT> pj;
             const int zoff = VIS == 2 ? (int)((unsigned)(pose0 + g) * (unsigned)(a.dgrid.last + 1) * 4u) : 0;
@@ -429,10 +429,12 @@
     }
 }
 
+static bool pcl_loss_format(int f) { return f == PCL_PANO_F32 || f == PCL_PANO_U8 || f == PCL_PANO_F16 || f == PCL_PANO_F16R; }
+
 int pcl_launch_loss_rooms(const PclRoomTable* rooms, const void* pano, int pano_format, int H, int W, const PclPoseRec* poses, int B, int G,
                           int ngroups, int nblk, float* partials, hipStream_t s, int flip, const PclFuseArgs* fuse)
 {
-    if (pano_format != PCL_PANO_F32 && pano_format != PCL_PANO_U8 && pano_format != PCL_PANO_F16) return PCL_EINVAL;
+    if (!pcl_loss_format(pano_format)) return PCL_EINVAL;
     if ((int64_t)(H + 2) * (W + 2) * pcl_texel_bytes(pano_format) >= ((int64_t)1 << 31)) return PCL_EINVAL;
     PclLossArgs a = PclLossArgs{};
     a.pano = pano; a.dims = pcl_make_dims(H, W, pano_format);
@@ -446,6 +448,9 @@
         } else if (pano_format == PCL_PANO_F16) {
             if (G == 2) hipLaunchKernelGGL((pcl_loss_fused_rooms_kernel<2, PCL_PANO_F16>), grid, blk, 0, s, a, *fuse, rooms);
             else hipLaunchKernelGGL((pcl_loss_fused_rooms_kernel<1, PCL_PANO_F16>), grid, blk, 0, s, a, *fuse, rooms);
+        } else if (pano_format == PCL_PANO_F16R) {
+            if (G == 2) hipLaunchKernelGGL((pcl_loss_fused_rooms_kernel<2, PCL_PANO_F16R>), grid, blk, 0, s, a, *fuse, rooms);
+            else hipLaunchKernelGGL((pcl_loss_fused_rooms_kernel<1, PCL_PANO_F16R>), grid, blk, 0, s, a, *fuse, rooms);
         } else {
             if (G == 2) hipLaunchKernelGGL((pcl_loss_fused_rooms_kernel<2, PCL_PANO_F32>), grid, blk, 0, s, a, *fuse, rooms);
             else hipLaunchKernelGGL((pcl_loss_fused_rooms_kernel<1, PCL_PANO_F32>), grid, blk, 0, s, a, *fuse, rooms);
@@ -457,6 +462,9 @@
         } else if (pano_format == PCL_PANO_F16) {
             if (G == 2) hipLaunchKernelGGL((pcl_loss_rooms_kernel<2, PCL_PANO_F16>), grid, blk, 0, s, a, rooms);
             else hipLaunchKernelGGL((pcl_loss_rooms_kernel<1, PCL_PANO_F16>), grid, blk, 0, s, a, rooms);
+        } else if (pano_format == PCL_PANO_F16R) {
+            if (G == 2) hipLaunchKernelGGL((pcl_loss_rooms_kernel<2, PCL_PANO_F16R>), grid, blk, 0, s, a, rooms);
+            else hipLaunchKernelGGL((pcl_loss_rooms_kernel<1, PCL_PANO_F16R>), grid, blk, 0, s, a, rooms);
         } else {
             if (G == 2) hipLaunchKernelGGL((pcl_loss_rooms_kernel<2, PCL_PANO_F32>), grid, blk, 0, s, a, rooms);
             else hipLaunchKernelGGL((pcl_loss_rooms_kernel<1, PCL_PANO_F32>), grid, blk, 0, s, a, rooms);
@@ -470,7 +478,7 @@
                     int B, bool grad, const uint8_t* visible, float* partials, hipStream_t s, int flip, const PclFuseArgs* fuse,
                     const PclDepthLook* depth, int color_sets)
 {
-    if (pano_format != PCL_PANO_F32 && pano_format != PCL_PANO_U8 && pano_format != PCL_PANO_F16) return PCL_EINVAL;
+    if (!pcl_loss_format(pano_format)) return PCL_EINVAL;
     if (n > PCL_MAX_POINTS || (int64_t)(H + 2) * (W + 2) * pcl_texel_bytes(pano_format) >= ((int64_t)1 << 31)) return PCL_EINVAL;
     const bool sets = color_sets > 1;
     if (sets && (B % color_sets || !grad || visible || depth || pcl_cloud_sets_bytes(n, color_sets) == 0)) return PCL_EINVAL;
@@ -501,6 +509,7 @@
     if (sets) {
         if (pano_format == PCL_PANO_U8) pcl_launch_sets<PCL_PANO_U8>(a, fuse, p.G, nblk, s);
         else if (pano_format == PCL_PANO_F16) pcl_launch_sets<PCL_PANO_F16>(a, fuse, p.G, nblk, s);
+        else if (pano_format == PCL_PANO_F16R) pcl_launch_sets<PCL_PANO_F16R>(a, fuse, p.G, nblk, s);
         else pcl_launch_sets<PCL_PANO_F32>(a, fuse, p.G, nblk, s);
         PCL_LAUNCH_CHECK();
         return 0;
@@ -509,12 +518,14 @@
         if (!grad || vis) return PCL_EINVAL;
         if (pano_format == PCL_PANO_U8) pcl_launch_fused<PCL_PANO_U8>(a, *fuse, p.G, nblk, s);
         else if (pano_format == PCL_PANO_F16) pcl_launch_fused<PCL_PANO_F16>(a, *fuse, p.G, nblk, s);
+        else if (pano_format == PCL_PANO_F16R) pcl_launch_fused<PCL_PANO_F16R>(a, *fuse, p.G, nblk, s);
         else pcl_launch_fused<PCL_PANO_F32>(a, *fuse, p.G, nblk, s);
         PCL_LAUNCH_CHECK();
         return 0;
     }
     if (pano_format == PCL_PANO_U8) pcl_launch_f<PCL_PANO_U8>(a, p.G, nblk, grad, vis, s);
     else if (pano_format == PCL_PANO_F16) pcl_launch_f<PCL_PANO_F16>(a, p.G, nblk, grad, vis, s);
+    else if (pano_format == PCL_PANO_F16R) pcl_launch_f<PCL_PANO_F16R>(a, p.G, nblk, grad, vis, s);
     else pcl_launch_f<PCL_PANO_F32>(a, p.G, nblk, grad, vis, s);
     PCL_LAUNCH_CHECK();
     return 0;
diff --git a/piccolo_amd/csrc/pcl_pack.hip b/piccolo_amd/csrc/pcl_pack.hip
--- a/piccolo_amd/csrc/pcl_pack.hip
+++ b/piccolo_amd/csrc/pcl_pack.hip
@@ -29,6 +29,10 @@
     if (H <= 0 || W <= 0) return 0;
     if (pano_format == PCL_PANO_U8P) return (size_t)((H + 3) >> 1) * (size_t)(W + 2) * 8;
     if (pano_format == PCL_PANO_U8V) return (size_t)(H + 2) * (size_t)(W + 2) * 8;
+    if (pano_format == PCL_PANO_F16R) {
+        const int64_t rec = (int64_t)(H + 2) * (W + 2) * 8;
+        return rec >= ((int64_t)1 << 31) ? 0 : (size_t)(pcl_f16r_offset(H, W) + rec);
+    }
     if (pano_format != PCL_PANO_F32 && pano_format != PCL_PANO_U8 && pano_format != PCL_PANO_F16) return 0;
     return (size_t)(H + 2) * (size_t)(W + 2) * (size_t)pcl_texel_bytes(pano_format);
 }
@@ -365,6 +369,33 @@
     return 0;
 }
 
+__global__ void __launch_bounds__(PCL_BLOCK) pcl_pano_f16_records_kernel(const pcl_i2* __restrict__ tex, int H, int W, pcl_i2* __restrict__ rec)
+{
+    typedef _Float16 h4 __attribute__((ext_vector_type(4)));
+    const h4* __restrict__ tx = (const h4*)tex;
+    const int Wp = W + 2;
+    int64_t i = (int64_t)blockIdx.x * PCL_BLOCK + threadIdx.x;
+    if (i >= (int64_t)Wp * (H + 2)) return;
+    const int xp = (int)(i % Wp);
+    const h4 t = tx[i];
+    h4 d = {};
+    if (xp + 1 < Wp) d = tx[i + 1] - t;
+    const h4 r = {t.x, t.y, t.z, d.z};
+    rec[i] = __builtin_bit_cast(pcl_i2, r);
+}
+
+extern "C" size_t pcl_pano_records_offset(int H, int W) { return H <= 0 || W <= 0 ? 0 : (size_t)pcl_f16r_offset(H, W); }
+
+extern "C" int pcl_pano_f16_records(void* pano, int H, int W, void* stream)
+{
+    if (!pano || H <= 0 || W <= 0 || pcl_pano_bytes(H, W, PCL_PANO_F16R) == 0) return PCL_EINVAL;
+    int64_t total = (int64_t)(H + 2) * (W + 2);
+    hipLaunchKernelGGL(pcl_pano_f16_records_kernel, dim3((unsigned)((total + PCL_BLOCK - 1) / PCL_BLOCK)), dim3(PCL_BLOCK), 0,
+                       (hipStream_t)stream, (const pcl_i2*)pano, H, W, (pcl_i2*)((char*)pano + pcl_f16r_offset(H, W)));
+    PCL_LAUNCH_CHECK();
+    return 0;
+}
+
 extern "C" int pcl_pano_pack_u8p(const float* img_hwc, int H, int W, uint32_t* pano, int* not_exact, void* stream)
 {
     if (!img_hwc || !pano || !not_exact || H <= 0 || W <= 0) return PCL_EINVAL;
diff --git a/piccolo_amd/csrc/pcl_sample_device.h b/piccolo_amd/csrc/pcl_sample_device.h
--- a/piccolo_amd/csrc/pcl_sample_device.h
+++ b/piccolo_amd/csrc/pcl_sample_device.h
@@ -61,6 +61,15 @@
 template <> struct PclTaps<PCL_PANO_U8> { pcl_i2 top, bot; };
 template <> struct PclTaps<PCL_PANO_F32> { int voff, row; };
 template <> struct PclTaps<PCL_PANO_F16> { pcl_i4 top, bot; };
+typedef int pcl_i3 __attribute__((ext_vector_type(3)));
+template <> struct PclTaps<PCL_PANO_F16R> { pcl_i3 top, bot; };
+
+template <int FMT>
+__device__ __forceinline__ __amdgpu_buffer_rsrc_t pcl_sample_rsrc(const void* pano, const PclDims& d)
+{
+    if constexpr (FMT == PCL_PANO_F16R) return pcl_tex_rsrc((const char*)pano + pcl_f16r_offset(d.H, d.W), d.H, d.W, pcl_texel_bytes(FMT));
+    else return pcl_tex_rsrc(pano, d.H, d.W, pcl_texel_bytes(FMT));
+}
 
 __device__ __forceinline__ void pcl_issue_taps(__amdgpu_buffer_rsrc_t tex, int x0, int y0, int Wp, PclTaps<PCL_PANO_U8>& o)
 {
@@ -73,6 +82,12 @@
     int voff = (int)(__umul24((unsigned)y0, (unsigned)Wp) + (unsigned)x0) * 8;
     o.top = __builtin_amdgcn_raw_buffer_load_b128(tex, voff, 0, 0);
     o.bot = __builtin_amdgcn_raw_buffer_load_b128(tex, voff, Wp * 8, 0);
+}
+__device__ __forceinline__ void pcl_issue_taps(__amdgpu_buffer_rsrc_t tex, int x0, int y0, int Wp, PclTaps<PCL_PANO_F16R>& o)
+{
+    int voff = (int)(__umul24((unsigned)y0, (unsigned)Wp) + (unsigned)x0) * 8;
+    o.top = __builtin_amdgcn_raw_buffer_load_b96(tex, voff, 0, 0);
+    o.bot = __builtin_amdgcn_raw_buffer_load_b96(tex, voff, Wp * 8, 0);
 }
 __device__ __forceinline__ void pcl_issue_taps(__amdgpu_buffer_rsrc_t tex, int x0, int y0, int Wp, PclTaps<PCL_PANO_F32>& o)
 {
@@ -126,6 +141,32 @@
         o.dh[0] = pcl_mix_lo(fy, dda, dta);
         o.dh[1] = pcl_mix_hi(fy, dda, dta);
         o.dh[2] = pcl_mix_lo(fy, ddb, dtb);
+    }
+}
+
+__device__ __forceinline__ float pcl_mix_hl(float a, pcl_h2 b)
+{
+    float r;
+    asm("v_fma_mix_f32 %0, %1, %2, %2 op_sel:[0,1,0] op_sel_hi:[0,1,1]" : "=v"(r) : "v"(a), "v"(b));
+    return r;
+}
+template <bool GRAD>
+__device__ __forceinline__ void pcl_bilerp_f16(const PclTaps<PCL_PANO_F16R>& r, float fx, float fy, PclBilerp1& o)
+{
+    typedef _Float16 pcl_h8 __attribute__((ext_vector_type(8)));
+    pcl_h8 tv = __builtin_bit_cast(pcl_h8, __builtin_shufflevector(r.top, r.top, 0, 1, 2, 2)),
+           bv = __builtin_bit_cast(pcl_h8, __builtin_shufflevector(r.bot, r.bot, 0, 1, 2, 2));
+    pcl_h2 t00a = __builtin_shufflevector(tv, tv, 0, 1), t00b = __builtin_shufflevector(tv, tv, 2, 3), t01a = __builtin_shufflevector(tv, tv, 4, 5);
+    pcl_h2 t10a = __builtin_shufflevector(bv, bv, 0, 1), t10b = __builtin_shufflevector(bv, bv, 2, 3), t11a = __builtin_shufflevector(bv, bv, 4, 5);
+    pcl_h2 dta = t01a - t00a, dba = t11a - t10a;
+    o.top[0] = pcl_mix_lo(fx, dta, t00a); o.bot[0] = pcl_mix_lo(fx, dba, t10a);
+    o.top[1] = pcl_mix_hi(fx, dta, t00a); o.bot[1] = pcl_mix_hi(fx, dba, t10a);
+    o.top[2] = pcl_mix_hl(fx, t00b); o.bot[2] = pcl_mix_hl(fx, t10b);
+    if (GRAD) {
+        pcl_h2 dda = dba - dta, ddb = t10b - t00b;
+        o.dh[0] = pcl_mix_lo(fy, dda, dta);
+        o.dh[1] = pcl_mix_hi(fy, dda, dta);
+        o.dh[2] = pcl_mix_hi(fy, ddb, t00b);
     }
 }
 
@@ -277,7 +318,7 @@
 {
     const f2 px = o.px, py = o.py, pz = o.pz, fx = o.fx, fy = o.fy;
     f2 c[3], dv[3], dtop[3], dbot[3], dhp[3];
-    if constexpr (FMT == PCL_PANO_F16) {
+    if constexpr (FMT == PCL_PANO_F16 || FMT == PCL_PANO_F16R) {
         PclBilerp1 ba, bb;
         pcl_bilerp_f16<GRAD>(o.ta, fx.x, fy.x, ba);
         pcl_bilerp_f16<GRAD>(o.tb, fx.y, fy.y, bb);
@@ -319,7 +360,7 @@
     acc[0] = pcl_fma2(n2, rn, acc[0]);
     if (GRAD) {
         f2 dh0, dh1, dh2;
-        if constexpr (FMT == PCL_PANO_F16) { dh0 = dhp[0]; dh1 = dhp[1]; dh2 = dhp[2]; }
+        if constexpr (FMT == PCL_PANO_F16 || FMT == PCL_PANO_F16R) { dh0 = dhp[0]; dh1 = dhp[1]; dh2 = dhp[2]; }
         else {
             dh0 = pcl_fma2(fy, dbot[0] - dtop[0], dtop[0]);
             dh1 = pcl_fma2(fy, dbot[1] - dtop[1], dtop[1]);
diff --git a/piccolo_amd/omniloc.py b/piccolo_amd/omniloc.py
--- a/piccolo_amd/omniloc.py
+++ b/piccolo_amd/omniloc.py
@@ -162,7 +162,7 @@
             g._cloud_src = weakref.ref(cloud)
             g._box_src, g._fresh = box, True
             return g
-        gd = _cached("gd", (xyz,), make_private, sub=(B, len(panos), p0.H, p0.W, p0.fmt, fuse, cloud.color_sets) + hyper)
+        gd = _cached("gd", (xyz,), make_private, sub=(B, len(panos), p0.H, p0.W, p0.loss_fmt, fuse, cloud.color_sets) + hyper)
         fresh, gd._fresh = gd._fresh, False
         if gd._cloud_src() is not cloud:
             gd.cloud.data.copy_(cloud.data)
@@ -281,7 +281,7 @@
     B = int(input_trans_list[0].shape[0])
     fmt = ops.refine_texels(xyz.shape[0], imgs[0].shape[0], imgs[0].shape[1])
     panos = [packed_pano(im, n_points=xyz.shape[0]) if I <= 8 else ops.Pano(im, fmt=fmt if ops._known_levels(im) else "auto") for im in imgs]
-    if len({p.fmt for p in panos}) > 1:
+    if len({p.loss_fmt for p in panos}) > 1:
         panos = [ops.Pano(im, fmt="f32") for im in imgs]
     box = quantile_box_of(xyz, _cfg(cfg, "out_of_room_quantile", 0.05))
     tr = torch.cat([ops._dev(t).reshape(B, 3) for t in input_trans_list])
@@ -325,7 +325,7 @@
         g._box_src, g._fresh = list(boxes), True
         return g
     xyzs = tuple(xyz for xyz, _ in rooms)
-    gd = _cached("gd_rooms", xyzs, make_private, sub=(per_room, pano.H, pano.W, pano.fmt, fuse) + hyper)
+    gd = _cached("gd_rooms", xyzs, make_private, sub=(per_room, pano.H, pano.W, pano.loss_fmt, fuse) + hyper)
     fresh, gd._fresh = gd._fresh, False
     for r, c in enumerate(clouds):
         if gd._cloud_src[r]() is not c:
diff --git a/piccolo_amd/ops.py b/piccolo_amd/ops.py
--- a/piccolo_amd/ops.py
+++ b/piccolo_amd/ops.py
@@ -7,6 +7,7 @@
 
 class _Experiment:
     pano_fmt = None
+    f16_records = None
     trim_fmt = None
     gd_graph = None
     verify_levels = False
@@ -141,6 +142,7 @@
             raise ValueError("img must be (H, W, 3)")
         self.H, self.W = int(img.shape[0]), int(img.shape[1])
         self.fmt = None
+        self.records = False
         if fmt not in ("auto", "f16", "u8", "u8p", "u8v", "f32"):
             raise ValueError("unknown texel format %r" % (fmt,))
         prefer = "f16"
@@ -150,18 +152,31 @@
                 fmt = "f32"
         if fmt != "f32":
             fn, code = self._PACK[prefer if fmt == "auto" else fmt]
-            data = _bytes(lib.pcl_pano_bytes(self.H, self.W, code))
+            records = code == _lib.PANO_F16 and f16_records_pay(self.H, self.W)
+            data = _bytes(lib.pcl_pano_bytes(self.H, self.W, _lib.PANO_F16R if records else code))
             known = _known_levels(src)
             flag = _scratch_flag(img.device) if known else torch.zeros(1, dtype=torch.int32, device=img.device)
             _lib.check(getattr(lib, fn)(_ptr(img), self.H, self.W, _ptr(data), _ptr(flag), _stream()), fn)
             if known or int(flag.item()) == 0:
                 self.fmt, self.data = code, data
+                if records:
+                    _lib.check(lib.pcl_pano_f16_records(_ptr(data), self.H, self.W, _stream()), "pcl_pano_f16_records")
+                    self.records = True
             elif fmt != "auto":
                 raise ValueError("image is not exactly k/255: cannot use %s texels" % fmt)
         if self.fmt is None:
             self.fmt = _lib.PANO_F32
             self.data = _bytes(lib.pcl_pano_bytes(self.H, self.W, _lib.PANO_F32))
             _lib.check(lib.pcl_pano_pack(_ptr(img), self.H, self.W, _ptr(self.data), _stream()), "pcl_pano_pack")
+
+    @property
+    def loss_fmt(self):
+        return _lib.PANO_F16R if self.records else self.fmt
+
+
+def f16_records_pay(H, W):
+    fits = 8 * (int(H) + 2) * (int(W) + 2) < (1 << 31)
+    return fits and (EXPERIMENT.f16_records is None or bool(EXPERIMENT.f16_records))
 
 
 _SCRATCH_FLAGS = {}
@@ -240,7 +255,7 @@
         if ws_bytes == 0:
             raise _lib.PiccoloHipError("pcl_loss_depth_workspace_bytes: invalid depth grid %dx%d" % (dh, dw))
         ws = _bytes(ws_bytes)
-        _lib.check(lib.pcl_sampling_loss_depth(_ptr(cloud.data), cloud.n, _ptr(pano.data), pano.fmt, pano.H, pano.W, _ptr(trans), _ptr(rot), B,
+        _lib.check(lib.pcl_sampling_loss_depth(_ptr(cloud.data), cloud.n, _ptr(pano.data), pano.loss_fmt, pano.H, pano.W, _ptr(trans), _ptr(rot), B,
                                                1 if with_grad else 0, dh, dw, tau, st, _ptr(out), _ptr(ws), ws_bytes, _stream()),
                    "pcl_sampling_loss_depth")
         return out
@@ -249,7 +264,7 @@
     vis = None
     if visible is not None:
         vis = _dev(visible, torch.uint8).reshape(B, cloud.n)
-    _lib.check(lib.pcl_sampling_loss(_ptr(cloud.data), cloud.n, _ptr(pano.data), pano.fmt, pano.H, pano.W, _ptr(trans), _ptr(rot), B,
+    _lib.check(lib.pcl_sampling_loss(_ptr(cloud.data), cloud.n, _ptr(pano.data), pano.loss_fmt, pano.H, pano.W, _ptr(trans), _ptr(rot), B,
                                      1 if with_grad else 0, _ptr(vis), _ptr(out), _ptr(ws), ws_bytes, _stream()),
                "pcl_sampling_loss")
     return out
@@ -614,7 +629,7 @@
     def run(self, num_iter, history=False, timer=None):
         lib = _lib.load()
         hist = torch.empty(num_iter, self.B, dtype=F32, device=self.state.device) if history else None
-        _lib.check(lib.pcl_gd_run(_ptr(self.cloud.data), self.cloud.n, _ptr(self.pano.data), self.pano.fmt, self.pano.H, self.pano.W,
+        _lib.check(lib.pcl_gd_run(_ptr(self.cloud.data), self.cloud.n, _ptr(self.pano.data), self.pano.loss_fmt, self.pano.H, self.pano.W,
                                   _ptr(self.state), self.B, _ptr(self.box), ctypes.byref(self.hyper), int(num_iter),
                                   _ptr(hist), _ptr(self.ws), self.ws_bytes, timer.handle if timer else None, _stream()),
                    "pcl_gd_run")
@@ -645,7 +660,7 @@
         lib = _lib.load()
         assert len(panos) == self.B
         for p in panos:
-            if (p.H, p.W, p.fmt) != (self.pano.H, self.pano.W, self.pano.fmt):
+            if (p.H, p.W, p.loss_fmt) != (self.pano.H, self.pano.W, self.pano.loss_fmt):
                 raise ValueError("all panoramas of a launch must share size and texel format")
         self._panos = list(panos)
         self.set_pano_table(torch.tensor([p.data.data_ptr() for p in panos], dtype=torch.int64, device=self.state.device),
@@ -663,7 +678,7 @@
         if I <= 0 or self.B % I:
             raise ValueError("set_pano_groups: %d candidates do not split into %d images" % (self.B, I))
         for p in panos:
-            if (p.H, p.W, p.fmt) != (self.pano.H, self.pano.W, self.pano.fmt):
+            if (p.H, p.W, p.loss_fmt) != (self.pano.H, self.pano.W, self.pano.loss_fmt):
                 raise ValueError("all panoramas of a launch must share size and texel format")
         self._panos = list(panos)
         self.hyper.images = I
@@ -732,7 +747,7 @@
     def run(self, num_iter, history=False, timer=None):
         lib = _lib.load()
         hist = torch.empty(num_iter, self.B, dtype=F32, device=self.state.device) if history else None
-        _lib.check(lib.pcl_gd_run_rooms(self._rooms, self.nrooms, _ptr(self.pano.data), self.pano.fmt, self.pano.H, self.pano.W, _ptr(self.state),
+        _lib.check(lib.pcl_gd_run_rooms(self._rooms, self.nrooms, _ptr(self.pano.data), self.pano.loss_fmt, self.pano.H, self.pano.W, _ptr(self.state),
                                         self.per_room, ctypes.byref(self.hyper), int(num_iter), _ptr(hist), _ptr(self.ws), self.ws_bytes,
                                         timer.handle if timer else None, _stream()), "pcl_gd_run_rooms")
         return hist
```
